# VCISwang/STCD

Hardware: AMD Instinct MI355X
Metric: image-pairs/sec (256x256 bf16 SiamUnet_diff train) (higher is better)
Workload: dtype bf16; 1 GPU; SiamUnet_diff(3,2) 256x256 full training step (fwd + cross_entropy + bwd + AdamW), 16 pairs/GPU, synthetic LEVIR-CD-shaped pairs resident in HBM; global_batch=16, image=256, parallelism=dp1

## Files before the change

include/stcd_hip.h:

```cpp
#ifndef STCD_HIP_H
#define STCD_HIP_H

#include <stdint.h>

#ifdef __cplusplus
extern "C" {
#endif

#define STCD_ABI_VERSION 2

#define STCD_ARCH_DIFF 0
#define STCD_ARCH_CONC 1
#define STCD_ARCH_SUB 2
#define STCD_ARCH_SNUNET 3
#define STCD_ARCH_SEGCD 4
#define STCD_ARCH_SEGCD_R18 5
#define STCD_ARCH_SEGCD_R34 6
#define STCD_ARCH_SEGCD_R101 7
#define STCD_ARCH_SEGCD_R152 8
#define STCD_ARCH_FCEF 9
#define STCD_ARCH_XCONC 10
#define STCD_ARCH_SNUNET_CONC 11
#define STCD_ARCH_SNUNET_CONC_DS 12
#define STCD_ARCH_UNETSEG 16
// ... 16 lines not shown
    int64_t numel;
} stcd_tensor_info;

typedef struct stcd_bn_info {
    char name[64];
    int32_t channels;
    int32_t calls_per_forward;
    int64_t offset;
} stcd_bn_info;

typedef struct stcd_dropout_info {
    char name[64];
    int32_t rows;
    int32_t channels;
    int64_t offset;
} stcd_dropout_info;

typedef struct stcd_cf_config {
    int32_t in_ch, out_ch;
    int32_t embed_dims[4];
    int32_t depths[4];
    int32_t num_heads[4];
    int32_t sr_ratios[4];
    int32_t mlp_ratio;
    int32_t embedding_dim;
    int32_t patch1, patch;
    float drop_rate, attn_drop, drop_path_rate;
    float diff_drop;
} stcd_cf_config;

typedef struct stcd_cf_site {
    char name[96];
    int32_t ndim;
    int32_t dims[4];
    float p;
} stcd_cf_site;

const char* stcd_last_error(void);
int stcd_abi_version(void);

int stcd_create(int arch, int in_ch, int label_ch, int dtype, stcd_engine** out);
int stcd_cf_default_config(stcd_cf_config* cfg);
int stcd_create_changeformer(const stcd_cf_config* cfg, int dtype, stcd_engine** out);
void stcd_destroy(stcd_engine* e);
int64_t stcd_output_floats(const stcd_engine* e);
int stcd_cf_output_info(const stcd_engine* e, int i, int64_t* offset, int* height, int* width);
int stcd_cf_num_sites(const stcd_engine* e);
int stcd_cf_site_get(const stcd_engine* e, int i, stcd_cf_site* out);
uint32_t stcd_cf_site_seed(uint64_t seed, int site);
int stcd_cf_set_drop_rates(stcd_engine* e, float drop_rate, float attn_drop, float diff_drop);
int stcd_cf_set_aux_backward(stcd_engine* e, int on);
int stcd_set_wgrad_side(stcd_engine* e, int on);

int stcd_num_params(const stcd_engine* e);
int stcd_param_info(const stcd_engine* e, int i, stcd_tensor_info* info);
int64_t stcd_param_floats(const stcd_engine* e);
int stcd_num_bn(const stcd_engine* e);
int stcd_bn_info_get(const stcd_engine* e, int i, stcd_bn_info* info);
int64_t stcd_bn_floats(const stcd_engine* e);

int stcd_configure(stcd_engine* e, int batch, int height, int width);
int64_t stcd_workspace_bytes(const stcd_engine* e);
int stcd_num_dropout(const stcd_engine* e);
int stcd_dropout_info_get(const stcd_engine* e, int i, stcd_dropout_info* info);
int64_t stcd_dropout_floats(const stcd_engine* e);
int stcd_set_dropout_p(stcd_engine* e, float p);

int stcd_forward(stcd_engine* e, const float* x1, const float* x2, const float* params, float* bn_running,
                 const float* dropout_masks, uint64_t dropout_seed, int training, float* logits,
                 void* workspace, void* hip_stream);

int stcd_backward(stcd_engine* e, const float* grad_logits, const float* params, float* grads,
                  void* workspace, int stage, void* hip_stream);
int stcd_set_weights_tag(stcd_engine* e, uint64_t tag);
int stcd_grad_stage_range(const stcd_engine* e, int stage, int64_t* begin, int64_t* end);

typedef struct stcd_ws_tensor {
    char name[96];
    int64_t offset_bytes;
    int n, h, w, c, ld;
    int dtype;
} stcd_ws_tensor;
int stcd_set_debug(stcd_engine* e, int flags);
int stcd_ws_tensor_count(const stcd_engine* e);
int stcd_ws_tensor_get(const stcd_engine* e, int index, stcd_ws_tensor* out);

#define STCD_PROFILE_CLASSES 8
int stcd_profile_enable(stcd_engine* e, int on);
int stcd_profile_read(stcd_engine* e, int klass, double* total_ms, int64_t* launches, double* flops, double* bytes);
int stcd_profile_num_kernels(const stcd_engine* e);
int stcd_profile_kernel(stcd_engine* e, int i, char* name, int name_cap, double* total_ms, int64_t* launches, double* flops,
                        double* bytes);

int64_t stcd_loss_scratch_bytes(void);
int stcd_loss_ce(const float* logits, const int64_t* target, int batch, int classes, int64_t hw, int ignore_index,
                 float* loss_out, float* dlogits, void* scratch, void* hip_stream);
int stcd_loss_bce_dice(const float* x, const float* target, int64_t numel, int from_logits, float* loss_out, float* dx,
                       void* scratch, void* hip_stream);
int stcd_loss_contrastive(const float* pred, const int64_t* cd_label, const int64_t* pse_label, int64_t numel_half, float* loss_out,
                          float* dpred, void* scratch, void* hip_stream);
int stcd_loss_focal(const float* x, const int64_t* target, int batch, int classes, int64_t hw, const float* alpha, float gamma,
                    float smooth, int flags, float* loss_out, float* dx, void* scratch, void* hip_stream);
int64_t stcd_loss_iou_scratch_bytes(int batch, int classes, int64_t hw);
int stcd_loss_iou(const float* logits, const int64_t* target, int batch, int classes, int64_t hw, const float* weight, int mode,
                  float* loss_out, float* dlogits, void* scratch, void* hip_stream);
int stcd_confusion_update(const float* logits, const int64_t* target, int batch, int classes, int64_t hw,
                          int64_t* cm, void* hip_stream);

int stcd_adam_step(float* params, const float* grads, float* exp_avg, float* exp_avg_sq, int64_t numel, int64_t step,
                   double lr, double beta1, double beta2, double eps, double weight_decay, int decoupled, void* hip_stream);

int stcd_adam_hyper(int64_t step, double lr, double beta1, double beta2, double eps, double weight_decay, float* hyper_host8);
int stcd_adam_step_dev(float* params, const float* grads, float* exp_avg, float* exp_avg_sq, int64_t numel, const float* hyper_dev8,
                       int decoupled, void* hip_stream);

int stcd_pseudo_pair(const uint8_t* img_a, const uint8_t* donor, const uint8_t* mask, const uint8_t* change, const float* alpha,
                     const int32_t* erase_xywh, uint64_t seed, int batch, int height, int width, const float* mean3,
                     const float* std3, float* x1, float* x2, int64_t* c_label, int64_t* s_label_a, int64_t* s_label_b,
                     void* hip_stream);

int64_t stcd_augment_scratch_bytes(int n_images, int height, int width);
int stcd_augment(const float* x, const float* params, int n_images, int height, int width, const float* mean3, const float* std3,
                 float* out, void* scratch, int64_t scratch_bytes, void* hip_stream);

int stcd_scene_gather(const uint8_t* scene_a, const uint8_t* scene_b, int height, int width, int tile, int stride, int tiles_x,
                      int first_tile, int n_tiles, const float* mean3, const float* std3, float* x1, float* x2, void* hip_stream);
int stcd_scene_stitch(const float* logits, int classes, int height, int width, int tile, int stride, int tiles_x, int tiles_y,
                      int first_tile, int n_tiles, const float* window, float* acc, float* wsum, void* hip_stream);
int stcd_scene_finalize(const float* acc, const float* wsum, int classes, int height, int width, float threshold,
                        const uint8_t* label, uint8_t* mask, float* prob, int64_t* cm, void* hip_stream);
int stcd_scene_gather_d4(const uint8_t* scene_a, const uint8_t* scene_b, int height, int width, int tile, int stride, int tiles_x,
                         int first_tile, int n_tiles, const float* mean3, const float* std3, float* x1, float* x2, int d4,
                         void* hip_stream);
int stcd_scene_stitch_d4(const float* logits, int classes, int height, int width, int tile, int stride, int tiles_x, int tiles_y,
                         int first_tile, int n_tiles, const float* window, float* acc, float* wsum, int d4, void* hip_stream);
int stcd_scene_gather_one_d4(const uint8_t* scene, int height, int width, int tile, int stride, int tiles_x, int first_tile,
                             int n_tiles, const float* mean3, const float* std3, float* x, int d4, void* hip_stream);
#define STCD_SCENE_MAX_HEADS 3
int stcd_scene_stitch_heads_d4(const float* const* logits, int n_heads, int classes, int height, int width, int tile, int stride,
                               int tiles_x, int tiles_y, int first_tile, int n_tiles, const float* window, float* acc, float* wsum,
                               int d4, void* hip_stream);
int stcd_scene_finalize_seg(const float* acc, const float* wsum, int classes, int height, int width, float seg_threshold,
                            float change_threshold, const uint8_t* label_a, const uint8_t* label_b, const uint8_t* label_c,
                            uint8_t* seg_a, uint8_t* seg_b, uint8_t* change, uint8_t* gated, float* prob, int64_t* cm,
                            void* hip_stream);

#define STCD_SELFTRAIN_MAX_MODELS 8
int stcd_selftrain_score(const float* const* logits, int n_models, int batch, int classes, int64_t hw, float threshold,
                         const uint8_t* label, int mask_value, uint8_t* mask, int64_t* agree, int64_t* cm, void* hip_stream);

int stcd_scene_cell_agree(const uint8_t* const* masks, int n_models, int height, int width, int cell, int cells_x, int cells_y,
                          const uint8_t* label, int64_t* agree, int64_t* cm, void* hip_stream);
int stcd_mask_close(const uint8_t* in, int height, int width, int radius, int mask_value, uint8_t* out, void* hip_stream);

int64_t stcd_objects_scratch_bytes(int height, int width);
int stcd_objects_label(const uint8_t* mask, int height, int width, int connectivity, int invert, int32_t* labels, int32_t* count,
                       void* scratch, int64_t scratch_bytes, void* hip_stream);
int stcd_objects_table(const int32_t* labels, int height, int width, int n, const uint8_t* overlay, int64_t* area, int32_t* bbox,
                       int64_t* overlap, void* hip_stream);
int stcd_mask_filter_objects(const uint8_t* in, int height, int width, int connectivity, int64_t min_area, int64_t max_hole,
                             int mask_value, uint8_t* out, void* scratch, int64_t scratch_bytes, void* hip_stream);

int64_t stcd_rings_scratch_bytes(int height, int width, int64_t max_corners);
int stcd_rings_count(const int32_t* labels, int height, int width, int connectivity, int64_t max_corners, int64_t* counts, void* scratch,
                     int64_t scratch_bytes, void* hip_stream);
int stcd_rings_write(const int32_t* labels, int height, int width, int connectivity, int64_t max_corners, int64_t n_rings, int64_t n_vertices,
// ... 105 lines not shown
```

stcd_amd/_lib.py:

```python
from __future__ import annotations

import ctypes as C
import os

import torch

_HERE = os.path.dirname(os.path.abspath(__file__))
LIB_PATH = os.environ.get("STCD_LIB_PATH") or os.path.join(_HERE, "libstcd_hip.so")

ARCH_DIFF, ARCH_CONC, ARCH_SUB, ARCH_SNUNET, ARCH_SEGCD = 0, 1, 2, 3, 4
ARCH_SEGCD_R18, ARCH_SEGCD_R34, ARCH_SEGCD_R101, ARCH_SEGCD_R152 = 5, 6, 7, 8
ARCH_FCEF = 9
ARCH_XCONC = 10
ARCH_SNUNET_CONC = 11
ARCH_SNUNET_CONC_DS = 12
ARCH_UNETSEG = 16
ARCH_FFCTLCD = 32
ARCH_BASE_RESNET = 48
ARCH_BIT = 52
ARCH_CHANGEFORMER = 64
DTYPE_F32, DTYPE_BF16 = 0, 1
ARCH_IDS = {"diff": ARCH_DIFF, "conc": ARCH_CONC, "sub": ARCH_SUB, "fcef": ARCH_FCEF, "xconc": ARCH_XCONC, "snunet": ARCH_SNUNET, "snunet_conc": ARCH_SNUNET_CONC, "snunet_conc_ds": ARCH_SNUNET_CONC_DS, "segcd": ARCH_SEGCD,
            "segcd_resnet50": ARCH_SEGCD, "segcd_resnet18": ARCH_SEGCD_R18, "segcd_resnet34": ARCH_SEGCD_R34,
            "segcd_resnet101": ARCH_SEGCD_R101, "segcd_resnet152": ARCH_SEGCD_R152,
# ... 16 lines not shown
class BnInfo(C.Structure):
    _fields_ = [("name", C.c_char * 64), ("channels", C.c_int32), ("calls_per_forward", C.c_int32),
                ("offset", C.c_int64)]


class DropoutInfo(C.Structure):
    _fields_ = [("name", C.c_char * 64), ("rows", C.c_int32), ("channels", C.c_int32), ("offset", C.c_int64)]


class ConvGeom(C.Structure):
    _fields_ = [("n", C.c_int32), ("hi", C.c_int32), ("wi", C.c_int32), ("ci", C.c_int32), ("ldi", C.c_int32),
                ("hm", C.c_int32), ("wm", C.c_int32), ("in_stride", C.c_int32),
                ("ho", C.c_int32), ("wo", C.c_int32), ("out_stride", C.c_int32), ("oy0", C.c_int32), ("ox0", C.c_int32),
                ("co", C.c_int32), ("ldo", C.c_int32), ("ntaps", C.c_int32),
                ("dy", C.c_int8 * 9), ("dx", C.c_int8 * 9), ("pad_", C.c_int8 * 2)]


class WsTensor(C.Structure):
    _fields_ = [("name", C.c_char * 96), ("offset_bytes", C.c_int64), ("n", C.c_int), ("h", C.c_int), ("w", C.c_int), ("c", C.c_int),
                ("ld", C.c_int), ("dtype", C.c_int)]


class CfConfig(C.Structure):
    _fields_ = [("in_ch", C.c_int32), ("out_ch", C.c_int32), ("embed_dims", C.c_int32 * 4), ("depths", C.c_int32 * 4),
                ("num_heads", C.c_int32 * 4), ("sr_ratios", C.c_int32 * 4), ("mlp_ratio", C.c_int32), ("embedding_dim", C.c_int32),
                ("patch1", C.c_int32), ("patch", C.c_int32), ("drop_rate", C.c_float), ("attn_drop", C.c_float),
                ("drop_path_rate", C.c_float), ("diff_drop", C.c_float)]


class CfSite(C.Structure):
    _fields_ = [("name", C.c_char * 96), ("ndim", C.c_int32), ("dims", C.c_int32 * 4), ("p", C.c_float)]


class MapGeom(C.Structure):
    _fields_ = [("n", C.c_int32), ("h", C.c_int32), ("w", C.c_int32), ("c", C.c_int32), ("groups", C.c_int32)]


CONV_SMALL, CONV_RES, CONV_TILE, CONV_GEMM, CONV_HALO, CONV_DMA = range(6)


class ConvFused(C.Structure):
    _fields_ = [("kernel", C.c_int32), ("groups", C.c_int32),
                ("sum_acc", C.c_void_p), ("sum_c0", C.c_int32), ("sum_c", C.c_int32), ("sum_scale1", C.c_float), ("sum_scale2", C.c_float),
                ("use_epi", C.c_int32), ("relu", C.c_int32), ("gate", C.c_void_p), ("res", C.c_void_p), ("ldg", C.c_int32), ("ldr", C.c_int32),
                ("alpha", C.c_float), ("beta", C.c_float),
                ("bw_y", C.c_void_p), ("bw_stat", C.c_void_p), ("bw_mask", C.c_void_p), ("bw_acc", C.c_void_p), ("bw_ldy", C.c_int32),
                ("blocks", C.c_int32), ("tiles_per_group", C.c_int32), ("blocks_per_group", C.c_int32), ("bn_rep", C.c_int32),
                ("tile_m", C.c_int32)]


_vp, _i, _i64, _f, _d = C.c_void_p, C.c_int, C.c_int64, C.c_float, C.c_double
_PROTOS = {
    "stcd_last_error": (C.c_char_p, []),
    "stcd_abi_version": (_i, []),
    "stcd_create": (_i, [_i, _i, _i, _i, C.POINTER(_vp)]),
    "stcd_destroy": (None, [_vp]),
    "stcd_cf_default_config": (_i, [C.POINTER(CfConfig)]),
    "stcd_create_changeformer": (_i, [C.POINTER(CfConfig), _i, C.POINTER(_vp)]),
    "stcd_output_floats": (_i64, [_vp]),
    "stcd_cf_output_info": (_i, [_vp, _i, C.POINTER(_i64), C.POINTER(_i), C.POINTER(_i)]),
    "stcd_cf_num_sites": (_i, [_vp]),
    "stcd_cf_site_get": (_i, [_vp, _i, C.POINTER(CfSite)]),
    "stcd_cf_site_seed": (C.c_uint32, [C.c_uint64, _i]),
    "stcd_cf_set_drop_rates": (_i, [_vp, _f, _f, _f]),
    "stcd_cf_set_aux_backward": (_i, [_vp, _i]),
    "stcd_set_wgrad_side": (_i, [_vp, _i]),
    "stcd_num_params": (_i, [_vp]),
    "stcd_param_info": (_i, [_vp, _i, C.POINTER(TensorInfo)]),
    "stcd_param_floats": (_i64, [_vp]),
    "stcd_num_bn": (_i, [_vp]),
    "stcd_bn_info_get": (_i, [_vp, _i, C.POINTER(BnInfo)]),
    "stcd_bn_floats": (_i64, [_vp]),
    "stcd_configure": (_i, [_vp, _i, _i, _i]),
    "stcd_workspace_bytes": (_i64, [_vp]),
    "stcd_num_dropout": (_i, [_vp]),
    "stcd_dropout_info_get": (_i, [_vp, _i, C.POINTER(DropoutInfo)]),
    "stcd_dropout_floats": (_i64, [_vp]),
    "stcd_set_dropout_p": (_i, [_vp, _f]),
    "stcd_forward": (_i, [_vp, _vp, _vp, _vp, _vp, _vp, C.c_uint64, _i, _vp, _vp, _vp]),
    "stcd_backward": (_i, [_vp, _vp, _vp, _vp, _vp, _i, _vp]),
    "stcd_grad_stage_range": (_i, [_vp, _i, C.POINTER(_i64), C.POINTER(_i64)]),
    "stcd_set_weights_tag": (_i, [_vp, C.c_uint64]),
    "stcd_set_debug": (_i, [_vp, _i]),
    "stcd_ws_tensor_count": (_i, [_vp]),
    "stcd_ws_tensor_get": (_i, [_vp, _i, C.POINTER(WsTensor)]),
    "stcd_profile_enable": (_i, [_vp, _i]),
    "stcd_profile_read": (_i, [_vp, _i, C.POINTER(C.c_double), C.POINTER(_i64), C.POINTER(C.c_double), C.POINTER(C.c_double)]),
    "stcd_profile_num_kernels": (_i, [_vp]),
    "stcd_profile_kernel": (_i, [_vp, _i, C.c_char_p, _i, C.POINTER(C.c_double), C.POINTER(_i64), C.POINTER(C.c_double), C.POINTER(C.c_double)]),
    "stcd_loss_scratch_bytes": (_i64, []),
    "stcd_loss_ce": (_i, [_vp, _vp, _i, _i, _i64, _i, _vp, _vp, _vp, _vp]),
    "stcd_loss_bce_dice": (_i, [_vp, _vp, _i64, _i, _vp, _vp, _vp, _vp]),
    "stcd_loss_contrastive": (_i, [_vp, _vp, _vp, _i64, _vp, _vp, _vp, _vp]),
    "stcd_loss_focal": (_i, [_vp, _vp, _i, _i, _i64, _vp, _f, _f, _i, _vp, _vp, _vp, _vp]),
    "stcd_loss_iou_scratch_bytes": (_i64, [_i, _i, _i64]),
    "stcd_loss_iou": (_i, [_vp, _vp, _i, _i, _i64, _vp, _i, _vp, _vp, _vp, _vp]),
    "stcd_confusion_update": (_i, [_vp, _vp, _i, _i, _i64, _vp, _vp]),
    "stcd_adam_step": (_i, [_vp, _vp, _vp, _vp, _i64, _i64, _d, _d, _d, _d, _d, _i, _vp]),
    "stcd_adam_hyper": (_i, [_i64, _d, _d, _d, _d, _d, C.POINTER(_f)]),
    "stcd_adam_step_dev": (_i, [_vp, _vp, _vp, _vp, _i64, _vp, _i, _vp]),
    "stcd_pseudo_pair": (_i, [_vp, _vp, _vp, _vp, _vp, _vp, C.c_uint64, _i, _i, _i, C.POINTER(_f), C.POINTER(_f), _vp, _vp, _vp, _vp, _vp, _vp]),
    "stcd_augment_scratch_bytes": (_i64, [_i, _i, _i]),
    "stcd_augment": (_i, [_vp, _vp, _i, _i, _i, C.POINTER(_f), C.POINTER(_f), _vp, _vp, _i64, _vp]),
    "stcd_scene_gather": (_i, [_vp, _vp, _i, _i, _i, _i, _i, _i, _i, C.POINTER(_f), C.POINTER(_f), _vp, _vp, _vp]),
    "stcd_scene_stitch": (_i, [_vp, _i, _i, _i, _i, _i, _i, _i, _i, _i, _vp, _vp, _vp, _vp]),
    "stcd_scene_finalize": (_i, [_vp, _vp, _i, _i, _i, _f, _vp, _vp, _vp, _vp, _vp]),
    "stcd_scene_gather_d4": (_i, [_vp, _vp, _i, _i, _i, _i, _i, _i, _i, C.POINTER(_f), C.POINTER(_f), _vp, _vp, _i, _vp]),
    "stcd_scene_stitch_d4": (_i, [_vp, _i, _i, _i, _i, _i, _i, _i, _i, _i, _vp, _vp, _vp, _i, _vp]),
    "stcd_scene_gather_one_d4": (_i, [_vp, _i, _i, _i, _i, _i, _i, _i, C.POINTER(_f), C.POINTER(_f), _vp, _i, _vp]),
    "stcd_scene_stitch_heads_d4": (_i, [C.POINTER(_vp), _i, _i, _i, _i, _i, _i, _i, _i, _i, _i, _vp, _vp, _vp, _i, _vp]),
    "stcd_scene_finalize_seg": (_i, [_vp, _vp, _i, _i, _i, _f, _f, _vp, _vp, _vp, _vp, _vp, _vp, _vp, _vp, _vp, _vp]),
    "stcd_selftrain_score": (_i, [C.POINTER(_vp), _i, _i, _i, _i64, _f, _vp, _i, _vp, _vp, _vp, _vp]),
    "stcd_scene_cell_agree": (_i, [C.POINTER(_vp), _i, _i, _i, _i, _i, _i, _vp, _vp, _vp, _vp]),
    "stcd_mask_close": (_i, [_vp, _i, _i, _i, _i, _vp, _vp]),
    "stcd_objects_scratch_bytes": (_i64, [_i, _i]),
    "stcd_objects_label": (_i, [_vp, _i, _i, _i, _i, _vp, _vp, _vp, _i64, _vp]),
    "stcd_objects_table": (_i, [_vp, _i, _i, _i, _vp, _vp, _vp, _vp, _vp]),
    "stcd_mask_filter_objects": (_i, [_vp, _i, _i, _i, _i64, _i64, _i, _vp, _vp, _i64, _vp]),
    "stcd_rings_scratch_bytes": (_i64, [_i, _i, _i64]),
    "stcd_rings_count": (_i, [_vp, _i, _i, _i, _i64, _vp, _vp, _i64, _vp]),
    "stcd_rings_write": (_i, [_vp, _i, _i, _i, _i64, _i64, _i64, _vp, _vp, _vp, _vp, _vp, _i64, _vp]),
    "stcd_op_conv": (_i, [_i, _i, C.POINTER(ConvGeom), _vp, _vp, _vp, _vp, _vp, _i64, _vp]),
    "stcd_op_conv_fused": (_i, [C.POINTER(ConvGeom), C.POINTER(ConvFused), _vp, _vp, _vp, _vp, _vp, _i64, _vp]),
    "stcd_op_wgrad": (_i, [_i, _i, C.POINTER(ConvGeom), _vp, _vp, _vp, _vp, _i64, _vp]),
    "stcd_op_scratch_bytes": (_i64, [C.POINTER(ConvGeom)]),
    "stcd_op_ew_scratch_bytes": (_i64, [C.POINTER(MapGeom)]),
    "stcd_op_bn_act": (_i, [_i, C.POINTER(MapGeom), _vp, _i, _vp, _vp, _vp, _vp, _vp, _i, _i, _vp, _i, _vp, _i, _vp, _vp, _i64, _vp]),
    "stcd_op_bn_act_pair": (_i, [_i, C.POINTER(MapGeom), _vp, _i, _vp, _vp, _vp, _vp, _vp, _i, _vp, _i, _vp, _i, _vp, _i, _vp, _vp, _i64, _vp]),
    "stcd_op_bn_act_bwd": (_i, [_i, C.POINTER(MapGeom), _vp, _i, _vp, _i, _vp, _vp, _i, _vp, _i, _vp, _vp, _vp, _i64, _vp]),
    "stcd_op_maxpool": (_i, [_i, C.POINTER(MapGeom), _vp, _i, _vp, _i, _vp]),
    "stcd_op_maxpool_bwd": (_i, [_i, C.POINTER(MapGeom), _vp, _i, _vp, _i, _vp, _i, _i, _vp]),
    "stcd_op_maxpool3": (_i, [_i, C.POINTER(MapGeom), _vp, _i, _vp, _i, _vp, _vp]),
    "stcd_op_maxpool3_bwd": (_i, [_i, C.POINTER(MapGeom), _vp, _vp, _i, _vp, _i, _vp]),
    "stcd_op_pairdw_scratch_bytes": (_i64, [C.POINTER(MapGeom)]),
    "stcd_op_pairdw": (_i, [_i, C.POINTER(MapGeom), _vp, _i, _vp, _vp, _vp, _i, _vp]),
    "stcd_op_pairdw_bwd": (_i, [_i, C.POINTER(MapGeom), _vp, _i, _vp, _i, _vp, _vp, _i, _vp, _vp, _i64, _vp]),
    "stcd_op_fuse": (_i, [_i, _i, C.POINTER(MapGeom), _vp, _i, _vp, _i, _vp]),
    "stcd_op_fuse_bwd": (_i, [_i, _i, C.POINTER(MapGeom), _vp, _i, _vp, _i, _vp, _i, _vp]),
    "stcd_op_rep_pad": (_i, [_i, C.POINTER(MapGeom), _vp, _i, _i, _i, _vp]),
    "stcd_op_rep_pad_bwd": (_i, [_i, C.POINTER(MapGeom), _vp, _i, _i, _i, _vp]),
    "stcd_op_skip_bwd": (_i, [_i, _i, C.POINTER(MapGeom), _vp, _i, _vp, _i, _vp, _i, _vp, _i, _vp, _vp, _vp, _i, _vp, _i, _vp, _vp, _vp, _i64, _vp]),
    "stcd_op_cf_scratch_bytes": (_i64, [_i64, _i, _i, _i, _i]),
    "stcd_op_cf_im2col": (_i, [_i, _vp, _vp, _i, _i, _i, _i, _i, _i, _i, _i, _vp]),
    "stcd_op_cf_col2im": (_i, [_i, _vp, _i, _vp, _i, _i, _i, _i, _i, _i, _i, _i, _vp]),
    "stcd_op_cf_layernorm": (_i, [_i, _vp, _vp, _vp, _vp, _vp, _i64, _i, _f, _vp]),
    "stcd_op_cf_layernorm_bwd": (_i, [_i, _vp, _vp, _vp, _vp, _vp, _vp, _vp, _vp, _vp, _vp, _i64, _i, _vp]),
    "stcd_op_cf_colsum": (_i, [_i, _vp, _i64, _i, _vp, _vp, _vp]),
    "stcd_op_cf_attention": (_i, [_i, _vp, _vp, _vp, _vp, _i, _i, _i, _i, _i, _f, C.c_uint64, _vp]),
    "stcd_op_cf_attention_scratch_bytes": (_i64, [_i, _i, _i, _i, _i]),
    "stcd_op_cf_attention_bwd": (_i, [_i, _vp, _vp, _vp, _vp, _vp, _vp, _vp, _vp, _i, _i, _i, _i, _i, _f, C.c_uint64, _vp]),
    "stcd_op_cf_dwgelu": (_i, [_i, _vp, _vp, _vp, _vp, _vp, _i, _i, _i, _i, _f, C.c_uint64, _vp]),
    "stcd_op_cf_dwgelu_scratch_bytes": (_i64, [_i, _i, _i, _i]),
    "stcd_op_cf_dwgelu_bwd": (_i, [_i, _vp, _vp, _vp, _vp, _vp, _vp, _vp, _vp, _i, _i, _i, _i, _f, C.c_uint64, _vp]),
    "stcd_op_cf_resid_drop": (_i, [_i, _vp, _vp, _vp, _i, _i64, _i, _f, _f, C.c_uint64, _i, _vp]),
    "stcd_op_cf_bilinear": (_i, [_i, _vp, _vp, _i, _i, _i, _i, _i, _i, _i, _i, _vp]),
    "stcd_op_cf_elementwise": (_i, [_i, _i, _vp, _vp, _vp, _i64, _i, _vp, _f, _f, _f, C.c_uint64, _vp]),
    "stcd_op_cf_prelu_bwd": (_i, [_i, _vp, _vp, _vp, _vp, _vp, _vp, _i64, _i, _vp]),
}
EXPORTS = tuple(_PROTOS)

_lib = None


class StcdError(RuntimeError):
    pass

# ... 22 lines not shown
```

stcd_amd/csrc/common.h:

```cpp
#pragma once
#include <hip/hip_runtime.h>
#include <stdint.h>
#include <stdio.h>
#include <stdlib.h>
#include <string>
#include <string.h>

#include "../../include/stcd_hip.h"

namespace stcd {

typedef __bf16 bf16;

enum DType { F32 = STCD_DTYPE_F32, BF16 = STCD_DTYPE_BF16 };
inline size_t dsize(int dt) { return dt == BF16 ? 2 : 4; }

void set_error(const std::string& msg);

static inline int env_int(const char* name, int dflt) { const char* v = getenv(name); return v ? atoi(v) : dflt; }
static inline bool env_flag(const char* name, bool dflt) { const char* v = getenv(name); return v && v[0] == (dflt ? '0' : '1') ? !dflt : dflt; }

#define STCD_CHECK_AS(fn, cond, msg)                                       \
    do {                                                                   \
        if (!(cond)) {                                                     \
            ::stcd::set_error(std::string(fn) + ": " + (msg));             \
            return 1;                                                      \
        }                                                                  \
    } while (0)
#define STCD_CHECK(cond, msg) STCD_CHECK_AS(__func__, cond, msg)

#define STCD_HIP(call)                                                                        \
    do {                                                                                      \
        hipError_t err_ = (call);                                                             \
        if (err_ != hipSuccess) {                                                             \
            ::stcd::set_error(std::string(__func__) + ": " #call ": " + hipGetErrorString(err_)); \
            return 1;                                                                         \
        }                                                                                     \
    } while (0)

template <typename T>
__device__ __forceinline__ void load8(const T* p, float (&v)[8]);
template <>
__device__ __forceinline__ void load8<float>(const float* p, float (&v)[8]) {
    float4 a = *reinterpret_cast<const float4*>(p), b = *reinterpret_cast<const float4*>(p + 4);
    v[0] = a.x; v[1] = a.y; v[2] = a.z; v[3] = a.w; v[4] = b.x; v[5] = b.y; v[6] = b.z; v[7] = b.w;
}
template <>
__device__ __forceinline__ void load8<bf16>(const bf16* p, float (&v)[8]) {
    uint4 r = *reinterpret_cast<const uint4*>(p);
    uint32_t w[4] = {r.x, r.y, r.z, r.w};
#pragma unroll
    for (int i = 0; i < 4; ++i) {
        v[2 * i] = __uint_as_float(w[i] << 16);
        v[2 * i + 1] = __uint_as_float(w[i] & 0xffff0000u);
    }
}
template <typename T>
__device__ __forceinline__ void store8(T* p, const float (&v)[8]);
template <>
__device__ __forceinline__ void store8<float>(float* p, const float (&v)[8]) {
    *reinterpret_cast<float4*>(p) = make_float4(v[0], v[1], v[2], v[3]);
    *reinterpret_cast<float4*>(p + 4) = make_float4(v[4], v[5], v[6], v[7]);
}
__device__ __forceinline__ void barrier_lds() { asm volatile("s_waitcnt lgkmcnt(0)\n\ts_barrier" ::: "memory"); }

__device__ __forceinline__ uint32_t pack_bf16x2(float lo, float hi) {
    typedef __attribute__((ext_vector_type(2))) __bf16 bf16x2;
    bf16x2 t;
    t[0] = (__bf16)lo;
    t[1] = (__bf16)hi;
    return __builtin_bit_cast(uint32_t, t);
}
template <>
__device__ __forceinline__ void store8<bf16>(bf16* p, const float (&v)[8]) {
    uint4 r;
    r.x = pack_bf16x2(v[0], v[1]); r.y = pack_bf16x2(v[2], v[3]);
    r.z = pack_bf16x2(v[4], v[5]); r.w = pack_bf16x2(v[6], v[7]);
    *reinterpret_cast<uint4*>(p) = r;
}
template <typename T>
__device__ __forceinline__ float round_as(float v) { return (float)(T)v; }

__device__ __forceinline__ float wave_sum(float v) {
#pragma unroll
    for (int o = 32; o > 0; o >>= 1) v += __shfl_xor(v, o, 64);
    return v;
}

constexpr int BN_REP = 8;
constexpr float BN_FS1 = 67108864.f;
constexpr float BN_FS2 = 262144.f;
constexpr float BN_BS = 68719476736.f;
inline int64_t bn_acc_bytes(int groups, int C) { return (int64_t)BN_REP * groups * 2 * C * 8; }
__device__ __forceinline__ void bn_acc_add(long long* acc, int rep, int groups, int C, int g, int which, int c, double v, float scale) {
    const long long q = (long long)llrint(v * (double)scale);
    atomicAdd(reinterpret_cast<unsigned long long*>(acc + (((int64_t)(rep & (BN_REP - 1)) * groups + g) * 2 + which) * C + c),
              (unsigned long long)q);
}
__device__ __forceinline__ double bn_acc_get(const long long* __restrict__ acc, int groups, int C, int g, int which, int c, float scale) {
    long long s = 0;
#pragma unroll
    for (int r = 0; r < BN_REP; ++r) s += acc[(((int64_t)r * groups + g) * 2 + which) * C + c];
    return (double)s * (1.0 / (double)scale);
}
__device__ __forceinline__ double bn_rsqrt(double x) {
    double y = (double)__frsqrt_rn((float)x);
    y = y * (1.5 - 0.5 * x * y * y);
    return y * (1.5 - 0.5 * x * y * y);
}

__device__ __forceinline__ void bn_fwd_table(float* tab, const long long* __restrict__ facc, const float* __restrict__ gamma,
                                             const float* __restrict__ beta, float* __restrict__ rmean, float* __restrict__ rvar,
                                             float* __restrict__ stat, int C, int groups, int64_t ppg, float momentum, float eps,
                                             bool publish, int cbase = 0, int CS = 0, int g_first = 0) {
    if (CS == 0) CS = C;
    const double inv_n = 1.0 / (double)ppg;
    for (int cl = threadIdx.x; cl < CS; cl += blockDim.x) {
        const int c = cbase + cl;
        if (facc) {
            const float gam = gamma[c], bet = beta[c];
            float rm = (publish && rmean) ? rmean[c] : 0.f, rv = (publish && rvar) ? rvar[c] : 0.f;
            for (int gi = 0; gi < groups; ++gi) {
                int g = gi + g_first;
                if (g >= groups) g -= groups;
                const double s1 = bn_acc_get(facc, groups, C, g, 0, c, BN_FS1), s2 = bn_acc_get(facc, groups, C, g, 1, c, BN_FS2);
                const double mean = s1 * inv_n;
                double var = s2 * inv_n - mean * mean;
                if (var < 0.0) var = 0.0;
                const double invstd = bn_rsqrt(var + (double)eps);
                const float sc = (float)(gam * invstd), sh = (float)(bet - mean * gam * invstd);
                tab[(g * 2 + 0) * CS + cl] = sc;
                tab[(g * 2 + 1) * CS + cl] = sh;
                if (publish) {
                    float* st = stat + (int64_t)g * 4 * C;
                    st[c] = (float)mean; st[C + c] = (float)invstd; st[2 * C + c] = sc; st[3 * C + c] = sh;
                    const double unb = ppg > 1 ? var * ((double)ppg / (double)(ppg - 1)) : var;
                    rm = (float)((1.0 - momentum) * rm + momentum * mean);
                    rv = (float)((1.0 - momentum) * rv + momentum * unb);
                }
            }
            if (publish && rmean) rmean[c] = rm;
            if (publish && rvar) rvar[c] = rv;
        } else if (gamma) {
            const float invstd = 1.f / sqrtf(rvar[c] + eps);
            const float sc = gamma[c] * invstd, sh = beta[c] - rmean[c] * gamma[c] * invstd;
            for (int g = 0; g < groups; ++g) {
                tab[(g * 2 + 0) * CS + cl] = sc;
                tab[(g * 2 + 1) * CS + cl] = sh;
            }
        } else {
            for (int g = 0; g < groups; ++g) {
                tab[(g * 2 + 0) * CS + cl] = stat[(int64_t)g * 4 * C + 2 * C + c];
                tab[(g * 2 + 1) * CS + cl] = stat[(int64_t)g * 4 * C + 3 * C + c];
            }
        }
    }
}

struct XfSrc {
    const long long* facc = nullptr;
    const float* gamma = nullptr;
    const float* beta = nullptr;
    float* rmean = nullptr; float* rvar = nullptr;
    float* stat = nullptr;
    const float* mask = nullptr;
    int C = 0, groups = 1, npg = 0, publish = 0;
    long long ppg = 0;
    float momentum = 0.1f, eps = 1e-5f;
    int on = 0;
};
__device__ __forceinline__ uint4 xf_act8(const uint4 raw, const float (&sc)[8], const float (&sh)[8], const unsigned okm) {
    typedef short s16x2 __attribute__((ext_vector_type(2)));
    const uint32_t w[4] = {raw.x, raw.y, raw.z, raw.w};
    uint32_t o[4];
#pragma unroll
    for (int i = 0; i < 4; ++i) {
        const float lo = fmaf(__uint_as_float(w[i] << 16), sc[2 * i], sh[2 * i]);
        const float hi = fmaf(__uint_as_float(w[i] & 0xffff0000u), sc[2 * i + 1], sh[2 * i + 1]);
        const s16x2 p = __builtin_bit_cast(s16x2, pack_bf16x2(lo, hi));
        o[i] = __builtin_bit_cast(uint32_t, __builtin_elementwise_max(p, s16x2{0, 0})) & okm;
    }
    return make_uint4(o[0], o[1], o[2], o[3]);
}
__device__ __forceinline__ void xf_fold8(const float* __restrict__ tab_sc, const float* __restrict__ tab_sh, const float4 m0, const float4 m1,
                                         float (&sc)[8], float (&sh)[8]) {
    const float mk[8] = {m0.x, m0.y, m0.z, m0.w, m1.x, m1.y, m1.z, m1.w};
#pragma unroll
    for (int j = 0; j < 8; ++j) { sc[j] = tab_sc[j] * mk[j]; sh[j] = tab_sh[j] * mk[j]; }
}


void launch_in_pack(int dt, const float* x1, const float* x2, void* X, int B, int cin, int H, int W, hipStream_t s, int dates = 2);
void launch_gout_pack(int dt, const float* g, void* G, int B, int L, int H, int W, hipStream_t s, long long* bias_acc = nullptr);
struct BiasJob { int64_t acc_off; int64_t out_off; int C, valid; float scale; int pad_; };
void launch_bias_finish(const BiasJob* jobs_dev, int njobs, const char* ws, float* grads, hipStream_t s);

void launch_conv_ref(int dt, const stcd_conv_geom& g, const void* in, const float* w, int kpad, int wld,
                     const float* bias, void* out, bool out_nchw_f32, hipStream_t s);
void launch_wgrad_ref(int dt, const stcd_conv_geom& g, const void* in, const void* dout, float* dw, int kpad, int wld,
                      hipStream_t s);
void launch_wgrad_ref_f64(int dt, const stcd_conv_geom& g, const void* in, const void* dout, double* dw, int kpad, int wld,
                          hipStream_t s);

struct ConvMfmaPlan {
    int CiB = 0, nchunks = 0, KS = 0, modeB = 0, NT = 0, NTtot = 0;
    int64_t wf_elems = 0;
    bool ok = false;
};
ConvMfmaPlan conv_mfma_plan(const stcd_conv_geom& g);
void launch_pack_frag(const stcd_conv_geom& g, const ConvMfmaPlan& p, const float* w, int kpad, int wld, void* dst,
                      hipStream_t s);
int launch_conv_mfma(const stcd_conv_geom& g, const ConvMfmaPlan& p, const void* in, const void* wf, const float* bias,
                     void* out, bool out_nchw_f32, hipStream_t s);
bool conv_mfma_x4_ok(const stcd_conv_geom g[4], const ConvMfmaPlan p[4]);
int launch_conv_mfma_x4(const stcd_conv_geom g[4], const ConvMfmaPlan p[4], const void* in, const void* const wf[4],
                        const float* bias, void* out, hipStream_t s);
struct ConvResPlan {
    int NT = 0, CW = 32, nslices = 0, P = 0, blocks = 0;
    int filt_bytes = 0, lds_bytes = 0;
    int single_halo = 0;
    bool ok = false;
};
ConvResPlan conv_res_plan(const stcd_conv_geom& g, const ConvMfmaPlan& p, int groups);
struct BwdSum {
    const void* Y = nullptr; int ldy = 0;
    const float* stat = nullptr;
    const float* mask = nullptr;
    long long* acc = nullptr;
    int groups = 1;
};
int launch_conv_res(const stcd_conv_geom& g, const ConvMfmaPlan& p, const ConvResPlan& rp, const void* in, const void* wf,
                    const float* bias, void* out, int groups, long long* stat_acc, int cpad, hipStream_t s, int stat_c0 = 0,
                    float s1_scale = BN_FS1, float s2_scale = BN_FS2, const XfSrc* xf = nullptr, const BwdSum* bs = nullptr);
bool conv_res_bwdsum_ok(const stcd_conv_geom& g, const ConvResPlan& rp);
bool conv_res_xf_ok(const stcd_conv_geom& g, const ConvResPlan& rp, int groups, const XfSrc& xf);
struct ConvTilePlan {
    int NT = 0, nparts = 0, nbuf = 0, nslices = 0, P = 0, blocks = 0, ntiles = 0;
    int filt_bytes = 0, lds_bytes = 0;
    bool ok = false;
};
ConvTilePlan conv_tile_plan(const stcd_conv_geom& g, const ConvMfmaPlan& p, int groups);
int launch_conv_tile(const stcd_conv_geom& g, const ConvMfmaPlan& p, const ConvTilePlan& tp, const void* in, const void* wf,
                     const float* bias, void* out, int groups, long long* stat_acc, int cpad, hipStream_t s, int stat_c0 = 0,
                     float s1_scale = BN_FS1, float s2_scale = BN_FS2);
struct ConvGemmPlan {
    int W = 0;
    int tiles_m = 0, tiles_n = 0, blocks = 0, lds_bytes = 0;
    int pix_chunks = 0;
    bool ok = false;
};
ConvGemmPlan conv_gemm_plan(const stcd_conv_geom& g, const ConvMfmaPlan& p, int groups);
struct ConvEpi {
    int relu = 0;
    const void* gate = nullptr; int ldg = 0;
    const void* res = nullptr; int ldr = 0;
    float alpha = 1.f, beta = 1.f;
};
int launch_conv_gemm(const stcd_conv_geom& g, const ConvMfmaPlan& p, const ConvGemmPlan& gp, const void* in, const void* wf,
                   const float* bias, void* out, int groups, long long* stat_acc, int cpad, hipStream_t s, int stat_c0 = 0,
                   float s1_scale = BN_FS1, float s2_scale = BN_FS2, const ConvEpi* epi = nullptr);
struct ConvHaloPlan {
    int NH = 0;
    int nslices = 0, P = 0, blocks = 0, lds_bytes = 0;
    bool ok = false;
};
ConvHaloPlan conv_halo_plan(const stcd_conv_geom& g, const ConvMfmaPlan& p);
int launch_conv_halo(const stcd_conv_geom& g, const ConvMfmaPlan& p, const ConvHaloPlan& hp, const void* in, const void* wf,
                     const float* bias, void* out, hipStream_t s, const ConvEpi* epi = nullptr);

struct ConvDmaPlan {
    int tiles_m = 0, tiles_n = 0, blocks = 0, lds_bytes = 0;
    bool ok = false;
};
ConvDmaPlan conv_dma_plan(const stcd_conv_geom& g, const ConvMfmaPlan& p);
int launch_conv_dma(const stcd_conv_geom& g, const ConvMfmaPlan& p, const ConvDmaPlan& dp, const void* in, const void* wf,
                    const float* bias, void* out, hipStream_t s, const ConvEpi* epi = nullptr);
// ... 6 lines not shown
bool conv_small_call_ok(const stcd_conv_geom& g, int groups, const XfSrc* xf);
bool conv_small_bwdsum_ok(const stcd_conv_geom& g);
struct WgradMfmaPlan {
    int WCI = 1, NTW = 1, gx = 1, gy = 1, gz = 1;
    int64_t slab_floats = 0;
    int wi_valid = 0;
    int gemm = 0;
    int dma = 0;
    bool ok = false;
};
WgradMfmaPlan wgrad_mfma_plan(const stcd_conv_geom& g, int kpad, int wld, bool allow_wide = false, int force_co64 = -1);
int launch_wgrad_mfma(const stcd_conv_geom& g, const WgradMfmaPlan& p, const void* in, const void* dout, float* slab,
                      int kpad, int wld, hipStream_t s);
struct WgradJob {
    stcd_conv_geom g;
    int64_t in_off, dout_off, slab_off;
    int kpad, wld;
    int dymin, dxmin, HH, HWp;
    int tiles_x, tiles_y, ntiles;
    int xrow_bytes;
    int x_bytes, y_bytes;
    int co_valid;
    unsigned in_bytes, dout_bytes;
    int gx, gy, gz;
    int start;
    int lds_bytes;
    int wi_valid;
    int dma_L, dma_nk;
    int pad_;
    int64_t xf_stat_off, xf_mask_off;
    int xf_C, xf_groups, xf_npg, pad2_;
};
WgradMfmaPlan wgrad_gemm_plan(const stcd_conv_geom& g, int kpad, int wld);
WgradJob wgrad_gemm_make_job(const stcd_conv_geom& g, const WgradMfmaPlan& p, int64_t in_off, int64_t dout_off, int64_t slab_off,
                             int kpad, int wld);
int launch_wgrad_gemm_group(int W, const WgradJob* jobs_dev, int njobs, int total_blocks, const char* base, hipStream_t s);
WgradMfmaPlan wgrad_dma_plan(const stcd_conv_geom& g, int kpad, int wld);
void wgrad_dma_set_split(WgradMfmaPlan& p, const stcd_conv_geom& g, int S, int kpad, int wld);
WgradJob wgrad_dma_make_job(const stcd_conv_geom& g, const WgradMfmaPlan& p, int64_t in_off, int64_t dout_off, int64_t slab_off,
                            int kpad, int wld);
int launch_wgrad_dma_group(const WgradJob* jobs_dev, int njobs, int total_blocks, const char* base, hipStream_t s);
WgradJob wgrad_make_job(const stcd_conv_geom& g, const WgradMfmaPlan& p, int64_t in_off, int64_t dout_off, int64_t slab_off,
                        int kpad, int wld);
void wgrad_job_set_xf(WgradJob& a, int64_t stat_off, int64_t mask_off, int C, int groups, int npg);
int wgrad_variant_slots(int WCI, int NTW, bool t9, int lds_bytes);
int launch_wgrad_group(int WCI, int NTW, bool t9, const WgradJob* jobs_dev, int njobs, int total_blocks, int lds_bytes,
                       const char* base, hipStream_t s, bool xf = false);
struct PackSpec;
struct ReduceJob {
    int64_t start, count;
    int64_t slab_off;
    int64_t out_off;
    int64_t slab_stride;
    int gx, ntaps, K, N, kpad, wld;
    int ks, kn_major;
    int8_t ky[9], kx[9];
    int8_t tiled, parts, pad_[4];
};
void launch_reduce_jobs(const ReduceJob* jobs_dev, int njobs, int64_t total, const char* ws, float* grads, hipStream_t s);
void launch_reduce_dw(const float* slab, int gx, const stcd_conv_geom& g, int K, int N, int kpad, int wld,
                      const PackSpec* ps, float* out, hipStream_t s);

struct PackSpec {
    int ks;
    int kn_major;
    int K, N, wld;
    int kpad;
    int ntaps;
    int8_t ky[9], kx[9];
};
void launch_pack_w(const PackSpec& ps, const float* src, float* dst, hipStream_t s);
void launch_unpack_dw(const PackSpec& ps, const double* dwe, float* gsrc, hipStream_t s);

struct PackJob {
    int64_t start, count;
    int64_t src_off;
    int64_t dst_off;
    int kind;
    PackSpec ps;
    int Ci, Co, CiB, nchunks, KS, NTtot, modeB;
    int aux;
};
void launch_pack_jobs(const PackJob* jobs_dev, int njobs, int64_t total, const float* params, char* ws, hipStream_t s);

int bn_stats_chunks(int64_t pixels_per_group, int C);
void launch_bn_stats(int dt, const void* Y, int ld, int C, int groups, int64_t pixels_per_group, long long* acc, hipStream_t s);
void launch_bn_eval_prepare(int C, int groups, const float* gamma, const float* beta, const float* running_mean,
                            const float* running_var, float* stat, float eps, hipStream_t s);
constexpr int MAX_VIEWS = 6;
struct SliceViews {
    int n = 0;
    void* p[MAX_VIEWS]; int ld[MAX_VIEWS]; int64_t goff[MAX_VIEWS]; int gmask[MAX_VIEWS];
};
struct BnActArgs {
    const void* Y; int ldy;
    void* A; int lda; int64_t a_group_off;
    void* P; int ldp;
    float* stat;
    const float* mask;
    int C, groups, npg, H, W;
    int relu;
    const void* res = nullptr; int ldres = 0;
    const long long* facc = nullptr;
    const float* gamma = nullptr; const float* beta = nullptr;
    float* running_mean = nullptr; float* running_var = nullptr;
    float momentum = 0.1f, eps = 1e-5f;
    SliceViews extra;
    int g_first = 0;
};
void launch_bn_act(int dt, const BnActArgs& a, hipStream_t s);
void launch_bn_act_pair(int dt, const BnActArgs& a, void* F, int ldf, int fmode, hipStream_t s);
void launch_maxpool(int dt, const void* A, int lda, void* P, int ldp, int N, int H, int W, int C, hipStream_t s);

void launch_fuse(int dt, int mode, const void* A, int lda, int64_t a_goff, void* D, int ldd, int B, int64_t HW, int C,
                 hipStream_t s);
void launch_fuse_bwd(int dt, int mode, const void* A, int lda, int64_t a_goff, const void* dD, int ldd, void* dA, int ldda,
                     int64_t da_goff, int B, int64_t HW, int C, hipStream_t s);
void launch_rep_pad(int dt, void* D, int ld, int N, int H, int W, int h0, int w0, int C, hipStream_t s);
void launch_rep_pad_bwd(int dt, void* dD, int ld, int N, int H, int W, int h0, int w0, int C, hipStream_t s);

void launch_bn_bwd_reduce(int dt, const void* dA, int ldda, int64_t da_goff, const void* Y, int ldy, const float* stat,
                          const float* mask, int C, int groups, int npg, int64_t HW, int relu, long long* bacc,
                          hipStream_t s, const void* res = nullptr, int ldres = 0, const SliceViews* extra_src = nullptr,
                          int base_valid = 1, void* dA_sum = nullptr);
void launch_bn_bwd_apply(int dt, const void* dA, int ldda, int64_t da_goff, void* dY, int lddy, const void* Y, int ldy,
                         const float* stat, const long long* bacc, float* dgamma, float* dbeta, const float* mask, int C, int groups,
                         int npg, int64_t HW, int relu, hipStream_t s, const void* res = nullptr, int ldres = 0,
                         void* dZout = nullptr, int lddz = 0, const void* extra = nullptr, int ldex = 0,
                         float* dbeta_copy = nullptr);
void launch_pairdw_fwd(int dt, const void* A, int lda, int64_t goff, void* G, int ldg, const float* w, const float* b, int B, int H,
                       int W, int C, hipStream_t s);
void launch_pairdw_bwd_data(int dt, const void* dG, int lddg, void* dA, int ldda, int64_t goff, const float* w, int B, int H, int W,
                            int C, hipStream_t s);
int64_t pairdw_partial_floats(int B, int H, int W, int C);
void launch_pairdw_bwd_filter(int dt, const void* A, int lda, int64_t goff, const void* dG, int lddg, float* dw, float* partial, int B,
                              int H, int W, int C, hipStream_t s);
void launch_slice(int dt, void* dst, int ldd, const void* src, int lds, int64_t pixels, int C, int accumulate, hipStream_t s);
void launch_ecam_forward(int dt, const void* X, int ld, void* Z, int ldz, int N, int64_t HW, int C4, const float* w1a,
                         const float* w2a, const float* w1b, const float* w2b, float* pool, int64_t* argm, float* att,
                         float* hid, float* part, hipStream_t s);
int64_t ecam_part_floats(int N, int C4);
void launch_ecam_backward(int dt, const void* X, int ld, const void* dZ, int lddz, void* dX, int lddx, int N, int64_t HW, int C4,
                          const float* w1a, const float* w2a, const float* w1b, const float* w2b, float* gw1a, float* gw2a,
                          float* gw1b, float* gw2b, const float* pool, const int64_t* argm, const float* att, const float* hid,
                          float* sums, float* dpool, float* part, hipStream_t s);
struct SnHeadParams { const float* w[4]; const float* b[4]; const float* wf; const float* bf; int L, ds; };
struct SnHeadGrads { float* w[4]; float* b[4]; float* wf; float* bf; };
int64_t snhead_scratch_floats(int B, int64_t HW, int L, int ds);
void launch_snhead_forward(int dt, const void* E, int ld, const SnHeadParams& p, float* out, int B, int64_t HW, hipStream_t s);
void launch_snhead_backward(int dt, const void* E, int ld, const SnHeadParams& p, const SnHeadGrads& g, const float* G, void* dE,
                            int ldd, float* scratch, int B, int64_t HW, hipStream_t s);
void launch_pool_bwd(int dt, const void* A, int lda, int64_t a_goff, const void* dP, int ldp, void* dA, int ldda,
                     int64_t da_goff, int groups, int npg, int H, int W, int C, int accumulate, hipStream_t s);
bool skip_pair_supported(int B, int H, int W, int C);
void launch_skip_bwd_pair(int dt, int mode, const void* Y, int ldy, const void* dD, int ldd, const void* dP, int ldp, void* dA,
                          int ldda, int64_t da_goff, const float* stat, const float* mask, int B, int H, int W, int C,
                          long long* partial, hipStream_t s);
void launch_skip_bwd(int dt, int mode, const void* A, int lda, int64_t a_goff, const void* Y, int ldy, const void* dD, int ldd,
                     const void* dP, int ldp, void* dA, int ldda, int64_t da_goff, const float* stat, const float* mask, int B,
                     int H, int W, int C, long long* bacc, hipStream_t s);
void launch_bias_grad(int dt, const void* dY, int ld, int64_t pixels, int C, float* db, hipStream_t s, long long* acc_i = nullptr);
void launch_dropout_gen(float* mask, int64_t n, uint64_t seed, float p, hipStream_t s);
void launch_fill(float* p, int64_t n, float v, hipStream_t s);

void launch_stem_fwd(int dt, const void* X, const float* w, void* Y, int N, int H, int W, int cin, int Co, hipStream_t s);
int64_t stem_wgrad_part_floats(int N, int H, int W, int cin, int Co);
// ... 160 lines not shown
```

stcd_amd/csrc/engine.hip:

```cpp
#include <algorithm>
#include <climits>
#include <cstdint>
#include <array>
#include <cstring>
#include <memory>
#include <vector>

#include "common.h"

namespace stcd {

static thread_local std::string g_err;
void set_error(const std::string& msg) { g_err = msg; }

enum ConvKind { K_CONV3 = 0, K_CONVT3_S1 = 1, K_UPCONV = 2, K_CONV1 = 3, K_CONVT2 = 4, K_CONV3_S2 = 5, K_CONV1_S2 = 6, K_STEM7 = 7 };

struct TRef { int64_t off = -1; int ld = 0; };
struct GRef { int64_t off = -1; int ld = 0; int64_t goff = 0; };

static inline int round8(int c) { return (c + 7) & ~7; }

struct ConvW {
    std::string name;
    int kind = 0, cin = 0, cout = 0;
// ... 139 lines not shown
    std::vector<ViewRef> extra_dst;
    std::vector<ViewRef> grad_src;
    bool grad_base = false;
    ConvOp f1, f2, d1, d2; WgradOp w1, w2;
};
struct SnUp {
    int conv = -1, N = 0, h = 0, w = 0, C = 0;
    TRef src, dsrc, out, dOut, tmp;
    ConvOp fwd[4], dgr; WgradOp wg[4];
    int64_t bias_acc = -1; bool bias_fused = false; int coff = 0;
};

struct CfPlan;
struct stcd_engine_impl {
    Prof prof;
    std::shared_ptr<CfPlan> cf;
    std::vector<NBlock> sn_blocks;
    std::vector<SnUp> sn_ups;
    std::vector<int> sn_order;
    std::vector<XConc> xc;
    int sn_final = -1;
    int64_t sn_w[4] = {0, 0, 0, 0};
    TRef snE, sndE, snZ, sndZ;
    TRef sn_dbg_dE;
    int64_t sn_pool = -1, sn_argm = -1, sn_att = -1, sn_hid = -1, sn_sums = -1, sn_dpool = -1, sn_part = -1;
    int64_t sn_dout_begin = -1, sn_dout_end = -1;
    ConvOp sn_final_fwd, sn_final_dgr; WgradOp sn_final_wg;
    int64_t snc_w[5] = {0, 0, 0, 0, 0}, snc_b[5] = {0, 0, 0, 0, 0}, snc_scratch = -1;
    std::vector<GLayer> g_layers;
    std::vector<GStep> g_fwd;
    int g_stem = -1, g_head_conv = -1;
    int debug_flags = 0;
    std::vector<stcd_ws_tensor> ws_tensors;
    std::vector<std::array<int, 4>> g_blocks;
    int seg_x = 4, seg_layers[4] = {3, 4, 6, 3};
    int seg_dates = 2;
    bool seg_ffc = false;
    TRef g_pool_idc;
    std::vector<std::array<int, 2>> g_dec;
    TRef gP0, gdP0, gX3, gdX3, gFuseTmp;
    int64_t g_pool_idx = -1;
    int64_t g_stem_part = -1;
    int64_t g_raw3 = -1, g_draw3 = -1;
    ConvOp g_head_fwd, g_head_dgr; WgradOp g_head_wg;
    bool bres = false; int seg_nstage = 4;
    int g_head_c = 16;
    int g_cls = -1, g_pred_conv = -1;
    ConvOp g_pred_fwd, g_pred_dgr; WgradOp g_pred_wg;
    int64_t g_pred_bias_acc = -1;
    struct BitPlan {
        bool on = false; int L = 1, dh = 64;
        int64_t pos_off = 0, wa_off = 0, enc_off = 0, dec_off = 0;
        int64_t tok_in = -1, tok_out = -1, dtok_out = -1, dtok_in = -1, stat = -1, AP = -1, dAP = -1, xs = -1, dG = -1, dec_part = -1,
                dmh = -1, dm = -1, enc_part = -1, tok_part = -1;
        TRef dec_din;
    } bit;
    int arch = 0, in_ch = 3, label = 2, dt = F32;
    int64_t min_bn_count = 0;
    float drop_p = 0.2f;
    std::vector<stcd_tensor_info> params;
    int64_t param_floats = 0, enc_param_end = 0;
    std::vector<ConvW> convs;
    std::vector<BnP> bns;
    int64_t bn_floats = 0;
    bool configured = false, fwd_training = false;
    int B = 0, H = 0, W = 0;
    std::vector<DropP> drops;
    int64_t drop_floats = 0;
    int64_t ws_bytes = 0;
    std::vector<Cbrd> enc, dec;
    std::vector<UpConv> ups;
    int final_conv = -1;
    ConvOp final_fwd, final_dgr; WgradOp final_wg;
    const Cbrd* final_dgr_bwd = nullptr;
    const Cbrd* final_xsrc = nullptr;
    int use_virt = 0;
    int fc_virt_layers = 0;
    std::vector<ConvOp*> conv_ops;
    int64_t slab = -1, slab_floats = 0;
    std::vector<WgradOp*> wgrad_ops;
    std::vector<WgradGroup> wgroups[2];
    std::vector<ReduceJob> rjobs[2];
    int64_t rjobs_total[2] = {0, 0}, rjobs_off[2] = {-1, -1};
    std::vector<PackJob> jobs[2];
    int64_t jobs_total[2] = {0, 0}, jobs_off[2] = {-1, -1};
    const void* jobs_uploaded_ws = nullptr;
    uint64_t weights_tag = 0, packed_tag = 0;
    const void* packed_ws = nullptr; const void* packed_params = nullptr; int packed_level = -1;
    TRef X0, G, finalIn, dFinalIn;
    int Hs[5] = {0}, Ws[5] = {0};
    TRef D[4], dD[4], P[4], dP[4];
    int64_t zero_begin = -1, zero_end = -1;
    int64_t final_bias_acc = -1;
    std::vector<BiasJob> bias_jobs; int64_t bias_jobs_off = -1;
    int64_t masks = -1, dwe_begin = -1, dwe_end = -1, scratch8 = -1;
    int use_mfma = 1, use_small = 1, use_wgroup = 1, use_res = 1, use_skip_fused = 1, use_act_fuse = 1, use_gemm = 1, use_skip_recompute = 1, use_bwdsum = 1, use_bwdsum_res = 0, use_tile = 1, use_halo = 0;
    int wg_side_on = 1;
    static constexpr int WG_SIDE_DIV = 4;
    static constexpr int WGROUP_ROUNDS = 1, WGROUP_MIN_TILES = 8;
    bool wg_early = false; hipStream_t wg_cur_side = nullptr;
    hipStream_t wg_side = nullptr; hipEvent_t wg_fork = nullptr, wg_join = nullptr; int wg_side_dev = -1;
};

}

using namespace stcd;
struct stcd_engine : stcd_engine_impl {};

namespace stcd {

static const int ENC_STAGE_CONVS[4] = {2, 2, 3, 3};
static const int ENC_C[4] = {16, 32, 64, 128};
static const int SKIP_IDX[4] = {1, 3, 6, 9};

static void add_param(stcd_engine& e, const std::string& name, std::initializer_list<int64_t> shape, int64_t* off_out) {
    stcd_tensor_info ti;
    memset(&ti, 0, sizeof(ti));
    snprintf(ti.name, sizeof(ti.name), "%s", name.c_str());
    ti.ndim = (int)shape.size();
    int64_t n = 1;
    int i = 0;
    for (auto s : shape) { ti.shape[i++] = s; n *= s; }
    ti.numel = n;
    ti.offset = e.param_floats;
    *off_out = ti.offset;
    e.param_floats += (n + 3) & ~(int64_t)3;
    e.params.push_back(ti);
}

static void make_specs(ConvW& c, bool need_dgrad) {
    if (c.kind == K_STEM7) {
        c.fwd = PackSpec{}; c.dgrad = PackSpec{};
        c.fwd.ks = 7; c.fwd.K = c.cin; c.fwd.N = c.cout; c.fwd.kpad = c.kin_p; c.fwd.wld = c.nout_p;
        return;
    }
    if (c.kind == K_CONV3_S2) {
        PackSpec& f = c.fwd;
        f.ks = 3; f.K = c.cin; f.N = c.cout; f.kpad = c.kin_p; f.wld = c.nout_p; f.ntaps = 9; f.kn_major = 0;
        {
            int t = 0;
            for (int py = 0; py < 2; ++py)
                for (int px = 0; px < 2; ++px)
                    for (int ky = 0; ky < 3; ++ky)
                        for (int kx = 0; kx < 3; ++kx)
                            if ((ky != 1) == (py == 1) && (kx != 1) == (px == 1)) { f.ky[t] = ky; f.kx[t] = kx; ++t; }
        }
        PackSpec& d = c.dgrad;
        d.ks = 3; d.K = c.cout; d.N = c.cin; d.kpad = c.nout_p; d.wld = round8(c.cin); d.ntaps = need_dgrad ? 9 : 0; d.kn_major = 1;
        int t = 0;
        for (int py = 0; py < 2; ++py)
            for (int px = 0; px < 2; ++px)
                for (int dy = 0; dy <= py; ++dy)
                    for (int dx = 0; dx <= px; ++dx) { d.ky[t] = py + 1 - 2 * dy; d.kx[t] = px + 1 - 2 * dx; ++t; }
        return;
    }
    if (c.kind == K_CONV1 || c.kind == K_CONVT2 || c.kind == K_CONV1_S2) {
        const int ks = c.kind == K_CONVT2 ? 2 : 1;
        PackSpec& f = c.fwd;
        f.ks = ks; f.K = c.cin; f.N = c.cout; f.kpad = c.kin_p; f.wld = c.nout_p;
        f.ntaps = ks * ks;
        f.kn_major = c.kind == K_CONVT2;
        for (int t = 0; t < f.ntaps; ++t) { f.ky[t] = t / ks; f.kx[t] = t % ks; }
        PackSpec& d = c.dgrad;
        d.ks = ks; d.K = c.cout; d.N = c.cin; d.kpad = c.nout_p; d.wld = round8(c.cin);
        d.ntaps = need_dgrad ? ks * ks : 0;
        d.kn_major = c.kind != K_CONVT2;
// ... 242 lines not shown

constexpr int TILE_MAX_TILES = 512;
static void pick_tile(const stcd_engine& e, ConvOp& op, const stcd_conv_geom& g, int groups) {
    if (!e.use_tile || !op.res.ok || op.gemm.ok || op.small) return;
    const ConvTilePlan tp = conv_tile_plan(g, op.plan, groups);
    if (tp.ok && tp.ntiles <= TILE_MAX_TILES) op.tile = tp;
}

static WgradMfmaPlan pick_wgrad_plan(const stcd_engine& e, const stcd_conv_geom& g, int kpad, int wld) {
    if (e.use_gemm && e.use_wgroup && 2.0 * g.n * g.hm * g.wm * (double)g.ci * g.co >= 0.8e9) {
        WgradMfmaPlan p = wgrad_gemm_plan(g, kpad, wld);
        if (p.ok) return p;
    }
    if (e.use_wgroup && (g.ntaps == 9 || (e.cf && g.ntaps == 4)) && (int64_t)g.n * g.hm * g.wm >= 65536) {
        WgradMfmaPlan p = wgrad_dma_plan(g, kpad, wld);
        if (p.ok) return p;
    }
    return wgrad_mfma_plan(g, kpad, wld, is_snunet(e.arch) || (e.cf && g.ntaps == 9));
}

static void plan_conv(const stcd_engine& e, ConvOp& op, int groups, bool with_tile) {
    op.plan = conv_mfma_plan(op.g);
    op.small = conv_small_ok(op.g, op.plan);
    if (e.use_res && !op.small) op.res = conv_res_plan(op.g, op.plan, groups);
    pick_gemm_or_res(e, op, op.g, groups);
    if (with_tile) pick_tile(e, op, op.g, groups);
}
static bool conv_on_ref(bool mfma, const ConvOp& op) { return !(mfma && op.plan.ok && op.wf >= 0); }
struct Binder {
    stcd_engine& e; Planner& ws;
    bool with_tile = false;
    void conv(ConvOp& op, const stcd_conv_geom& g, int conv, bool dgrad, int tap0, int kreal, int nreal, int groups = 1) const {
        op = ConvOp();
        op.g = g; op.conv = conv; op.dgrad = dgrad; op.tap0 = tap0; op.kreal = kreal; op.nreal = nreal; op.res_groups = groups;
        if (e.dt == BF16) plan_conv(e, op, groups, with_tile);
        if (op.plan.ok) op.wf = ws.take(op.plan.wf_elems * 2);
        e.conv_ops.push_back(&op);
    }
    void stem(ConvOp& op, const stcd_conv_geom& g, int conv, int groups) const {
        op = ConvOp();
        op.g = g; op.conv = conv; op.kreal = e.convs[conv].cin; op.nreal = g.co; op.res_groups = groups;
        op.plan = conv_mfma_plan(g);
        if (g.ldi == 8 && g.co % 64 == 0) op.gemm = conv_gemm_plan(g, op.plan, groups);
        op.gemm.pix_chunks = 1;
        if (!op.gemm.ok) return;
        op.wf = ws.take(op.plan.wf_elems * 2);
        e.conv_ops.push_back(&op);
    }
    void wgrad(WgradOp& op, const stcd_conv_geom& g, int conv, int64_t in_off, int64_t dout_off, int stage = 0, int tap0 = 0,
               int wi_valid = 0, const int8_t* own_ky = nullptr, const int8_t* own_kx = nullptr) const {
        const ConvW& cv = e.convs[conv];
        op = WgradOp();
        op.g = g; op.conv = conv; op.tap0 = tap0; op.kreal = cv.cin; op.nreal = cv.cout;
        op.in_off = in_off; op.dout_off = dout_off; op.stage = stage;
        op.own_taps = own_ky != nullptr;
        for (int t = 0; t < g.ntaps && op.own_taps; ++t) { op.oky[t] = own_ky[t]; op.okx[t] = own_kx[t]; }
        if (e.dt == BF16) { op.plan = pick_wgrad_plan(e, g, cv.fwd.kpad, cv.fwd.wld); op.plan.wi_valid = wi_valid; }
        e.wgrad_ops.push_back(&op);
    }
};
static void take_ref_images(stcd_engine& e, Planner& ws, bool with_dwe = true) {
    for (auto& c : e.convs) {
        c.wpk_fwd = ws.take((int64_t)c.fwd.ntaps * c.fwd.kpad * c.fwd.wld * 4);
        if (c.dgrad.ntaps) c.wpk_dgrad = ws.take((int64_t)c.dgrad.ntaps * c.dgrad.kpad * c.dgrad.wld * 4);
    }
    e.dwe_begin = ws.cur;
    for (auto& c : e.convs) {
        c.dwe_floats = (int64_t)c.fwd.ntaps * c.fwd.kpad * c.fwd.wld;
        c.dwe = with_dwe ? ws.take(c.dwe_floats * 8) : -1;
    }
    e.dwe_end = ws.cur;
}

static bool same_group(const WgradGroup& G, const WgradOp& op) {
    const bool t9 = !op.plan.dma && op.g.ntaps == 9;
    return G.gemm == op.plan.gemm && G.dma == op.plan.dma && G.WCI == op.plan.WCI && G.NTW == op.plan.NTW && G.t9 == t9 && G.xf == (op.xf_C > 0);
}

static bool cf_side_on() { static const bool on = env_flag("STCD_CF_SIDE", true); return on; }

static void build_pack_jobs(stcd_engine& e, Planner& ws) {
    for (int st = 0; st < 2; ++st) { e.rjobs[st].clear(); e.rjobs_total[st] = 0; }
    for (int st = 0; st < 2; ++st) e.wgroups[st].clear();
    if (e.dt == BF16 && e.use_mfma) {
        if (e.use_wgroup) {
            for (WgradOp* op : e.wgrad_ops) {
                if (!op->plan.ok) continue;
                const bool t9 = !op->plan.dma && op->g.ntaps == 9;
                std::vector<WgradGroup>& gs = e.wgroups[op->stage];
                size_t gi = 0;
                while (gi < gs.size() && !same_group(gs[gi], *op)) ++gi;
                if (gi == gs.size()) { WgradGroup g; g.WCI = op->plan.WCI; g.NTW = op->plan.NTW; g.t9 = t9; g.gemm = op->plan.gemm; g.dma = op->plan.dma; g.xf = op->xf_C > 0; gs.push_back(g); }
                op->grouped = true;
            }
            for (int st = 0; st < 2; ++st)
                for (WgradGroup& G : e.wgroups[st]) {
                    if (G.gemm) { G.lds_bytes = 2 * 2 * G.gemm * (64 * 64 + 8 * 32); continue; }
                    if (G.dma) {
                        G.lds_bytes = 128 * 1024;
                        std::vector<WgradOp*> dops;
                        for (WgradOp* op : e.wgrad_ops)
                            if (op->grouped && op->stage == st && op->plan.dma) dops.push_back(op);
                        auto blocks_at = [&](int64_t kt) {
                            int64_t b = 0;
                            for (WgradOp* op : dops) {
                                const int64_t M = (int64_t)op->g.n * op->g.hi * op->g.wi;
                                b += ((M + kt * 64 - 1) / (kt * 64)) * op->plan.gy * op->plan.gz;
                            }
                            return b;
                        };
                        int64_t lo = 1, hi = 1;
                        const int dma_blocks = e.wg_side_on && cf_side_on() ? 192 : 256;
                        while (blocks_at(hi) > dma_blocks) hi *= 2;
                        while (lo < hi) { const int64_t mid = (lo + hi) / 2; if (blocks_at(mid) <= dma_blocks) hi = mid; else lo = mid + 1; }
                        for (WgradOp* op : dops) {
                            const ConvW& cv = e.convs[op->conv];
                            const int64_t M = (int64_t)op->g.n * op->g.hi * op->g.wi;
                            int64_t S = (M + lo * 64 - 1) / (lo * 64);
                            const int64_t slab_bytes = (int64_t)op->g.ntaps * cv.fwd.kpad * cv.fwd.wld * 4;
                            S = std::min<int64_t>(S, std::max<int64_t>(1, ((int64_t)64 << 20) / slab_bytes));
                            wgrad_dma_set_split(op->plan, op->g, (int)S, cv.fwd.kpad, cv.fwd.wld);
                        }
                        continue;
                    }
                    std::vector<WgradOp*> ops;
                    int64_t W = 0;
                    for (WgradOp* op : e.wgrad_ops)
                        if (op->grouped && op->stage == st && same_group(G, *op)) {
                            ops.push_back(op);
                            const int64_t ntiles = (int64_t)op->g.n * ((op->g.wm + 15) / 16) * ((op->g.hm + 7) / 8);
                            W += ntiles * op->plan.gy * op->plan.gz;
                        }
                    for (WgradOp* op : ops) {
                        const ConvW& cv = e.convs[op->conv];
                        WgradJob j = wgrad_make_job(op->g, op->plan, 0, 0, 0, cv.fwd.kpad, cv.fwd.wld);
                        if (op->xf_C > 0) wgrad_job_set_xf(j, op->xf_stat_off, op->xf_mask_off, op->xf_C, op->xf_groups, op->xf_npg);
                        G.lds_bytes = std::max(G.lds_bytes, j.lds_bytes);
                    }
                    int slots = wgrad_variant_slots(G.WCI, G.NTW, G.t9, G.lds_bytes);
                    if (st == 0 && e.wg_side_on && fc_family(e)) slots = std::max(64, slots / stcd_engine_impl::WG_SIDE_DIV);
                    const int64_t rounds = stcd_engine_impl::WGROUP_ROUNDS;
                    const int64_t tpb = std::max<int64_t>(stcd_engine_impl::WGROUP_MIN_TILES, (W + rounds * slots - 1) / (rounds * slots));
                    for (WgradOp* op : ops) {
                        const ConvW& cv = e.convs[op->conv];
                        const int64_t ntiles = (int64_t)op->g.n * ((op->g.wm + 15) / 16) * ((op->g.hm + 7) / 8);
                        const int64_t slab_bytes = (int64_t)op->g.ntaps * cv.fwd.kpad * cv.fwd.wld * 4;
                        int64_t gx = std::max<int64_t>(1, (ntiles + tpb - 1) / tpb);
                        gx = std::min<int64_t>(gx, std::max<int64_t>(1, ((int64_t)32 << 20) / slab_bytes));
                        op->plan.gx = (int)gx;
                        op->plan.slab_floats = gx * op->g.ntaps * cv.fwd.kpad * cv.fwd.wld;
                    }
                }
        }
        int64_t cur[2] = {0, 0};
        for (WgradOp* op : e.wgrad_ops) {
            if (!op->plan.ok) continue;
            const ConvW& cv = e.convs[op->conv];
            op->slab = ws.take(op->plan.slab_floats * 4);
            if (op->grouped) {
                for (WgradGroup& G : e.wgroups[op->stage])
                    if (same_group(G, *op)) {
                        op->group = (int)(&G - e.wgroups[op->stage].data());
                        WgradJob j = op->plan.dma ? wgrad_dma_make_job(op->g, op->plan, op->in_off, op->dout_off, op->slab, cv.fwd.kpad, cv.fwd.wld)
                                   : op->plan.gemm ? wgrad_gemm_make_job(op->g, op->plan, op->in_off, op->dout_off, op->slab, cv.fwd.kpad, cv.fwd.wld)
                                                   : wgrad_make_job(op->g, op->plan, op->in_off, op->dout_off, op->slab, cv.fwd.kpad, cv.fwd.wld);
                        if (op->xf_C > 0 && !op->plan.dma && !op->plan.gemm) wgrad_job_set_xf(j, op->xf_stat_off, op->xf_mask_off, op->xf_C, op->xf_groups, op->xf_npg);
                        j.start = G.total_blocks;
                        G.total_blocks += j.gx * j.gy * j.gz;
                        G.jobs.push_back(j);
                        double fl, by;
                        conv_work(e, op->g, op->kreal, op->nreal, &fl, &by);
                        G.flops += fl; G.bytes += by;
                    }
            }
            ReduceJob j{};
            j.slab_off = op->slab; j.out_off = cv.w_off;
            j.slab_stride = (int64_t)op->g.ntaps * cv.fwd.kpad * cv.fwd.wld;
            j.gx = op->plan.gx; j.ntaps = op->g.ntaps; j.K = cv.cin; j.N = cv.cout; j.kpad = cv.fwd.kpad; j.wld = cv.fwd.wld;
            j.ks = cv.fwd.ks; j.kn_major = cv.fwd.kn_major;
            for (int t = 0; t < op->g.ntaps; ++t) {
                j.ky[t] = op->own_taps ? op->oky[t] : cv.fwd.ky[op->tap0 + t];
                j.kx[t] = op->own_taps ? op->okx[t] : cv.fwd.kx[op->tap0 + t];
            }
            j.tiled = (int64_t)j.ntaps * j.K * j.N >= 512 * 1024;
            if (!j.tiled) {
                const int64_t outs = (int64_t)j.ntaps * j.K * j.N;
                int parts = 1;
                while (parts < 64 && parts * 32 < j.gx) parts *= 2;
                j.parts = (int8_t)parts;
                const int64_t OUTS = 256 / parts;
                j.count = ((outs + OUTS - 1) / OUTS) * 256;
            } else {
                const int TK = j.ntaps == 1 ? 32 : 16;
                const int64_t ntiles = (int64_t)((j.N + 31) / 32) * ((j.K + TK - 1) / TK);
                j.parts = 1;
                j.count = ntiles * 256;
            }
            j.start = cur[op->stage];
            cur[op->stage] += (j.count + 255) & ~(int64_t)255;
            e.rjobs[op->stage].push_back(j);
        }
        for (int st = 0; st < 2; ++st) {
            e.rjobs_total[st] = cur[st];
            e.rjobs_off[st] = ws.take((int64_t)e.rjobs[st].size() * sizeof(ReduceJob) + 16);
            for (WgradGroup& G : e.wgroups[st]) G.table_off = ws.take((int64_t)G.jobs.size() * sizeof(WgradJob) + 16);
        }
    }
    for (int with_dgrad = 0; with_dgrad < 2; ++with_dgrad) {
        std::vector<PackJob>& jobs = e.jobs[with_dgrad];
        jobs.clear();
        int64_t cur = 0;
        auto push = [&](PackJob j) { j.start = cur; cur += (j.count + 255) & ~(int64_t)255; jobs.push_back(j); };
        const bool mfma = e.dt == BF16 && e.use_mfma;
        if (!mfma) {
            for (auto& cv : e.convs)
                for (int d = 0; d <= with_dgrad; ++d) {
                    const PackSpec& ps = d ? cv.dgrad : cv.fwd;
                    if (!ps.ntaps) continue;
                    PackJob j{};
                    j.kind = 0; j.ps = ps; j.src_off = cv.w_off; j.dst_off = d ? cv.wpk_dgrad : cv.wpk_fwd;
                    j.count = (int64_t)ps.ntaps * ps.kpad * ps.wld;
                    push(j);
                }
        } else {
            for (const ConvOp* op : e.conv_ops) {
                if (op->dgrad && !with_dgrad) continue;
                const ConvW& cv = e.convs[op->conv];
                const PackSpec& full = op->dgrad ? cv.dgrad : cv.fwd;
                PackJob j{};
                j.ps = full;
                j.ps.ntaps = op->g.ntaps;
                for (int t = 0; t < op->g.ntaps; ++t) { j.ps.ky[t] = full.ky[op->tap0 + t]; j.ps.kx[t] = full.kx[op->tap0 + t]; }
                j.src_off = cv.w_off;
                if (cv.kind == K_STEM7) {
                    j.kind = 2; j.dst_off = op->wf; j.count = op->plan.wf_elems;
                    j.Co = cv.cout; j.NTtot = op->plan.NTtot; j.aux = cv.cin;
                    push(j);
                    continue;
                }
                if (!conv_on_ref(true, *op)) {
                    j.kind = 1; j.dst_off = op->wf;
                    j.count = op->plan.modeB ? op->plan.wf_elems : op->plan.wf_elems / op->g.ntaps;
                    j.Ci = op->g.ci; j.Co = op->g.co; j.CiB = op->plan.CiB; j.nchunks = op->plan.nchunks; j.KS = op->plan.KS;
                    j.NTtot = op->plan.NTtot; j.modeB = op->plan.modeB;
                } else {
                    j.kind = 0;
                    j.dst_off = (op->dgrad ? cv.wpk_dgrad : cv.wpk_fwd) + (int64_t)op->tap0 * full.kpad * full.wld * 4;
                    j.count = (int64_t)j.ps.ntaps * full.kpad * full.wld;
                }
                push(j);
            }
        }
        e.jobs_total[with_dgrad] = cur;
        e.jobs_off[with_dgrad] = ws.take((int64_t)jobs.size() * sizeof(PackJob) + 16);
    }
}

static int configure_fcsiam(stcd_engine& e, int B, int H, int W) {
    const int64_t T = (int64_t)dsize(e.dt);
    const int ND = fc_dates(e);
    e.Hs[0] = H; e.Ws[0] = W;
    for (int s = 0; s < 4; ++s) { e.Hs[s + 1] = e.Hs[s] / 2; e.Ws[s + 1] = e.Ws[s] / 2; }
    Planner ws(e);
    auto add_drop = [&](const std::string& name, int rows, int C) {
        DropP d; d.name = name; d.rows = rows; d.C = C; d.off = e.drop_floats;
        e.drop_floats += (int64_t)rows * C;
        e.drops.push_back(d);
        return (int)e.drops.size() - 1;
    };

    e.X0 = ws.plain(ND * B, H, W, 8);
    for (int s = 0; s < 4; ++s) {
        int Cd = ENC_C[s] + (e.arch == STCD_ARCH_CONC ? 2 : 1) * ENC_C[s];
        e.D[s] = ws.plain(B, e.Hs[s], e.Ws[s], Cd);
        e.dD[s] = ws.plain(B, e.Hs[s], e.Ws[s], Cd);
        e.P[s] = ws.plain(ND * B, e.Hs[s + 1], e.Ws[s + 1], ENC_C[s]);
        e.dP[s] = ws.plain(ND * B, e.Hs[s + 1], e.Ws[s + 1], ENC_C[s]);
    }
    auto r256 = [](int64_t b) { return (b + 255) & ~(int64_t)255; };
    auto zero_arena = [&](int64_t at, bool assign) {
        auto acc = [&](int groups, int C) { const int64_t o = at; at += r256(bn_acc_bytes(groups, C)); return o; };
        for (int s = 0; s < 4 && fc_cross(e); ++s) {
            const int C = ENC_C[s];
// ... 169 lines not shown
            for (size_t i = 1; i < v.size(); ++i) {
                Cbrd& N = v[i]; Cbrd& P = v[i - 1];
                if (N.has_dIn && N.dgr_sum_acc < 0 && dest_ok(P, N.dgr, N.dIn.off, N.dIn.ld, N.N)) { N.dgr_bwd = &P; P.bwd_sums_fused = true; }
            }
        };
        scan(e.enc); scan(e.dec);
        if (!e.dec.empty() && dest_ok(e.dec.back(), e.final_dgr, e.dFinalIn.off, e.dFinalIn.ld, e.dec.back().N)) {
            e.final_dgr_bwd = &e.dec.back(); e.dec.back().bwd_sums_fused = true;
        }
    }

    e.final_xsrc = nullptr; e.fc_virt_layers = 0;
    for (auto& L : e.enc) { L.virt = false; L.xsrc = nullptr; }
    for (auto& L : e.dec) { L.virt = false; L.xsrc = nullptr; }
    if (e.use_virt && e.dt == BF16 && e.use_mfma && e.use_wgroup && !fc_cross(e)) {
        auto fwd_ok = [&](const ConvOp& op, bool nchw) {
            if (op.wf < 0 || (op.gemm.ok && !nchw)) return false;
            if (op.small && e.use_small) return true;
            return op.res.ok && !nchw && !op.res.single_halo;
        };
        auto wg_ok = [&](const WgradOp& op) { return op.plan.ok && !op.plan.gemm && !op.plan.dma && op.plan.WCI < 4 && op.plan.NTW < 4; };
        auto link = [&](Cbrd& P, ConvOp& cf, WgradOp& cw, bool nchw) {
            if (P.pool || P.fuse_dst.off >= 0) return false;
            if (!fwd_ok(cf, nchw) || !wg_ok(cw)) return false;
            P.virt = true; ++e.fc_virt_layers;
            cw.in_off = P.Y.off;
            cw.xf_stat_off = P.stat;
            cw.xf_mask_off = (P.drop >= 0) ? e.masks + e.drops[P.drop].off * 4 : -1;
            cw.xf_C = e.convs[P.conv].cout; cw.xf_groups = P.groups; cw.xf_npg = P.npg;
            return true;
        };
        for (size_t i = 0; i + 1 < e.enc.size(); ++i) {
            Cbrd& P = e.enc[i]; Cbrd& Cn = e.enc[i + 1];
            if (Cn.in.off != P.A.off) continue;
            if (link(P, Cn.fwd, Cn.wg, false)) { Cn.xsrc = &P; Cn.in.off = P.Y.off; Cn.in.ld = P.Y.ld; }
        }
        for (size_t i = 0; i < e.dec.size(); ++i) {
            Cbrd& P = e.dec[i];
            if (i + 1 < e.dec.size() && e.dec[i + 1].in.off == P.A.off) {
                Cbrd& Cn = e.dec[i + 1];
                if (link(P, Cn.fwd, Cn.wg, false)) { Cn.xsrc = &P; Cn.in.off = P.Y.off; Cn.in.ld = P.Y.ld; }
            } else if (e.finalIn.off == P.A.off) {
                if (link(P, e.final_fwd, e.final_wg, true)) { e.final_xsrc = &P; e.finalIn.off = P.Y.off; e.finalIn.ld = P.Y.ld; }
            }
        }
    }

    {
        size_t di = 0;
        for (int k = 0; k < 4; ++k) {
            UpConv& U = e.ups[k];
            Cbrd& L = e.dec[di];
            int nb = 0;
            for (int j = 0; j < DEC[k].n; ++j) nb += DEC[k].cout[j] >= 0;
            di += nb;
            U.bias_fused = false;
            const bool even = 2 * U.h == U.Ho && 2 * U.w == U.Wo;
            if (e.dt == BF16 && e.use_mfma && nb > 0 && L.has_dIn && L.dIn.off == U.dOut.off && L.dgr.res.ok && L.dgr.wf >= 0 && even) {
                U.bias_fused = true;
                L.dgr_sum_acc = U.bias_acc; L.dgr_sum_c0 = 0; L.dgr_sum_C = U.C;
            }
            if (e.dt == BF16) ws.bias_job(U.bias_acc, U.conv, U.C, U.C);
        }
        ws.bias_job(e.final_bias_acc, e.final_conv, 8, e.label);
    }

    auto rec_layer = [&](const Cbrd& L) {
        const ConvW& cv = e.convs[L.conv];
        ws.tensor(cv.name + (L.xsrc ? ".in.virt" : ".in"), L.in, L.N, L.H, L.W, L.K);
        ws.tensor(cv.name + ".Y", L.Y, L.N, L.H, L.W, cv.cout);
        for (int g = 0; g < L.groups && !L.virt && !skip_recomputed(e, L); ++g)
            ws.tensor(cv.name + ".A.g" + std::to_string(g), L.A.off + g * L.A.goff * T, L.A.ld, L.npg, L.H, L.W, cv.cout);
        ws.tensor(cv.name + ".dY", L.dY, L.N, L.H, L.W, cv.cout);
    };
    for (const Cbrd& L : e.enc) rec_layer(L);
    for (const Cbrd& L : e.dec) rec_layer(L);
    for (const XConc& X : e.xc) {
        const std::string n = "cross_conc" + std::to_string(X.level + 1) + ".diff.0.";
        const Cbrd& R = X.res;
        ws.tensor(n + "Y", X.G, R.N, R.H, R.W, X.C); ws.tensor(n + "A.g0", X.R, R.N, R.H, R.W, X.C); ws.tensor(n + "dY", X.dG, R.N, R.H, R.W, X.C);
        rec_layer(R);
    }

    ws.tables();
    return 0;
}

struct Ctx {
    stcd_engine& e;
    char* ws;
    const float* params;
    float* grads;
    hipStream_t s;
    template <typename P = void> P* at(int64_t off) const { return (P*)(ws + off); }
};

struct ProfScope {
    Prof& p; hipStream_t s; bool on; hipEvent_t b;
    ProfScope(const Ctx& c, int klass, double flops, double bytes, const char* kernel = nullptr);
    ~ProfScope() { if (on) (void)hipEventRecord(b, s); }
};

ProfScope::ProfScope(const Ctx& c, int klass, double flops, double bytes, const char* kernel)
    : p(c.e.prof), s(c.s), on(c.e.prof.on), b(nullptr) {
    if (!on) return;
    static const char* DEF[PC_COUNT] = {"k_conv", "k_wgrad", "k_bn_reduce<T, 0>", "k_bn_act", "k_bn_reduce<T, 1>", "k_bn_bwd_apply",
                                        "k_pool_bwd|k_fuse|k_slice", "k_pack_jobs|k_reduce_dw"};
    ProfRec r;
    r.a = p.get(); r.b = p.get(); r.klass = klass; r.flops = flops; r.bytes = bytes;
    r.name_id = p.intern(kernel ? kernel : DEF[klass]);
    b = r.b;
    p.recs.push_back(r);
    (void)hipEventRecord(r.a, s);
}

static void conv_work(const stcd_engine& e, const stcd_conv_geom& g, int kreal, int nreal, double* flops, double* bytes) {
    double pos = (double)g.n * g.hm * g.wm;
    *flops = 2.0 * pos * g.ntaps * kreal * nreal;
    double in_px = g.in_stride == 1 ? pos : (double)g.n * (2.0 * g.hm) * (2.0 * g.wm);
    *bytes = (in_px * kreal + pos * nreal + (double)g.ntaps * kreal * nreal) * (double)dsize(e.dt);
}

static bool mfma_on(const stcd_engine& e) { return e.dt == BF16 && e.use_mfma; }

struct StatReq { long long* acc = nullptr; int groups = 1; int c0 = 0; int C = 0; float s1 = BN_FS1, s2 = BN_FS2; };

enum class ConvKernel { REF, MFMA, SMALL, RES, TILE, GEMM, HALO, DMA };
constexpr unsigned conv_kernel_bit(ConvKernel k) { return 1u << (int)k; }
struct ConvCall {
    bool nchw = false;
    int stat_groups = 0;
    bool bn_form = false;
    const XfSrc* xf = nullptr;
    bool bwd = false;
    unsigned allowed = ~0u;
};
static int conv_small_groups(const ConvCall& k) {
    return (k.xf && k.xf->on) ? k.xf->groups : (k.stat_groups > 0 && k.bn_form) ? k.stat_groups : 1;
}
static ConvKernel conv_kernel(bool mfma, bool use_small, const ConvOp& op, const ConvCall& k) {
    auto may = [&](ConvKernel x) { return (k.allowed & conv_kernel_bit(x)) != 0; };
    if (conv_on_ref(mfma, op)) return ConvKernel::REF;
    const bool xf_on = k.xf && k.xf->on, stats = k.stat_groups > 0;
    const bool small = op.small && use_small;
    if (k.bwd) return small ? ConvKernel::SMALL : ConvKernel::RES;
    if (op.gemm.ok && !k.nchw) {
        if (op.dma.ok && op.res_groups == 1 && !stats && may(ConvKernel::DMA)) return ConvKernel::DMA;
        if (op.halo.ok && !stats && may(ConvKernel::HALO)) return ConvKernel::HALO;
        return ConvKernel::GEMM;
    }
    if (small && conv_small_call_ok(op.g, conv_small_groups(k), k.xf)) return ConvKernel::SMALL;
    if (op.res.ok && !k.nchw && !small) {
        if (op.tile.ok && !xf_on && may(ConvKernel::TILE)) return ConvKernel::TILE;
        if (!xf_on || conv_res_xf_ok(op.g, op.res, op.res_groups, *k.xf)) return ConvKernel::RES;
    }
    return ConvKernel::MFMA;
}
static void conv_kernel_name(ConvKernel kern, const ConvOp& op, bool bwd, char (&kname)[64]) {
    switch (kern) {
        case ConvKernel::DMA: snprintf(kname, sizeof(kname), "k_conv_dma"); break;
        case ConvKernel::HALO: snprintf(kname, sizeof(kname), "k_conv_halo"); break;
        case ConvKernel::GEMM: snprintf(kname, sizeof(kname), "k_conv_gemm<%d>", op.gemm.W); break;
        case ConvKernel::TILE: snprintf(kname, sizeof(kname), "k_conv_tile<%d>", op.tile.NT); break;
        case ConvKernel::RES:
            if (bwd) snprintf(kname, sizeof(kname), "k_conv_res<bwd>");
            else snprintf(kname, sizeof(kname), "k_conv_res<%d, %d, %s>", op.res.NT, op.res.CW, op.res.single_halo ? "true" : "false");
            break;
// ... 59 lines not shown
        case ConvKernel::TILE:
            rc = launch_conv_tile(op.g, op.plan, op.tile, in, wf, bias, out, op.res_groups, sp, sC, c.s, sc0, s1, s2);
            if (stat_chunks && want) *stat_chunks = 1;
            break;
        case ConvKernel::RES:
            if (bs) {
                rc = launch_conv_res(op.g, op.plan, op.res, in, wf, bias, out, op.res_groups, nullptr, op.g.co, c.s, 0, BN_BS, BN_BS, nullptr, bs);
            } else {
                rc = launch_conv_res(op.g, op.plan, op.res, in, wf, bias, out, op.res_groups, sp, sC, c.s, sc0, s1, s2, xf);
                if (stat_chunks && want) *stat_chunks = 1;
            }
            break;
        case ConvKernel::MFMA:
            rc = launch_conv_mfma(op.g, op.plan, in, wf, bias, out, nchw, c.s);
            break;
        case ConvKernel::REF: {
            const PackSpec& ps = op.dgrad ? cv.dgrad : cv.fwd;
            const float* w = c.at<float>(op.dgrad ? cv.wpk_dgrad : cv.wpk_fwd) + (int64_t)op.tap0 * ps.kpad * ps.wld;
            launch_conv_ref(c.e.dt, op.g, in, w, ps.kpad, ps.wld, bias, out, nchw, c.s);
            break;
        }
    }
    if (rc != 0)
        set_error(bs ? std::string("fused BatchNorm-backward sums: the data-gradient launch of ") + cv.name + " does not fit " + kname
                     : std::string("internal: ") + kname + " rejected the " + (op.dgrad ? "data-gradient" : "forward") + " launch of " +
                           cv.name + " it was chosen for");
}

static bool exec_conv_x4(const Ctx& c, const ConvOp ops[4], const void* in, const float* bias, void* out) {
    if (!mfma_on(c.e)) return false;
    stcd_conv_geom g[4]; ConvMfmaPlan p[4]; const void* wf[4];
    double fl = 0.0, by = 0.0;
    for (int k = 0; k < 4; ++k) {
        if (!ops[k].plan.ok || ops[k].wf < 0) return false;
        g[k] = ops[k].g; p[k] = ops[k].plan; wf[k] = c.at(ops[k].wf);
        double f1, b1;
        conv_work(c.e, ops[k].g, ops[k].kreal, ops[k].nreal, &f1, &b1);
        fl += f1; by += b1;
    }
    if (!conv_mfma_x4_ok(g, p)) return false;
    char kname[64];
    snprintf(kname, sizeof(kname), "k_conv_mfma_x4<%d>", p[0].NT);
    ProfScope prof(c, PC_CONV, fl, by, kname);
    if (launch_conv_mfma_x4(g, p, in, wf, bias, out, c.s) != 0) set_error(std::string("internal: ") + kname + " rejected the launch it was chosen for");
    return true;
}

static void wgroup_member_ready(const Ctx& c, const WgradOp& op);
static void exec_wgrad(const Ctx& c, const WgradOp& op, const void* in, const void* dout) {
    const ConvW& cv = c.e.convs[op.conv];
    PackSpec sub = cv.fwd;
    sub.ntaps = op.g.ntaps;
    for (int t = 0; t < op.g.ntaps; ++t) {
        sub.ky[t] = op.own_taps ? op.oky[t] : cv.fwd.ky[op.tap0 + t];
        sub.kx[t] = op.own_taps ? op.okx[t] : cv.fwd.kx[op.tap0 + t];
    }
    double fl, by;
    conv_work(c.e, op.g, op.kreal, op.nreal, &fl, &by);
    if (mfma_on(c.e) && op.plan.ok && op.grouped) {
        if (c.e.wg_early) wgroup_member_ready(c, op);
        return;
    }
    if (mfma_on(c.e) && op.plan.ok) {
        int rc;
        {
            char kname[64];
            snprintf(kname, sizeof(kname), "k_wgrad_mfma<%d, %d>", op.plan.WCI, op.plan.NTW);
            ProfScope prof(c, PC_WGRAD, fl, by, kname);
            rc = launch_wgrad_mfma(op.g, op.plan, in, dout, c.at<float>(op.slab), sub.kpad, sub.wld, c.s);
        }
        if (rc == 0) return;
    }
    if (op.own_taps) { set_error("internal: no reference fallback for a launch with its own tap table"); return; }
    double* dwe = c.at<double>(cv.dwe) + (int64_t)op.tap0 * sub.kpad * sub.wld;
    if (mfma_on(c.e))
        (void)hipMemsetAsync(dwe, 0, (size_t)sub.ntaps * sub.kpad * sub.wld * 8, c.s);
    {
        ProfScope prof(c, PC_WGRAD, fl, by, "k_wgrad_ref");
        launch_wgrad_ref_f64(c.e.dt, op.g, in, dout, dwe, sub.kpad, sub.wld, c.s);
    }
    launch_unpack_dw(sub, dwe, c.grads + cv.w_off, c.s);
}

static int pack_all_weights(const Ctx& c, bool with_dgrad) {
    stcd_engine& e = c.e;
    if (e.jobs_uploaded_ws != (const void*)c.ws) {
        for (int k = 0; k < 2; ++k) {
            if (!e.jobs[k].empty())
                STCD_HIP(hipMemcpyAsync(c.at(e.jobs_off[k]), e.jobs[k].data(), e.jobs[k].size() * sizeof(PackJob),
                                        hipMemcpyHostToDevice, c.s));
            if (!e.rjobs[k].empty())
                STCD_HIP(hipMemcpyAsync(c.at(e.rjobs_off[k]), e.rjobs[k].data(), e.rjobs[k].size() * sizeof(ReduceJob),
                                        hipMemcpyHostToDevice, c.s));
            for (WgradGroup& G : e.wgroups[k])
                STCD_HIP(hipMemcpyAsync(c.at(G.table_off), G.jobs.data(), G.jobs.size() * sizeof(WgradJob), hipMemcpyHostToDevice, c.s));
        }
        if (!e.bias_jobs.empty())
            STCD_HIP(hipMemcpyAsync(c.at(e.bias_jobs_off), e.bias_jobs.data(), e.bias_jobs.size() * sizeof(BiasJob), hipMemcpyHostToDevice, c.s));
        e.jobs_uploaded_ws = c.ws;
    }
    const int k = with_dgrad ? 1 : 0;
    if (k == 0 && e.weights_tag != 0 && e.weights_tag == e.packed_tag && e.packed_ws == (const void*)c.ws && e.packed_params == (const void*)c.params)
        return 0;
    ProfScope prof(c, PC_PACK, 0.0, 0.0);
    launch_pack_jobs(c.at<PackJob>(e.jobs_off[k]), (int)e.jobs[k].size(), e.jobs_total[k], c.params, c.ws, c.s);
    e.packed_tag = k == 0 ? e.weights_tag : 0; e.packed_ws = c.ws; e.packed_params = c.params; e.packed_level = k;
    return 0;
}

static void launch_wgroup(const Ctx& c, WgradGroup& G) {
    {
        char kname[64];
        if (G.dma) snprintf(kname, sizeof(kname), "k_wgrad_dma");
        else if (G.gemm) snprintf(kname, sizeof(kname), "k_wgrad_gemm<%d>", G.gemm);
        else snprintf(kname, sizeof(kname), "k_wgrad_group<%d, %d, %s>", G.WCI, G.NTW, G.t9 ? "true" : "false");
        ProfScope prof(c, PC_WGRAD, G.flops, G.bytes, kname);
        G.launched = true;
        if (G.dma) {
            launch_wgrad_dma_group(c.at<WgradJob>(G.table_off), (int)G.jobs.size(), G.total_blocks, c.ws, c.s);
            return;
        }
        if (G.gemm) {
            launch_wgrad_gemm_group(G.gemm, c.at<WgradJob>(G.table_off), (int)G.jobs.size(), G.total_blocks, c.ws, c.s);
            return;
        }
        if (launch_wgrad_group(G.WCI, G.NTW, G.t9, c.at<WgradJob>(G.table_off), (int)G.jobs.size(), G.total_blocks, G.lds_bytes,
                               c.ws, c.s, G.xf) != 0)
            set_error("grouped weight-gradient launch exceeds the LDS budget");
    }
}

static void wgroup_member_ready(const Ctx& c, const WgradOp& op) {
    stcd_engine& e = c.e;
    if (op.group < 0 || op.group >= (int)e.wgroups[op.stage].size()) return;
    WgradGroup& G = e.wgroups[op.stage][op.group];
    if (++G.seen < (int)G.jobs.size() || G.launched) return;
    if (e.wg_cur_side) {
        if (hipEventRecord(e.wg_fork, c.s) != hipSuccess || hipStreamWaitEvent(e.wg_cur_side, e.wg_fork, 0) != hipSuccess) { set_error("side-stream fork failed"); return; }
        Ctx cs{e, c.ws, c.params, c.grads, e.wg_cur_side};
        launch_wgroup(cs, G);
    } else {
        launch_wgroup(c, G);
    }
}

static void reduce_stage(const Ctx& c, int stage) {
    stcd_engine& e = c.e;
    for (WgradGroup& G : e.wgroups[stage]) {
        if (!G.launched) launch_wgroup(c, G);
        G.launched = false; G.seen = 0;
    }
    if (e.rjobs[stage].empty()) return;
    ProfScope prof(c, PC_PACK, 0.0, 0.0, "k_reduce_jobs");
    launch_reduce_jobs(c.at<ReduceJob>(e.rjobs_off[stage]), (int)e.rjobs[stage].size(), e.rjobs_total[stage], c.ws, c.grads, c.s);
}

static XfSrc xf_source(const Ctx& c, const Cbrd& P, float* bn_running, bool training) {
    stcd_engine& e = c.e;
    const BnP& bn = e.bns[P.bn];
    XfSrc x;
    x.C = e.convs[P.conv].cout; x.groups = P.groups; x.npg = P.npg; x.ppg = (long long)P.npg * P.H * P.W;
    x.facc = training ? c.at<long long>(P.facc) : nullptr;
    x.gamma = c.params + bn.g_off; x.beta = c.params + bn.b_off;
    x.rmean = bn_running + bn.run_off; x.rvar = bn_running + bn.run_off + x.C;
    x.stat = c.at<float>(P.stat);
    x.mask = (training && e.drop_p > 0.f && P.drop >= 0) ? c.at<float>(e.masks) + e.drops[P.drop].off : nullptr;
    x.publish = training ? 1 : 0;
    x.on = 1;
    return x;
}

static void cbrd_forward(const Ctx& c, const Cbrd& L, float* bn_running, bool training) {
    stcd_engine& e = c.e;
    const ConvW& cv = e.convs[L.conv];
    const BnP& bn = e.bns[L.bn];
    const int C = cv.cout;
    int fused_chunks = 0;
    StatReq sr; sr.acc = training ? c.at<long long>(L.facc) : nullptr; sr.groups = L.groups; sr.C = C;
    XfSrc xf;
    if (L.xsrc) xf = xf_source(c, *L.xsrc, bn_running, training);
    exec_conv(c, L.fwd, c.at(L.in.off), c.params + cv.b_off, c.at(L.Y.off), false, &sr, &fused_chunks, nullptr, nullptr, L.xsrc ? &xf : nullptr);
    const int64_t ppg = (int64_t)L.npg * L.H * L.W;
    const double act_bytes = (double)L.N * L.H * L.W * C * (double)dsize(e.dt);
    float* stat = c.at<float>(L.stat);
    if (training) {
        if (!fused_chunks) {
            ProfScope ps(c, PC_BN_STATS, 0.0, act_bytes);
            launch_bn_stats(e.dt, c.at(L.Y.off), L.Y.ld, C, L.groups, ppg, c.at<long long>(L.facc), c.s);
        }
    }
    if (L.virt) return;
    BnActArgs a;
    a.Y = c.at(L.Y.off); a.ldy = L.Y.ld;
    a.A = skip_recomputed(e, L) ? nullptr : c.at(L.A.off); a.lda = L.A.ld; a.a_group_off = L.A.goff;
    a.P = L.pool ? c.at(L.P.off) : nullptr; a.ldp = L.P.ld;
    a.stat = stat;
    a.mask = (training && e.drop_p > 0.f && L.drop >= 0) ? c.at<float>(e.masks) + e.drops[L.drop].off : nullptr;
    a.C = C; a.groups = L.groups; a.npg = L.npg; a.H = L.H; a.W = L.W; a.relu = 1;
    a.facc = training ? c.at<long long>(L.facc) : nullptr;
    a.gamma = c.params + bn.g_off; a.beta = c.params + bn.b_off;
    a.running_mean = bn_running + bn.run_off; a.running_var = bn_running + bn.run_off + C;
    if (L.fuse_dst.off >= 0 && e.use_act_fuse && L.groups == 2) {
        ProfScope ps(c, PC_BN_ACT, 0.0, act_bytes * (a.A ? 2.75 : 1.75), "k_bn_act_pair");
        launch_bn_act_pair(e.dt, a, c.at(L.fuse_dst.off), L.fuse_dst.ld, e.arch == STCD_ARCH_DIFF ? 0 : 1, c.s);
        return;
    }
    ProfScope ps(c, PC_BN_ACT, 0.0, act_bytes * (L.pool ? 2.25 : 2.0));
    launch_bn_act(e.dt, a, c.s);
}

static BwdSum bwd_sum_of(const Ctx& c, const Cbrd& P) {
    stcd_engine& e = c.e;
    BwdSum b;
    b.Y = c.at(P.Y.off); b.ldy = P.Y.ld; b.stat = c.at<float>(P.stat);
    b.mask = (e.drop_p > 0.f && P.drop >= 0) ? c.at<float>(e.masks) + e.drops[P.drop].off : nullptr;
    b.acc = c.at<long long>(P.bacc); b.groups = P.groups;
    return b;
}

static void cbrd_backward(const Ctx& c, const Cbrd& L, int skip_chunks = 0) {
    stcd_engine& e = c.e;
    const ConvW& cv = e.convs[L.conv];
    const BnP& bn = e.bns[L.bn];
    const int C = cv.cout;
    const int64_t HW = (int64_t)L.H * L.W, ppg = (int64_t)L.npg * HW;
    const float* stat = c.at<float>(L.stat);
    const float* mask = (e.drop_p > 0.f && L.drop >= 0) ? c.at<float>(e.masks) + e.drops[L.drop].off : nullptr;
    long long* bacc = c.at<long long>(L.bacc);
    const double act_bytes = (double)L.N * HW * C * (double)dsize(e.dt);
    (void)ppg;
    if (!skip_chunks && !L.bwd_sums_fused) {
        ProfScope ps(c, PC_BN_BWD_REDUCE, 0.0, 2.0 * act_bytes);
        launch_bn_bwd_reduce(e.dt, c.at(L.dA.off), L.dA.ld, L.dA.goff, c.at(L.Y.off), L.Y.ld, stat, mask, C, L.groups, L.npg, HW, 1,
                             bacc, c.s);
    }
// ... 3 lines not shown
                            c.grads + bn.g_off, c.grads + bn.b_off, mask, C, L.groups, L.npg, HW, 1, c.s);
    }
    exec_wgrad(c, L.wg, c.at(L.in.off), c.at(L.dY.off));
    if (L.has_dIn) {
        StatReq sr;
        if (L.dgr_sum_acc >= 0) { sr.acc = c.at<long long>(L.dgr_sum_acc); sr.groups = 1; sr.c0 = L.dgr_sum_c0; sr.C = L.dgr_sum_C; sr.s1 = sr.s2 = BN_BS; }
        BwdSum bs;
        if (L.dgr_bwd) bs = bwd_sum_of(c, *L.dgr_bwd);
        exec_conv(c, L.dgr, c.at(L.dY.off), nullptr, c.at(L.dIn.off), false, L.dgr_sum_acc >= 0 ? &sr : nullptr, nullptr, nullptr, nullptr, nullptr,
                  L.dgr_bwd ? &bs : nullptr);
    }
}

static void upconv_forward(const Ctx& c, const UpConv& U) {
    stcd_engine& e = c.e;
    const ConvW& cv = e.convs[U.conv];
    if (!exec_conv_x4(c, U.fwd, c.at(U.in.off), c.params + cv.b_off, c.at(U.out.off)))
        for (int ph = 0; ph < 4; ++ph) exec_conv(c, U.fwd[ph], c.at(U.in.off), c.params + cv.b_off, c.at(U.out.off), false);
    launch_rep_pad(e.dt, c.at(U.out.off), U.out.ld, U.N, U.Ho, U.Wo, 2 * U.h, 2 * U.w, U.C, c.s);
}

static void upconv_backward(const Ctx& c, const UpConv& U) {
    stcd_engine& e = c.e;
    const ConvW& cv = e.convs[U.conv];
    launch_rep_pad_bwd(e.dt, c.at(U.dOut.off), U.dOut.ld, U.N, U.Ho, U.Wo, 2 * U.h, 2 * U.w, U.C, c.s);
    if (U.bias_fused && mfma_on(e)) {
    } else if (2 * U.h == U.Ho && 2 * U.w == U.Wo) {
        launch_bias_grad(e.dt, c.at(U.dOut.off), U.dOut.ld, (int64_t)U.N * U.Ho * U.Wo, U.C, c.grads + cv.b_off, c.s,
                         e.dt == BF16 ? c.at<long long>(U.bias_acc) : nullptr);
    } else {
        const int64_t T = (int64_t)dsize(e.dt);
        for (int n = 0; n < U.N; ++n)
            for (int y = 0; y < 2 * U.h; ++y)
                launch_bias_grad(e.dt, c.at<char>(U.dOut.off) + ((int64_t)(n * U.Ho + y) * U.Wo) * U.dOut.ld * T, U.dOut.ld,
                                 2 * U.w, U.C, c.grads + cv.b_off, c.s, e.dt == BF16 ? c.at<long long>(U.bias_acc) : nullptr);
    }
    for (int ph = 0; ph < 4; ++ph) exec_wgrad(c, U.wg[ph], c.at(U.in.off), c.at(U.dOut.off));
    exec_conv(c, U.dgr, c.at(U.dOut.off), nullptr, c.at(U.dIn.off), false);
}

static void xconc_forward(const Ctx& c, const XConc& X, const Cbrd& skip, float* bn_running, bool training) {
    stcd_engine& e = c.e;
    const BnP& bn = e.bns[X.bn1];
    const int C = X.C, B = X.res.N, h = X.res.H, w = X.res.W;
    {
        ProfScope ps(c, PC_POOL_FUSE, 0.0, 3.0 * B * h * w * C * (double)dsize(e.dt), "k_pairdw_fwd");
        launch_pairdw_fwd(e.dt, c.at(skip.A.off), skip.A.ld, skip.A.goff, c.at(X.G.off), X.G.ld, c.params + X.w_off, c.params + X.b_off, B, h, w, C, c.s);
    }
    if (training) launch_bn_stats(e.dt, c.at(X.G.off), X.G.ld, C, 1, (int64_t)B * h * w, c.at<long long>(X.facc1), c.s);
    BnActArgs a;
    a.Y = c.at(X.G.off); a.ldy = X.G.ld;
    a.A = c.at(X.R.off); a.lda = X.R.ld; a.a_group_off = 0;
    a.P = nullptr; a.ldp = 0;
    a.stat = c.at<float>(X.stat1);
    a.mask = nullptr;
    a.C = C; a.groups = 1; a.npg = B; a.H = h; a.W = w; a.relu = 1;
    a.facc = training ? c.at<long long>(X.facc1) : nullptr;
    a.gamma = c.params + bn.g_off; a.beta = c.params + bn.b_off;
    a.running_mean = bn_running + bn.run_off; a.running_var = bn_running + bn.run_off + C;
    launch_bn_act(e.dt, a, c.s);
    cbrd_forward(c, X.res, bn_running, training);
}
static void xconc_backward(const Ctx& c, const XConc& X, const Cbrd& skip) {
    stcd_engine& e = c.e;
    const BnP& bn = e.bns[X.bn1];
    const int C = X.C, B = X.res.N, h = X.res.H, w = X.res.W;
    const int64_t HW = (int64_t)h * w;
    cbrd_backward(c, X.res);
    launch_bn_bwd_reduce(e.dt, c.at(X.dR.off), X.dR.ld, 0, c.at(X.G.off), X.G.ld, c.at<float>(X.stat1), nullptr, C, 1, B, HW, 1,
                         c.at<long long>(X.bacc1), c.s);
    launch_bn_bwd_apply(e.dt, c.at(X.dR.off), X.dR.ld, 0, c.at(X.dG.off), X.dG.ld, c.at(X.G.off), X.G.ld, c.at<float>(X.stat1),
                        c.at<long long>(X.bacc1), c.grads + bn.g_off, c.grads + bn.b_off, nullptr, C, 1, B, HW, 1, c.s);
    ProfScope ps(c, PC_POOL_FUSE, 0.0, 6.0 * B * h * w * C * (double)dsize(e.dt), "k_pairdw_bwd");
    launch_pairdw_bwd_data(e.dt, c.at(X.dG.off), X.dG.ld, c.at(skip.dA.off), skip.dA.ld, skip.dA.goff, c.params + X.w_off, B, h, w, C, c.s);
    launch_pairdw_bwd_filter(e.dt, c.at(skip.A.off), skip.A.ld, skip.A.goff, c.at(X.dG.off), X.dG.ld, c.grads + X.w_off, c.at<float>(X.part),
                             B, h, w, C, c.s);
}

static int forward_fcsiam(stcd_engine& e, const float* x1, const float* x2, const float* params, float* bn_running,
                          const float* masks, uint64_t seed, int training, float* logits, void* workspace, hipStream_t s) {
    Ctx c{e, (char*)workspace, params, nullptr, s};
    const int B = e.B, dt = e.dt;
    const int64_t T = (int64_t)dsize(dt);
    if (training && e.drop_p > 0.f) {
        if (masks) STCD_HIP(hipMemcpyAsync(c.at(e.masks), masks, e.drop_floats * 4, hipMemcpyDeviceToDevice, s));
        else launch_dropout_gen(c.at<float>(e.masks), e.drop_floats, seed, e.drop_p, s);
    } else if (training && e.fc_virt_layers > 0) {
        launch_dropout_gen(c.at<float>(e.masks), e.drop_floats, seed, 0.f, s);
    }
    if (pack_all_weights(c, training != 0)) return 1;
    if (training) STCD_HIP(hipMemsetAsync(c.at(e.zero_begin), 0, e.zero_end - e.zero_begin, s));
    launch_in_pack(dt, x1, x2, c.at(e.X0.off), B, e.in_ch, e.H, e.W, s, e.arch == STCD_ARCH_FCEF ? 0 : 2);
    for (auto& L : e.enc) cbrd_forward(c, L, bn_running, training != 0);
    size_t di = 0;
    for (int k = 0; k < 4; ++k) {
        const UpConv& U = e.ups[k];
        const int s_ = U.level, C = ENC_C[s_];
        upconv_forward(c, U);
        const Cbrd& skip = e.enc[SKIP_IDX[s_]];
        if (fc_cross(e)) xconc_forward(c, e.xc[s_], skip, bn_running, training != 0);
        else if (!fc_concat_skips(e) && !(e.use_act_fuse && skip.fuse_dst.off >= 0)) {
            ProfScope ps(c, PC_POOL_FUSE, 0.0, 3.0 * B * e.Hs[s_] * e.Ws[s_] * C * (double)T);
            launch_fuse(dt, e.arch == STCD_ARCH_DIFF ? 0 : 1, c.at(skip.A.off), skip.A.ld, skip.A.goff,
                        c.at<char>(e.D[s_].off) + C * T, e.D[s_].ld, B, (int64_t)e.Hs[s_] * e.Ws[s_], C, s);
        }
        for (int j = 0; j < DEC[k].n; ++j) {
            if (DEC[k].cout[j] < 0) break;
            cbrd_forward(c, e.dec[di++], bn_running, training != 0);
        }
    }
    {
        XfSrc xf;
        if (e.final_xsrc) xf = xf_source(c, *e.final_xsrc, bn_running, training != 0);
        exec_conv(c, e.final_fwd, c.at(e.finalIn.off), params + e.convs[e.final_conv].b_off, logits, true, nullptr, nullptr, nullptr, nullptr,
                  e.final_xsrc ? &xf : nullptr);
    }
    STCD_HIP(hipGetLastError());
    return 0;
}

static hipStream_t wgrad_side_stream(stcd_engine& e, hipStream_t s) {
    if (!e.wg_side_on || !e.use_wgroup || !mfma_on(e)) return nullptr;
    if (e.prof.on) return nullptr;
    hipStreamCaptureStatus cap = hipStreamCaptureStatusNone;
    if (hipStreamIsCapturing(s, &cap) != hipSuccess) { (void)hipGetLastError(); return nullptr; }
    if (cap != hipStreamCaptureStatusNone) return nullptr;
    int dev = 0;
    if (hipGetDevice(&dev) != hipSuccess) { (void)hipGetLastError(); return nullptr; }
    if (e.wg_side && e.wg_side_dev == dev) return e.wg_side;
    if (e.wg_side) return nullptr;
    int prio_lo = 0, prio_hi = 0;
    (void)hipDeviceGetStreamPriorityRange(&prio_lo, &prio_hi);
    hipStream_t st = nullptr;
    if (hipStreamCreateWithPriority(&st, hipStreamNonBlocking, prio_lo) != hipSuccess) { (void)hipGetLastError(); e.wg_side_on = 0; return nullptr; }
    if (hipEventCreateWithFlags(&e.wg_fork, hipEventDisableTiming) != hipSuccess || hipEventCreateWithFlags(&e.wg_join, hipEventDisableTiming) != hipSuccess) {
        (void)hipGetLastError(); (void)hipStreamDestroy(st); e.wg_side_on = 0; return nullptr;
    }
    e.wg_side = st; e.wg_side_dev = dev;
    return st;
}

static void finish_biases(const Ctx& c) {
    launch_bias_finish(c.at<BiasJob>(c.e.bias_jobs_off), (int)c.e.bias_jobs.size(), c.ws, c.grads, c.s);
}

template <typename Extra>
static int stage_tail(const Ctx& c, int stage, hipStream_t side, bool wait_join, Extra extra) {
    stcd_engine& e = c.e;
    if (!side) { reduce_stage(c, stage); extra(c); return 0; }
    STCD_HIP(hipEventRecord(e.wg_fork, c.s));
    STCD_HIP(hipStreamWaitEvent(side, e.wg_fork, 0));
    Ctx cs{e, c.ws, c.params, c.grads, side};
    reduce_stage(cs, stage);
    extra(cs);
    STCD_HIP(hipEventRecord(e.wg_join, side));
    if (wait_join) STCD_HIP(hipStreamWaitEvent(c.s, e.wg_join, 0));
    return 0;
}

struct EarlyScope {
    stcd_engine& e;
    EarlyScope(stcd_engine& e_, bool on, hipStream_t sd) : e(e_) { e.wg_early = on; e.wg_cur_side = sd; }
    ~EarlyScope() { e.wg_early = false; e.wg_cur_side = nullptr; }
};

static int backward_fcsiam(stcd_engine& e, const float* grad_logits, const float* params, float* grads, void* workspace,
                           int stage, hipStream_t s) {
    Ctx c{e, (char*)workspace, params, grads, s};
    hipStream_t side = stage < 0 ? wgrad_side_stream(e, s) : nullptr;
    EarlyScope early_scope(e, mfma_on(e) && e.use_wgroup, side);
    for (int st = 0; st < 2; ++st)
        if (stage < 0 || stage == st)
            for (WgradGroup& G : e.wgroups[st]) { G.seen = 0; G.launched = false; }
    const int B = e.B, dt = e.dt;
    const int64_t T = (int64_t)dsize(dt);
    if (stage <= 0) {
        STCD_HIP(hipMemsetAsync(grads, 0, e.param_floats * 4, s));
        if (!mfma_on(e)) STCD_HIP(hipMemsetAsync(c.at(e.dwe_begin), 0, e.dwe_end - e.dwe_begin, s));
        launch_gout_pack(dt, grad_logits, c.at(e.G.off), B, e.label, e.H, e.W, s, c.at<long long>(e.final_bias_acc));
        exec_wgrad(c, e.final_wg, c.at(e.finalIn.off), c.at(e.G.off));
        {
            BwdSum bs;
            if (e.final_dgr_bwd) bs = bwd_sum_of(c, *e.final_dgr_bwd);
            exec_conv(c, e.final_dgr, c.at(e.G.off), nullptr, c.at(e.dFinalIn.off), false, nullptr, nullptr, nullptr, nullptr, nullptr,
                      e.final_dgr_bwd ? &bs : nullptr);
        }
        int di = (int)e.dec.size() - 1;
        for (int k = 3; k >= 0; --k) {
            int nb = 0;
            for (int j = 0; j < DEC[k].n; ++j) nb += DEC[k].cout[j] >= 0;
            for (int j = 0; j < nb; ++j) cbrd_backward(c, e.dec[di--]);
            const UpConv& U = e.ups[k];
            const int s_ = U.level, C = ENC_C[s_];
            upconv_backward(c, U);
            const Cbrd& skip = e.enc[SKIP_IDX[s_]];
            if (fc_cross(e)) xconc_backward(c, e.xc[s_], skip);
            else if (!fc_concat_skips(e) && !e.use_skip_fused) {
                ProfScope ps(c, PC_POOL_FUSE, 0.0, (e.arch == STCD_ARCH_DIFF ? 5.0 : 3.0) * B * e.Hs[s_] * e.Ws[s_] * C * (double)T);
                launch_fuse_bwd(dt, e.arch == STCD_ARCH_DIFF ? 0 : 1, c.at(skip.A.off), skip.A.ld, skip.A.goff,
                                c.at<char>(e.dD[s_].off) + C * T, e.dD[s_].ld, c.at(skip.dA.off), skip.dA.ld, skip.dA.goff, B,
                                (int64_t)e.Hs[s_] * e.Ws[s_], C, s);
            }
        }
        if (stage_tail(c, 0, side, false, finish_biases)) return 1;
    }
    if (stage < 0 || stage == 1) {
        for (int li = (int)e.enc.size() - 1; li >= 0; --li) {
            const Cbrd& L = e.enc[li];
            int skip_chunks = 0;
            if (L.pool && !fc_concat_skips(e) && !fc_cross(e) && e.use_skip_fused) {
                const int C = e.convs[L.conv].cout;
                int lvl = 0;
                while (lvl < 4 && SKIP_IDX[lvl] != li) ++lvl;
                const float* mk = e.drop_p > 0.f ? c.at<float>(e.masks) + e.drops[L.drop].off : nullptr;
                if (skip_recomputed(e, L)) {
                    ProfScope ps(c, PC_POOL_FUSE, 0.0, 2.75 * L.N * L.H * L.W * C * (double)T, "k_skip_bwd_pair");
                    launch_skip_bwd_pair(dt, e.arch == STCD_ARCH_DIFF ? 0 : 1, c.at(L.Y.off), L.Y.ld, c.at<char>(e.dD[lvl].off) + C * T,
                                         e.dD[lvl].ld, c.at(L.dPool.off), L.dPool.ld, c.at(L.dA.off), L.dA.ld, L.dA.goff,
                                         c.at<float>(L.stat), mk, L.npg, L.H, L.W, C, c.at<long long>(L.bacc), s);
                } else {
                ProfScope ps(c, PC_POOL_FUSE, 0.0, 4.75 * L.N * L.H * L.W * C * (double)T, "k_skip_bwd");
                launch_skip_bwd(dt, e.arch == STCD_ARCH_DIFF ? 0 : 1, c.at(L.A.off), L.A.ld, L.A.goff, c.at(L.Y.off), L.Y.ld,
                                c.at<char>(e.dD[lvl].off) + C * T, e.dD[lvl].ld, c.at(L.dPool.off), L.dPool.ld, c.at(L.dA.off), L.dA.ld,
                                L.dA.goff, c.at<float>(L.stat), e.drop_p > 0.f ? c.at<float>(e.masks) + e.drops[L.drop].off : nullptr,
                                L.npg, L.H, L.W, C, c.at<long long>(L.bacc), s);
                }
                skip_chunks = 1;
            } else if (L.pool) {
                const int C = e.convs[L.conv].cout;
                ProfScope ps(c, PC_POOL_FUSE, 0.0, 3.25 * L.N * L.H * L.W * C * (double)T);
                launch_pool_bwd(dt, c.at(L.A.off), L.A.ld, L.A.goff, c.at(L.dPool.off), L.dPool.ld, c.at(L.dA.off), L.dA.ld,
                                L.dA.goff, L.groups, L.npg, L.H, L.W, C, 1, s);
            }
            cbrd_backward(c, L, skip_chunks);
        }
        if (stage_tail(c, 1, side, true, [](const Ctx&) {})) return 1;
    }
    STCD_HIP(hipGetLastError());
    return 0;
}

static const int SN_F[5] = {32, 64, 128, 256, 512};

static int add_block_params(stcd_engine& e, const std::string& name, int cin, int c, int calls, bool need_dgrad1, NBlock* b) {
    b->name = name; b->Cin = cin; b->C = c;
    b->c1 = add_conv(e, name + ".conv1", K_CONV3, cin, c, need_dgrad1);
    b->bn1 = add_bn(e, name + ".bn1", c, calls);
    b->c2 = add_conv(e, name + ".conv2", K_CONV3, c, c, true);
    b->bn2 = add_bn(e, name + ".bn2", c, calls);
    return 0;
}

static void build_snunet_tables(stcd_engine& e) {
    const int* f = SN_F;
    e.sn_blocks.clear(); e.sn_ups.clear();
    auto blk = [&](const std::string& n, int cin, int c, int calls, bool dg) {
        NBlock b; add_block_params(e, n, cin, c, calls, dg, &b); e.sn_blocks.push_back(b);
    };
    auto up = [&](const std::string& n, int c) {
        SnUp u; u.C = c; u.conv = add_conv(e, n + ".up", K_CONVT2, c, c, true); e.sn_ups.push_back(u);
    };
    blk("conv0_0", e.in_ch, f[0], 2, false);
// ... 1026 lines not shown
    if (stage == 1) return 0;
    Ctx c{e, (char*)workspace, params, grads, s};
    const int B = e.B, dt = e.dt;
    const int64_t T = (int64_t)dsize(dt), HW = (int64_t)e.H * e.W;
    STCD_HIP(hipMemsetAsync(grads, 0, e.param_floats * 4, s));
    if (!mfma_on(e)) STCD_HIP(hipMemsetAsync(c.at(e.dwe_begin), 0, e.dwe_end - e.dwe_begin, s));
    if (e.seg_dates == 1 || e.bres) {
        launch_gout_pack(dt, grad_logits, c.at(e.G.off), B, e.label, e.H, e.W, s, c.at<long long>(e.final_bias_acc));
        exec_wgrad(c, e.g_head_wg, c.at(e.gX3.off), c.at(e.G.off));
        exec_conv(c, e.g_head_dgr, c.at(e.G.off), nullptr, c.at(e.gdX3.off), false);
    } else {
        launch_segcd_combine_bwd(c.at<float>(e.g_raw3), grad_logits, c.at<float>(e.g_draw3), (int64_t)B * e.label * HW, s);
        launch_gout_pack(dt, c.at<float>(e.g_draw3), c.at(e.G.off), 3 * B, e.label, e.H, e.W, s, c.at<long long>(e.final_bias_acc));
        exec_wgrad(c, e.g_head_wg, c.at(e.gX3.off), c.at(e.G.off));
        exec_conv(c, e.g_head_dgr, c.at(e.G.off), nullptr, c.at(e.gdX3.off), false);
        if (!e.seg_ffc) launch_fuse_bwd(dt, 0, c.at(e.gX3.off), 16, (int64_t)B * HW * 16, c.at<char>(e.gdX3.off) + (int64_t)2 * B * HW * 16 * T, 16,
                        c.at(e.gFuseTmp.off), 16, (int64_t)B * HW * 16, B, HW, 16, s);
    }
    for (int k = (int)e.g_fwd.size() - 1; k >= 0; --k) {
        const GStep& st = e.g_fwd[k];
        if (st.kind == GS_LAYER) glayer_backward(c, e.g_layers[st.layer]);
        else if (st.kind == GS_UPSAMPLE)
            launch_upsample2_bwd(dt, c.at(st.ddst.off), st.ddst.ld, c.at(st.dsrc.off), st.dsrc.ld, st.N, st.h, st.w, st.C, s);
        else if (st.kind == GS_ABSDIFF) {
            const int64_t hw = (int64_t)st.h * st.w;
            launch_fuse_bwd(dt, 0, c.at(st.src.off), st.src.ld, (int64_t)st.N * hw * st.src.ld,
                            c.at<char>(st.dsrc.off) + (int64_t)2 * st.N * hw * st.dsrc.ld * T, st.dsrc.ld,
                            c.at(st.ddst.off), st.ddst.ld, (int64_t)st.N * hw * st.ddst.ld, st.N, hw, st.C, s);
        }
        else if (st.kind == GS_TOKENDEC) {
            auto& b = e.bit;
            const int n = st.h * st.w;
            const double rows = (double)st.N * n;
            {
                ProfScope ps(c, PC_POOL_FUSE, 3.0 * 12288.0 * b.L * rows, rows * 32 * ((b.L + 2.0) * (double)T + 8.0 * (b.L - 1)), "k_bit_dec_bwd");
                if (launch_bit_dec_bwd(dt, c.at(st.src.off), c.at(b.xs), c.at(st.ddst.off), c.at<float>(b.dG), c.at(st.dsrc.off), c.at<float>(b.AP),
                                       params + b.dec_off, c.at<float>(b.dec_part), n, st.N, b.L, b.dh, s)) return 1;
            }
            ProfScope ps(c, PC_POOL_FUSE, 2.0 * b.L * st.N * 6.0 * 8 * b.dh * 32 * 4, 4.0 * (double)bit_dec_part_floats(n, st.N, b.L), "k_bit_sum_parts|k_bit_dec_unfold|k_bit_dec_mfinish");
            launch_bit_dec_finish(c.at<float>(b.dec_part), c.at<float>(b.dAP), c.at<float>(b.tok_out), params + b.dec_off, grads + b.dec_off,
                                  c.at<float>(b.dmh), c.at<float>(b.dm), c.at<float>(b.dtok_out), n, st.N, b.L, b.dh, s);
        } else if (st.kind == GS_TOKENENC) {
            auto& b = e.bit;
            ProfScope ps(c, PC_POOL_FUSE, 6.0 * B * 8 * (4.0 * 512 * 32 + 2.0 * 32 * 64), 4.0 * (double)bit_enc_part_floats(B, 64) * 2, "k_bit_enc<true>");
            launch_bit_enc_bwd(c.at<float>(b.tok_in), params + b.pos_off, params + b.enc_off, c.at<float>(b.dtok_out), c.at<float>(b.dtok_in),
                               c.at<float>(b.enc_part), grads + b.enc_off, grads + b.pos_off, B, 64, s);
        } else if (st.kind == GS_TOKENIZE) {
            auto& b = e.bit;
            ProfScope ps(c, PC_POOL_FUSE, 48.0 * 32 * st.N * st.h * st.w, 4.0 * st.N * st.h * st.w * 32 * (double)T, "k_bit_tok_bwd");
            launch_bit_tok_bwd(dt, c.at(st.src.off), params + b.wa_off, c.at<float>(b.stat), c.at<float>(b.dtok_in), c.at(b.dec_din.off),
                               c.at(st.dsrc.off), c.at<float>(b.tok_part), grads + b.wa_off, st.N, st.h * st.w, s);
        }
        else if (st.kind == GS_BILINEAR) {
            ProfScope ps(c, PC_POOL_FUSE, 0.0, 17.0 * st.N * st.h * st.w * st.C * (double)T, "k_bilinear_bwd");
            launch_bilinear_bwd(dt, c.at(st.ddst.off), st.ddst.ld, c.at(st.dsrc.off), st.dsrc.ld, st.N, st.h, st.w, 4 * st.h, 4 * st.w, st.C, 0, s);
        } else if (st.kind == GS_ABSPAIR) {
            const int64_t hw = (int64_t)st.h * st.w;
            ProfScope ps(c, PC_POOL_FUSE, 0.0, 5.0 * st.N * hw * st.C * (double)T, "k_fuse_bwd");
            launch_fuse_bwd(dt, 0, c.at(st.src.off), st.src.ld, (int64_t)st.N * hw * st.src.ld, c.at(st.ddst.off), st.ddst.ld,
                            c.at(st.dsrc.off), st.dsrc.ld, (int64_t)st.N * hw * st.dsrc.ld, st.N, hw, st.C, s);
        } else if (st.kind == GS_BCONV) {
            { ProfScope ps(c, PC_POOL_FUSE, 0.0, (double)st.N * st.h * st.w * 32 * (double)T, "k_bias_grad");
            launch_bias_grad(dt, c.at(st.ddst.off), st.ddst.ld, (int64_t)st.N * st.h * st.w, 32, grads + e.convs[e.g_pred_conv].b_off, s,
                             dt == BF16 ? c.at<long long>(e.g_pred_bias_acc) : nullptr); }
            exec_wgrad(c, e.g_pred_wg, c.at(st.src.off), c.at(st.ddst.off));
            exec_conv(c, e.g_pred_dgr, c.at(st.ddst.off), nullptr, c.at(st.dsrc.off), false);
        }
        else {
            launch_slice(dt, c.at(st.ddst.off), st.ddst.ld, c.at(e.g_pool_idc.off), e.g_pool_idc.ld, (int64_t)st.N * (st.h / 2) * (st.w / 2), st.C, 1, s);
            launch_maxpool3_bwd(dt, c.at<unsigned char>(e.g_pool_idx), c.at(st.ddst.off), st.ddst.ld, c.at(st.dsrc.off), st.dsrc.ld, st.N, st.h, st.w, st.C, s);
        }
    }
    reduce_stage(c, 0);
    launch_bias_finish(c.at<BiasJob>(e.bias_jobs_off), (int)e.bias_jobs.size(), c.ws, c.grads, s);
    STCD_HIP(hipGetLastError());
    return 0;
}

#include "engine_cf.inl"

static void reset_plan(stcd_engine& e) {
    e.enc.clear(); e.dec.clear(); e.ups.clear();
    e.drops.clear(); e.drop_floats = 0;
    e.conv_ops.clear(); e.wgrad_ops.clear(); e.slab_floats = 0;
    e.ws_tensors.clear(); e.bias_jobs.clear();
    e.g_fwd.clear(); e.sn_order.clear();
    if (e.cf) cf_reset_plan(*e.cf);
}

}

extern "C" {

const char* stcd_last_error(void) { return stcd::g_err.c_str(); }
int stcd_abi_version(void) { return STCD_ABI_VERSION; }

static void engine_env_switches(stcd_engine* e) {
    e->use_mfma = !env_flag("STCD_FORCE_REF_KERNELS", false);
    e->use_small = !env_flag("STCD_NO_SMALL_KERNEL", false);
    e->use_gemm = !env_flag("STCD_NO_GEMM_KERNEL", false);
    e->use_res = !env_flag("STCD_NO_RES_KERNEL", false);
    e->use_halo = env_flag("STCD_HALO_KERNEL", false);
    e->use_tile = !env_flag("STCD_NO_TILE_KERNEL", false);
    e->use_wgroup = !env_flag("STCD_NO_WGRAD_GROUPS", false);
    e->use_act_fuse = !env_flag("STCD_NO_ACT_FUSE", false);
    e->use_skip_fused = !env_flag("STCD_NO_SKIP_FUSED", false);
    e->use_skip_recompute = !env_flag("STCD_NO_SKIP_RECOMPUTE", false);
    e->use_bwdsum = !env_flag("STCD_NO_BWDSUM_FUSE", false);
    e->use_bwdsum_res = env_flag("STCD_BWDSUM_RES", false);
    e->use_virt = env_int("STCD_VIRT_ACT", e->use_virt) != 0;
    e->wg_side_on = env_int("STCD_WGRAD_SIDE", e->wg_side_on) != 0;
}

int stcd_cf_default_config(stcd_cf_config* cfg) {
    STCD_CHECK(cfg != nullptr, "cfg is null");
    static const int E[4] = {64, 128, 320, 512}, DP[4] = {3, 3, 4, 3}, HD[4] = {1, 2, 4, 8}, SR[4] = {8, 4, 2, 1};
    memset(cfg, 0, sizeof(*cfg));
    cfg->in_ch = 3; cfg->out_ch = 2;
    for (int i = 0; i < 4; ++i) { cfg->embed_dims[i] = E[i]; cfg->depths[i] = DP[i]; cfg->num_heads[i] = HD[i]; cfg->sr_ratios[i] = SR[i]; }
    cfg->mlp_ratio = 4; cfg->embedding_dim = 256; cfg->patch1 = 7; cfg->patch = 7;
    cfg->drop_rate = 0.1f; cfg->attn_drop = 0.1f; cfg->drop_path_rate = 0.1f; cfg->diff_drop = 0.6f;
    return 0;
}

int stcd_create_changeformer(const stcd_cf_config* cfg, int dtype, stcd_engine** out) {
    STCD_CHECK(out != nullptr && cfg != nullptr, "null argument");
    STCD_CHECK(cfg->in_ch >= 1 && cfg->in_ch <= 8, "in_ch must be in [1,8]");
    STCD_CHECK(cfg->out_ch >= 1 && cfg->out_ch <= 8, "out_ch must be in [1,8]");
    STCD_CHECK(dtype == STCD_DTYPE_F32 || dtype == STCD_DTYPE_BF16, "unknown dtype");
    STCD_CHECK(cfg->mlp_ratio >= 1 && cfg->embedding_dim >= 8 && cfg->embedding_dim % 8 == 0, "embedding_dim must be a positive multiple of 8");
    STCD_CHECK((cfg->embedding_dim & (cfg->embedding_dim - 1)) == 0, "embedding_dim must be a power of two (BatchNorm kernels)");
    STCD_CHECK((cfg->patch1 & 1) && (cfg->patch & 1) && cfg->patch1 >= 3 && cfg->patch >= 3, "patch sizes must be odd and >= 3");
    for (int i = 0; i < 4; ++i) {
        STCD_CHECK(cfg->embed_dims[i] >= 8 && cfg->embed_dims[i] % 8 == 0 && cfg->embed_dims[i] <= 1024, "embed_dims must be multiples of 8, <= 1024");
        STCD_CHECK(cfg->depths[i] >= 1 && cfg->num_heads[i] >= 1 && cfg->sr_ratios[i] >= 1, "depths, num_heads and sr_ratios must be >= 1");
        STCD_CHECK(cfg->embed_dims[i] % cfg->num_heads[i] == 0, "embed_dims must be divisible by num_heads");
    }
    for (float p : {cfg->drop_rate, cfg->attn_drop, cfg->drop_path_rate, cfg->diff_drop}) STCD_CHECK(p >= 0.f && p < 1.f, "drop rates must be in [0,1)");
    std::unique_ptr<stcd_engine> e(new stcd_engine());
    e->arch = STCD_ARCH_CHANGEFORMER; e->in_ch = cfg->in_ch; e->label = cfg->out_ch; e->dt = dtype;
    engine_env_switches(e.get());
    e->cf = std::make_shared<CfPlan>();
    CfPlan& P = *e->cf;
    for (int i = 0; i < 4; ++i) { P.E[i] = cfg->embed_dims[i]; P.depths[i] = cfg->depths[i]; P.heads[i] = cfg->num_heads[i]; P.srs[i] = cfg->sr_ratios[i]; }
    P.mlp_ratio = cfg->mlp_ratio; P.D = cfg->embedding_dim; P.patch1 = cfg->patch1; P.patch = cfg->patch;
    P.drop = cfg->drop_rate; P.attn_drop = cfg->attn_drop; P.drop_path = cfg->drop_path_rate; P.diff_drop = cfg->diff_drop;
    build_cf_tables(*e);
    *out = e.release();
    return 0;
}

int stcd_cf_num_sites(const stcd_engine* e) { return e && e->cf && e->configured ? (int)e->cf->sites.size() : 0; }
int stcd_cf_site_get(const stcd_engine* e, int i, stcd_cf_site* out) {
    STCD_CHECK(e && e->cf && e->configured && out && i >= 0 && i < (int)e->cf->sites.size(), "bad argument");
    memset(out, 0, sizeof(*out));
    const CfPlan::Site& s = e->cf->sites[i];
    snprintf(out->name, sizeof(out->name), "%s", s.name.c_str());
    out->ndim = s.nd;
    for (int k = 0; k < s.nd; ++k) out->dims[k] = s.dims[k];
    out->p = s.p;
    return 0;
}
uint32_t stcd_cf_site_seed(uint64_t seed, int site) { return cf_site_seed(seed, site); }
int stcd_cf_set_aux_backward(stcd_engine* e, int on) {
    STCD_CHECK(e && e->cf, "not a ChangeFormer engine");
    if (e->cf->aux_bwd != (on != 0)) e->configured = false;
    e->cf->aux_bwd = on != 0;
// ... 86 lines not shown
        STCD_CHECK(height % 32 == 0 && width % 32 == 0, "ChangeFormer needs height and width divisible by 32 (stride-4 patch embedding, sr_ratio 8)");
        if (configure_cf(*e, batch, height, width)) return 1;
    } else if (is_snunet(e->arch)) {
        STCD_CHECK(height % 16 == 0 && width % 16 == 0, "SNUNet needs height and width divisible by 16 (the reference's cat of up-sampled maps fails otherwise)");
        if (configure_snunet(*e, batch, height, width)) return 1;
    } else if (is_segcd(e->arch)) {
        STCD_CHECK(!is_bres(e->arch) || (height % 32 == 0 && width % 32 == 0), "base_resnet needs height and width divisible by 32 (the engine's rule: 1/8-resolution trunk, row tiles of 4 pixels at that level)");
        STCD_CHECK(height % 32 == 0 && width % 32 == 0, "SegCD needs height and width divisible by 32 (five stride-2 stages; the reference's cat of the x2 up-sampled maps fails otherwise)");
        STCD_CHECK((int64_t)3 * batch * height * width * 16 < ((int64_t)1 << 31), "tensor too large for 32-bit pixel indexing");
        if (configure_segcd(*e, batch, height, width)) return 1;
    } else if (configure_fcsiam(*e, batch, height, width)) return 1;
    e->min_bn_count = INT64_MAX;
    for (const auto& L : e->enc) e->min_bn_count = std::min<int64_t>(e->min_bn_count, (int64_t)L.npg * L.H * L.W);
    for (const auto& L : e->dec) e->min_bn_count = std::min<int64_t>(e->min_bn_count, (int64_t)L.npg * L.H * L.W);
    for (const auto& b : e->sn_blocks) e->min_bn_count = std::min<int64_t>(e->min_bn_count, (int64_t)b.npg * b.H * b.W);
    for (const auto& L : e->g_layers) e->min_bn_count = std::min<int64_t>(e->min_bn_count, (int64_t)L.npg * L.Ho * L.Wo);
    if (e->cf) e->min_bn_count = std::min<int64_t>(e->min_bn_count, (int64_t)batch * (height / 32) * (width / 32));
    e->configured = true;
    e->fwd_training = false;
    return 0;
}
int64_t stcd_workspace_bytes(const stcd_engine* e) { return e && e->configured ? e->ws_bytes : 0; }
int stcd_num_dropout(const stcd_engine* e) { return e && e->configured ? (int)e->drops.size() : 0; }
int stcd_dropout_info_get(const stcd_engine* e, int i, stcd_dropout_info* info) {
    STCD_CHECK(e && e->configured && info && i >= 0 && i < (int)e->drops.size(), "bad argument");
    memset(info, 0, sizeof(*info));
    snprintf(info->name, sizeof(info->name), "%s", e->drops[i].name.c_str());
    info->rows = e->drops[i].rows;
    info->channels = e->drops[i].C;
    info->offset = e->drops[i].off;
    return 0;
}
int64_t stcd_dropout_floats(const stcd_engine* e) { return e && e->configured ? e->drop_floats : 0; }
int stcd_set_dropout_p(stcd_engine* e, float p) {
    STCD_CHECK(e != nullptr, "engine is null");
    STCD_CHECK(p >= 0.f && p < 1.f, "p must be in [0,1)");
    e->drop_p = p;
    return 0;
}

int stcd_forward(stcd_engine* e, const float* x1, const float* x2, const float* params, float* bn_running,
                 const float* dropout_masks, uint64_t dropout_seed, int training, float* logits, void* workspace,
                 void* hip_stream) {
    STCD_CHECK(e && e->configured, "engine not configured");
    STCD_CHECK(x1 && x2 && params && bn_running && logits && workspace, "null pointer argument");
    STCD_CHECK(!(training && e->min_bn_count <= 1), "Expected more than 1 value per channel when training: a BatchNorm layer of this network sees "
               "one value per channel at this batch / image size (torch.nn.BatchNorm2d raises the same)");
    e->fwd_training = false;
    int rc = is_cf(e->arch)
                 ? forward_cf(*e, x1, x2, params, bn_running, dropout_masks, dropout_seed, training, logits, workspace, (hipStream_t)hip_stream)
             : is_snunet(e->arch)
                 ? forward_snunet(*e, x1, x2, params, bn_running, training, logits, workspace, (hipStream_t)hip_stream)
                 : is_segcd(e->arch)
                       ? forward_segcd(*e, x1, x2, params, bn_running, training, logits, workspace, (hipStream_t)hip_stream)
                       : forward_fcsiam(*e, x1, x2, params, bn_running, dropout_masks, dropout_seed, training, logits, workspace,
                                        (hipStream_t)hip_stream);
    if (rc == 0) e->fwd_training = training != 0;
    return rc;
}

int stcd_backward(stcd_engine* e, const float* grad_logits, const float* params, float* grads, void* workspace, int stage,
                  void* hip_stream) {
    STCD_CHECK(e && e->configured, "engine not configured");
    STCD_CHECK(e->fwd_training, "backward requires a preceding training-mode forward on this engine that no backward has consumed "
               "(one backward per forward: it overwrites the stored activations in place)");
    STCD_CHECK(grad_logits && params && grads && workspace, "null pointer argument");
    STCD_CHECK(stage >= -1 && stage <= 1, "stage must be -1, 0 or 1");
    if (stage != 0) e->fwd_training = false;
    if (is_cf(e->arch)) return backward_cf(*e, grad_logits, params, grads, workspace, stage, (hipStream_t)hip_stream);
    if (is_snunet(e->arch)) return backward_snunet(*e, grad_logits, params, grads, workspace, stage, (hipStream_t)hip_stream);
    if (is_segcd(e->arch)) return backward_segcd(*e, grad_logits, params, grads, workspace, stage, (hipStream_t)hip_stream);
    return backward_fcsiam(*e, grad_logits, params, grads, workspace, stage, (hipStream_t)hip_stream);
}

int stcd_set_weights_tag(stcd_engine* e, uint64_t tag) {
    STCD_CHECK(e != nullptr, "engine is null");
    e->weights_tag = tag;
    return 0;
}
int stcd_set_debug(stcd_engine* e, int flags) {
    STCD_CHECK(e != nullptr, "engine is null");
    e->debug_flags = flags;
    e->configured = false;
    return 0;
}
int stcd_ws_tensor_count(const stcd_engine* e) { return e ? (int)e->ws_tensors.size() : 0; }
int stcd_ws_tensor_get(const stcd_engine* e, int index, stcd_ws_tensor* out) {
    STCD_CHECK(e != nullptr && out != nullptr, "null argument");
    STCD_CHECK(index >= 0 && index < (int)e->ws_tensors.size(), "tensor index out of range");
    *out = e->ws_tensors[index];
    return 0;
}

int stcd_grad_stage_range(const stcd_engine* e, int stage, int64_t* begin, int64_t* end) {
    STCD_CHECK(e && begin && end, "bad argument");
    STCD_CHECK(stage == 0 || stage == 1, "stage must be 0 or 1");
    if (stage == 0) { *begin = e->enc_param_end; *end = e->param_floats; }
    else { *begin = 0; *end = e->enc_param_end; }
    return 0;
}

int stcd_profile_enable(stcd_engine* e, int on) {
    STCD_CHECK(e != nullptr, "engine is null");
    e->prof.on = on != 0;
    e->prof.recs.clear();
    e->prof.names.clear();
    e->prof.used = 0;
    return 0;
}
int stcd_profile_read(stcd_engine* e, int klass, double* total_ms, int64_t* launches, double* flops, double* bytes) {
    STCD_CHECK(e && total_ms && launches && flops && bytes, "bad argument");
    STCD_CHECK(klass >= 0 && klass < PC_COUNT, "unknown kernel class");
    *total_ms = 0.0; *launches = 0; *flops = 0.0; *bytes = 0.0;
    for (auto& r : e->prof.recs) {
        if (r.klass != klass) continue;
        STCD_HIP(hipEventSynchronize(r.b));
        float ms = 0.f;
        STCD_HIP(hipEventElapsedTime(&ms, r.a, r.b));
        *total_ms += ms; *launches += 1; *flops += r.flops; *bytes += r.bytes;
    }
    return 0;
}

int stcd_profile_num_kernels(const stcd_engine* e) { return e ? (int)e->prof.names.size() : 0; }
int stcd_profile_kernel(stcd_engine* e, int i, char* name, int name_cap, double* total_ms, int64_t* launches, double* flops,
                        double* bytes) {
    STCD_CHECK(e && name && total_ms && launches && flops && bytes && name_cap > 0, "bad argument");
    STCD_CHECK(i >= 0 && i < (int)e->prof.names.size(), "kernel index out of range");
    snprintf(name, (size_t)name_cap, "%s", e->prof.names[i].c_str());
    *total_ms = 0.0; *launches = 0; *flops = 0.0; *bytes = 0.0;
    for (auto& r : e->prof.recs) {
        if (r.name_id != i) continue;
        STCD_HIP(hipEventSynchronize(r.b));
        float ms = 0.f;
        STCD_HIP(hipEventElapsedTime(&ms, r.a, r.b));
        *total_ms += ms; *launches += 1; *flops += r.flops; *bytes += r.bytes;
    }
    return 0;
}

int64_t stcd_loss_scratch_bytes(void) { return loss_scratch_bytes(); }
int stcd_loss_ce(const float* logits, const int64_t* target, int batch, int classes, int64_t hw, int ignore_index,
                 float* loss_out, float* dlogits, void* scratch, void* hip_stream) {
    STCD_CHECK(logits && target && loss_out && scratch, "null pointer argument");
    STCD_CHECK(batch >= 1 && classes >= 2 && classes <= 16 && hw >= 1, "bad shape");
    launch_loss_ce(logits, target, batch, classes, hw, ignore_index, loss_out, dlogits, scratch, (hipStream_t)hip_stream);
    STCD_HIP(hipGetLastError());
    return 0;
}
int stcd_loss_bce_dice(const float* logits, const float* target, int64_t numel, int from_logits, float* loss_out,
                       float* dlogits, void* scratch, void* hip_stream) {
    STCD_CHECK(logits && target && loss_out && scratch, "null pointer argument");
    STCD_CHECK(numel >= 1, "bad shape");
    launch_loss_bce_dice(logits, target, numel, from_logits, loss_out, dlogits, scratch, (hipStream_t)hip_stream);
    STCD_HIP(hipGetLastError());
    return 0;
}
int stcd_loss_contrastive(const float* pred, const int64_t* cd_label, const int64_t* pse_label, int64_t numel_half, float* loss_out,
                          float* dpred, void* scratch, void* hip_stream) {
    STCD_CHECK(pred && cd_label && pse_label && loss_out && scratch, "null pointer argument");
    STCD_CHECK(numel_half >= 1, "bad shape");
    launch_loss_contrastive(pred, cd_label, pse_label, numel_half, loss_out, dpred, scratch, (hipStream_t)hip_stream);
    STCD_HIP(hipGetLastError());
    return 0;
}
int64_t stcd_loss_iou_scratch_bytes(int batch, int classes, int64_t hw) {
// ... 349 lines not shown
```

stcd_amd/csrc/kernels_conv_mfma.hip:

```cpp
#include "common.h"

namespace stcd {

typedef __attribute__((ext_vector_type(8))) __bf16 bf16x8;
typedef __attribute__((ext_vector_type(4))) float f32x4;
typedef __attribute__((ext_vector_type(4))) unsigned u32x4;

struct ConvMfmaArgs {
    stcd_conv_geom g;
    const bf16* in;
    const bf16* wf;
    const float* bias;
    void* out;
    int out_nchw;
    int CiB, nchunks, KS;
    int modeB;
    int NTtot;
    int dymin, dxmin, HH, HWp, swmask;
    int tiles_x, tiles_y;
    int halo_bytes, wbuf_bytes;
    int tap[9];
};

static inline void fill_taps(const stcd_conv_geom& g, int* tap) {
// ... 177 lines not shown
    }
}

template <int NT>
__global__ void __launch_bounds__(256, 2)
k_conv_mfma(const ConvMfmaArgs a) {
    conv_mfma_body<NT>(a, blockIdx.x, blockIdx.y);
}

struct ConvMfmaArgs4 { ConvMfmaArgs a[4]; };
template <int NT>
__global__ void __launch_bounds__(256, 2)
k_conv_mfma_x4(const ConvMfmaArgs4 j) {
    conv_mfma_body<NT>(j.a[blockIdx.z], blockIdx.x, blockIdx.y);
}

static void taps_extent(const stcd_conv_geom& g, int* dymin, int* dymax, int* dxmin, int* dxmax) {
    *dymin = *dxmin = 127; *dymax = *dxmax = -127;
    for (int t = 0; t < g.ntaps; ++t) {
        *dymin = std::min<int>(*dymin, g.dy[t]); *dymax = std::max<int>(*dymax, g.dy[t]);
        *dxmin = std::min<int>(*dxmin, g.dx[t]); *dxmax = std::max<int>(*dxmax, g.dx[t]);
    }
}

static size_t conv_mfma_lds(const stcd_conv_geom& g, const ConvMfmaPlan& p) {
    int dymin, dymax, dxmin, dxmax;
    taps_extent(g, &dymin, &dymax, &dxmin, &dxmax);
    const int HH = 7 * g.in_stride + (dymax - dymin) + 1, HWp = 15 * g.in_stride + (dxmax - dxmin) + 1;
    const int halo_bytes = (HH * HWp * p.CiB * 2 + 255) & ~255;
    const int wbuf_bytes = p.modeB ? ((p.KS * p.NT * 1024 + 1) / 2 + 255) & ~255 : (p.KS * p.NT * 1024 + 255) & ~255;
    return (size_t)halo_bytes + 2 * (size_t)wbuf_bytes + 128;
}

ConvMfmaPlan conv_mfma_plan(const stcd_conv_geom& g) {
    ConvMfmaPlan p;
    const int Ci = g.ci;
    if (Ci % 64 == 0) p.CiB = 64;
    else if (Ci % 32 == 0) p.CiB = 32;
    else p.CiB = Ci;
    p.modeB = (p.CiB % 32) != 0;
    p.nchunks = Ci / p.CiB;
    p.KS = p.modeB ? (g.ntaps * Ci + 31) / 32 : p.CiB / 32;
    p.NTtot = (g.co + 15) / 16;
    p.NT = p.NTtot >= 8 ? 8 : p.NTtot >= 4 ? 4 : p.NTtot >= 2 ? 2 : 1;
    {
        const int64_t tiles = (int64_t)g.n * ((g.hm + 7) / 8) * ((g.wm + 15) / 16);
        while (p.NT > 1 && tiles * ((p.NTtot + p.NT - 1) / p.NT) < 512) p.NT /= 2;
    }
    p.NTtot = ((p.NTtot + p.NT - 1) / p.NT) * p.NT;
    p.wf_elems = p.modeB ? (int64_t)p.KS * p.NTtot * 512 : (int64_t)p.nchunks * g.ntaps * p.KS * p.NTtot * 512;
    p.ok = (Ci % 8 == 0) && (p.modeB ? (Ci <= 64 && p.KS <= 24) : true) && g.ldi % 8 == 0 && conv_mfma_lds(g, p) <= 160 * 1024;
    return p;
}

__global__ void k_pack_frag(const float* __restrict__ w, int kpad, int wld, int ntaps, int Ci, int Co, int CiB, int nchunks,
                            int KS, int NTtot, int modeB, bf16* __restrict__ dst, int64_t total) {
    int64_t i = (int64_t)blockIdx.x * blockDim.x + threadIdx.x;
    if (i >= total) return;
    const int j = (int)(i & 7), lane = (int)((i >> 3) & 63);
    int64_t f = i >> 9;
    const int nt = (int)(f % NTtot); f /= NTtot;
    const int ks = (int)(f % KS); f /= KS;
    const int co = nt * 16 + (lane & 15);
    int t, ci;
    if (modeB) {
        const int kf = ks * 32 + 8 * (lane >> 4) + j;
        t = kf / Ci; ci = kf - t * Ci;
    } else {
        t = (int)(f % ntaps);
        const int cc = (int)(f / ntaps);
        ci = cc * CiB + ks * 32 + 8 * (lane >> 4) + j;
    }
    float v = 0.f;
    if (t < ntaps && ci < Ci && co < Co) v = w[((int64_t)t * kpad + ci) * wld + co];
    dst[i] = (bf16)v;
}

__device__ __forceinline__ float ref_weight(const PackSpec& ps, const float* src, int t, int k, int n) {
    if (n >= ps.N || k >= ps.K) return 0.f;
    const int64_t a_ = ps.kn_major ? ((int64_t)k * ps.N + n) : ((int64_t)n * ps.K + k);
    return src[(a_ * ps.ks + ps.ky[t]) * ps.ks + ps.kx[t]];
}

__global__ void __launch_bounds__(256)
k_pack_jobs(const PackJob* __restrict__ jobs, int njobs, int64_t total, const float* __restrict__ params, char* __restrict__ ws) {
    const int64_t i0 = (int64_t)blockIdx.x * blockDim.x, i = i0 + threadIdx.x;
    int lo = 0, hi = njobs - 1;
    while (lo < hi) {
        const int mid = (lo + hi + 1) >> 1;
        if (jobs[mid].start <= i0) lo = mid; else hi = mid - 1;
    }
    const PackJob& jb = jobs[lo];
    const int64_t e = i - jb.start;
    if (e >= jb.count) return;
    const float* src = params + jb.src_off;
    if (jb.kind == 0) {
        const int n = (int)(e % jb.ps.wld);
        const int k = (int)((e / jb.ps.wld) % jb.ps.kpad);
        const int t = (int)(e / ((int64_t)jb.ps.wld * jb.ps.kpad));
        reinterpret_cast<float*>(ws + jb.dst_off)[e] = ref_weight(jb.ps, src, t, k, n);
    } else if (jb.kind == 2) {
        const int j = (int)(e & 7), lane = (int)((e >> 3) & 63);
        int64_t f = e >> 9;
        const int nt = (int)(f % jb.NTtot); f /= jb.NTtot;
        const int ks = (int)(f % 2); f /= 2;
        const int ky = (int)f, co = nt * 16 + (lane & 15);
        const int k = ks * 32 + 8 * (lane >> 4) + j, kx = k >> 3, c = k & 7;
        float v = 0.f;
        if (ky < 7 && kx < 7 && c < jb.aux && co < jb.Co) v = src[(((int64_t)co * jb.aux + c) * 7 + ky) * 7 + kx];
        reinterpret_cast<bf16*>(ws + jb.dst_off)[e] = (bf16)v;
    } else if (!jb.modeB) {
        const int j = (int)(e & 7), lane = (int)((e >> 3) & 63);
        int64_t f = e >> 9;
        const int nt = (int)(f % jb.NTtot); f /= jb.NTtot;
        const int ks = (int)(f % jb.KS);
        const int cc = (int)(f / jb.KS);
        const int co = nt * 16 + (lane & 15), ci = cc * jb.CiB + ks * 32 + 8 * (lane >> 4) + j;
        const bool in = ci < jb.Ci && co < jb.Co;
        bf16* dst = reinterpret_cast<bf16*>(ws + jb.dst_off) + (((int64_t)cc * jb.ps.ntaps * jb.KS + ks) * jb.NTtot + nt) * 512 + (e & 511);
        const int64_t tstride = (int64_t)jb.KS * jb.NTtot * 512;
        for (int t = 0; t < jb.ps.ntaps; ++t) dst[t * tstride] = (bf16)(in ? ref_weight(jb.ps, src, t, ci, co) : 0.f);
    } else {
        const int j = (int)(e & 7), lane = (int)((e >> 3) & 63);
        int64_t f = e >> 9;
        const int nt = (int)(f % jb.NTtot); f /= jb.NTtot;
        const int ks = (int)(f % jb.KS); f /= jb.KS;
        const int co = nt * 16 + (lane & 15);
        int t, ci;
        if (jb.modeB) {
            const int kf = ks * 32 + 8 * (lane >> 4) + j;
            t = kf / jb.Ci; ci = kf - t * jb.Ci;
        } else {
            t = (int)(f % jb.ps.ntaps);
            ci = (int)(f / jb.ps.ntaps) * jb.CiB + ks * 32 + 8 * (lane >> 4) + j;
        }
        float v = 0.f;
        if (t < jb.ps.ntaps && ci < jb.Ci && co < jb.Co) v = ref_weight(jb.ps, src, t, ci, co);
        reinterpret_cast<bf16*>(ws + jb.dst_off)[e] = (bf16)v;
    }
}
void launch_pack_jobs(const PackJob* jobs_dev, int njobs, int64_t total, const float* params, char* ws, hipStream_t s) {
    if (njobs > 0 && total > 0) k_pack_jobs<<<(unsigned)((total + 255) / 256), 256, 0, s>>>(jobs_dev, njobs, total, params, ws);
}

void launch_pack_frag(const stcd_conv_geom& g, const ConvMfmaPlan& p, const float* w, int kpad, int wld, void* dst,
                      hipStream_t s) {
    k_pack_frag<<<(unsigned)((p.wf_elems + 255) / 256), 256, 0, s>>>(w, kpad, wld, g.ntaps, g.ci, g.co, p.CiB, p.nchunks, p.KS,
                                                                      p.NTtot, p.modeB, (bf16*)dst, p.wf_elems);
}

static size_t conv_mfma_args(const stcd_conv_geom& g, const ConvMfmaPlan& p, const void* in, const void* wf, const float* bias,
                             void* out, bool out_nchw, ConvMfmaArgs& a) {
    a.g = g;
    a.in = (const bf16*)in; a.wf = (const bf16*)wf; a.bias = bias; a.out = out; a.out_nchw = out_nchw ? 1 : 0;
    a.CiB = p.CiB; a.nchunks = p.nchunks; a.KS = p.KS; a.modeB = p.modeB; a.NTtot = p.NTtot;
    int dymax, dxmax;
    taps_extent(g, &a.dymin, &dymax, &a.dxmin, &dxmax);
    a.HH = 7 * g.in_stride + (dymax - a.dymin) + 1;
    a.HWp = 15 * g.in_stride + (dxmax - a.dxmin) + 1;
    const int nch8 = p.CiB / 8;
    a.swmask = (nch8 & (nch8 - 1)) == 0 ? nch8 - 1 : 0;
    a.tiles_x = (g.wm + 15) / 16;
    a.tiles_y = (g.hm + 7) / 8;
    a.halo_bytes = (a.HH * a.HWp * p.CiB * 2 + 255) & ~255;
    a.wbuf_bytes = p.modeB ? ((p.KS * p.NT * 1024 + 1) / 2 + 255) & ~255 : (p.KS * p.NT * 1024 + 255) & ~255;
    fill_taps(g, a.tap);
    return conv_mfma_lds(g, p);
}

int launch_conv_mfma(const stcd_conv_geom& g, const ConvMfmaPlan& p, const void* in, const void* wf, const float* bias,
                     void* out, bool out_nchw, hipStream_t s) {
    ConvMfmaArgs a;
    const size_t lds = conv_mfma_args(g, p, in, wf, bias, out, out_nchw, a);
    if (lds > 160 * 1024) return 1;
    dim3 grid((unsigned)(a.tiles_x * a.tiles_y * g.n), (unsigned)(p.NTtot / p.NT));
#define LAUNCH_NT(N_)                                                                                             \
    do {                                                                                                          \
        static bool attr_set = false;                                                                             \
        if (!attr_set) {                                                                                          \
            (void)hipFuncSetAttribute((const void*)k_conv_mfma<N_>, hipFuncAttributeMaxDynamicSharedMemorySize, 160 * 1024); \
            attr_set = true;                                                                                      \
        }                                                                                                         \
        k_conv_mfma<N_><<<grid, 256, lds, s>>>(a);                                                                \
    } while (0)
    switch (p.NT) {
        case 1: LAUNCH_NT(1); break;
        case 2: LAUNCH_NT(2); break;
        case 4: LAUNCH_NT(4); break;
        default: LAUNCH_NT(8); break;
    }
#undef LAUNCH_NT
    return 0;
}

bool conv_mfma_x4_ok(const stcd_conv_geom g[4], const ConvMfmaPlan p[4]) {
    for (int k = 0; k < 4; ++k)
        if (!p[k].ok || p[k].NT != p[0].NT || p[k].NTtot != p[0].NTtot || g[k].n != g[0].n || g[k].hm != g[0].hm || g[k].wm != g[0].wm)
            return false;
    return true;
}
int launch_conv_mfma_x4(const stcd_conv_geom g[4], const ConvMfmaPlan p[4], const void* in, const void* const wf[4],
                        const float* bias, void* out, hipStream_t s) {
    if (!conv_mfma_x4_ok(g, p)) return 1;
    ConvMfmaArgs4 j;
    size_t lds = 0;
    for (int k = 0; k < 4; ++k) lds = std::max(lds, conv_mfma_args(g[k], p[k], in, wf[k], bias, out, false, j.a[k]));
    if (lds > 160 * 1024) return 1;
    dim3 grid((unsigned)(j.a[0].tiles_x * j.a[0].tiles_y * g[0].n), (unsigned)(p[0].NTtot / p[0].NT), 4);
#define LAUNCH_X4(N_)                                                                                             \
    do {                                                                                                          \
        static bool attr_set = false;                                                                             \
        if (!attr_set) {                                                                                          \
            (void)hipFuncSetAttribute((const void*)k_conv_mfma_x4<N_>, hipFuncAttributeMaxDynamicSharedMemorySize, 160 * 1024); \
            attr_set = true;                                                                                      \
        }                                                                                                         \
        k_conv_mfma_x4<N_><<<grid, 256, lds, s>>>(j);                                                             \
    } while (0)
    switch (p[0].NT) {
        case 1: LAUNCH_X4(1); break;
        case 2: LAUNCH_X4(2); break;
        case 4: LAUNCH_X4(4); break;
        default: LAUNCH_X4(8); break;
    }
#undef LAUNCH_X4
    return 0;
// ... 1889 lines not shown
```

stcd_amd/csrc/kernels_ew.hip:

```cpp
#include <cstdlib>

#include "common.h"

namespace stcd {

__device__ __forceinline__ void ld8f(const float* p, float (&v)[8]) {
    float4 a = *reinterpret_cast<const float4*>(p), b = *reinterpret_cast<const float4*>(p + 4);
    v[0] = a.x; v[1] = a.y; v[2] = a.z; v[3] = a.w; v[4] = b.x; v[5] = b.y; v[6] = b.z; v[7] = b.w;
}


template <typename T> struct Raw8;
template <> struct Raw8<bf16> {
    uint4 v;
    __device__ __forceinline__ void opaque() { asm volatile("" : "+v"(v.x), "+v"(v.y), "+v"(v.z), "+v"(v.w)); }
    __device__ __forceinline__ void ld(const bf16* p) { v = *reinterpret_cast<const uint4*>(p); }
    __device__ __forceinline__ void get(float (&o)[8]) const {
        const uint32_t w[4] = {v.x, v.y, v.z, v.w};
#pragma unroll
        for (int i = 0; i < 4; ++i) { o[2 * i] = __uint_as_float(w[i] << 16); o[2 * i + 1] = __uint_as_float(w[i] & 0xffff0000u); }
    }
};
template <> struct Raw8<float> {
    float4 a, b;
    __device__ __forceinline__ void opaque() {}
    __device__ __forceinline__ void ld(const float* p) { a = *reinterpret_cast<const float4*>(p); b = *reinterpret_cast<const float4*>(p + 4); }
    __device__ __forceinline__ void get(float (&o)[8]) const { o[0] = a.x; o[1] = a.y; o[2] = a.z; o[3] = a.w; o[4] = b.x; o[5] = b.y; o[6] = b.z; o[7] = b.w; }
};

template <typename T, int V> struct RawV;
template <typename T> struct RawV<T, 8> : Raw8<T> {};
template <> struct RawV<bf16, 4> {
    uint2 v;
    __device__ __forceinline__ void opaque() { asm volatile("" : "+v"(v.x), "+v"(v.y)); }
    __device__ __forceinline__ void ld(const bf16* p) { v = *reinterpret_cast<const uint2*>(p); }
    __device__ __forceinline__ void get(float (&o)[4]) const {
        o[0] = __uint_as_float(v.x << 16); o[1] = __uint_as_float(v.x & 0xffff0000u);
        o[2] = __uint_as_float(v.y << 16); o[3] = __uint_as_float(v.y & 0xffff0000u);
    }
};
template <> struct RawV<float, 4> {
    float4 a;
    __device__ __forceinline__ void opaque() {}
    __device__ __forceinline__ void ld(const float* p) { a = *reinterpret_cast<const float4*>(p); }
    __device__ __forceinline__ void get(float (&o)[4]) const { o[0] = a.x; o[1] = a.y; o[2] = a.z; o[3] = a.w; }
};
template <int V> __device__ __forceinline__ void ldVf(const float* p, float (&v)[V]) {
#pragma unroll
    for (int i = 0; i < V / 4; ++i) {
        const float4 a = *reinterpret_cast<const float4*>(p + 4 * i);
        v[4 * i] = a.x; v[4 * i + 1] = a.y; v[4 * i + 2] = a.z; v[4 * i + 3] = a.w;
    }
}
template <typename T, int V> __device__ __forceinline__ void storeV(T* p, const float (&v)[V]);
template <> __device__ __forceinline__ void storeV<bf16, 8>(bf16* p, const float (&v)[8]) { store8<bf16>(p, v); }
template <> __device__ __forceinline__ void storeV<float, 8>(float* p, const float (&v)[8]) { store8<float>(p, v); }
template <> __device__ __forceinline__ void storeV<bf16, 4>(bf16* p, const float (&v)[4]) {
    *reinterpret_cast<uint2*>(p) = make_uint2(pack_bf16x2(v[0], v[1]), pack_bf16x2(v[2], v[3]));
}
template <> __device__ __forceinline__ void storeV<float, 4>(float* p, const float (&v)[4]) {
    *reinterpret_cast<float4*>(p) = make_float4(v[0], v[1], v[2], v[3]);
}

static inline int cdiv(int64_t a, int64_t b) { return (int)((a + b - 1) / b); }
static inline int ew_grid(int64_t total_threads) { return (int)std::min<int64_t>(cdiv(total_threads, 256), 2048); }
static inline int bn_slabs(int C) {
    constexpr int min_c = 128;
    return (C >= min_c && C % 64 == 0) ? C / 64 : 1;
}

struct GV {
    int ld;
    int64_t goff;
};

template <typename T>
__global__ void k_in_pack(const float* __restrict__ x1, const float* __restrict__ x2, T* __restrict__ X, int B, int cin,
                          int64_t HW, int64_t total, int concat) {
    int64_t i = (int64_t)blockIdx.x * blockDim.x + threadIdx.x;
    if (i >= total) return;
    int n = (int)(i / HW);
    int64_t p = i - (int64_t)n * HW;
    float v[8];
    if (concat) {
        const float* s1 = x1 + (int64_t)n * cin * HW + p;
        const float* s2 = x2 + (int64_t)n * cin * HW + p;
#pragma unroll
        for (int c = 0; c < 8; ++c) v[c] = c < cin ? s1[(int64_t)c * HW] : c < 2 * cin ? s2[(int64_t)(c - cin) * HW] : 0.f;
    } else {
        const float* src = (n < B ? x1 + (int64_t)n * cin * HW : x2 + (int64_t)(n - B) * cin * HW) + p;
#pragma unroll
        for (int c = 0; c < 8; ++c) v[c] = c < cin ? src[(int64_t)c * HW] : 0.f;
    }
    store8<T>(X + i * 8, v);
}

void launch_in_pack(int dt, const float* x1, const float* x2, void* X, int B, int cin, int H, int W, hipStream_t s, int dates) {
    const int concat = dates == 0 ? 1 : 0;
    int64_t HW = (int64_t)H * W, n = (int64_t)(concat ? 1 : dates) * B * HW;
    if (dt == BF16) k_in_pack<bf16><<<cdiv(n, 256), 256, 0, s>>>(x1, x2, (bf16*)X, B, cin, HW, n, concat);
    else k_in_pack<float><<<cdiv(n, 256), 256, 0, s>>>(x1, x2, (float*)X, B, cin, HW, n, concat);
}

template <typename T>
__global__ void __launch_bounds__(256)
k_gout_pack(const float* __restrict__ g, T* __restrict__ G, int B, int L, int64_t HW, long long* __restrict__ bias_acc) {
    __shared__ float red[4][8];
    int64_t i = (int64_t)blockIdx.x * blockDim.x + threadIdx.x;
    float v[8];
#pragma unroll
    for (int c = 0; c < 8; ++c) v[c] = 0.f;
    if (i < (int64_t)B * HW) {
        int n = (int)(i / HW);
        int64_t p = i - (int64_t)n * HW;
#pragma unroll
        for (int c = 0; c < 8; ++c) v[c] = c < L ? g[((int64_t)n * L + c) * HW + p] : 0.f;
        store8<T>(G + i * 8, v);
    }
    if (bias_acc) {
#pragma unroll
        for (int c = 0; c < 8; ++c) {
            const float t_ = wave_sum(v[c]);
            if ((threadIdx.x & 63) == 0) red[threadIdx.x >> 6][c] = t_;
        }
        __syncthreads();
        if ((int)threadIdx.x < L)
            bn_acc_add(bias_acc, blockIdx.x, 1, 8, 0, 0, threadIdx.x,
                       (red[0][threadIdx.x] + red[1][threadIdx.x]) + (red[2][threadIdx.x] + red[3][threadIdx.x]), BN_BS);
    }
}

void launch_gout_pack(int dt, const float* g, void* G, int B, int L, int H, int W, hipStream_t s, long long* bias_acc) {
    int64_t HW = (int64_t)H * W, n = (int64_t)B * HW;
    if (dt == BF16) k_gout_pack<bf16><<<cdiv(n, 256), 256, 0, s>>>(g, (bf16*)G, B, L, HW, bias_acc);
    else k_gout_pack<float><<<cdiv(n, 256), 256, 0, s>>>(g, (float*)G, B, L, HW, bias_acc);
}

__global__ void k_bias_finish(const BiasJob* __restrict__ jobs, const char* __restrict__ ws, float* __restrict__ grads) {
    const BiasJob& jb = jobs[blockIdx.x];
    const long long* acc = reinterpret_cast<const long long*>(ws + jb.acc_off);
    for (int c = threadIdx.x; c < jb.valid; c += blockDim.x) grads[jb.out_off + c] = (float)bn_acc_get(acc, 1, jb.C, 0, 0, c, jb.scale);
}
void launch_bias_finish(const BiasJob* jobs_dev, int njobs, const char* ws, float* grads, hipStream_t s) {
    if (njobs > 0) k_bias_finish<<<njobs, 128, 0, s>>>(jobs_dev, ws, grads);
}

__global__ void k_pack_w(PackSpec ps, const float* __restrict__ src, float* __restrict__ dst) {
    int64_t i = (int64_t)blockIdx.x * blockDim.x + threadIdx.x;
    int64_t total = (int64_t)ps.ntaps * ps.kpad * ps.wld;
    if (i >= total) return;
    int n = (int)(i % ps.wld);
    int k = (int)((i / ps.wld) % ps.kpad);
    int t = (int)(i / ((int64_t)ps.wld * ps.kpad));
    float v = 0.f;
    if (n < ps.N && k < ps.K) {
        int64_t a = ps.kn_major ? ((int64_t)k * ps.N + n) : ((int64_t)n * ps.K + k);
        v = src[(a * ps.ks + ps.ky[t]) * ps.ks + ps.kx[t]];
    }
    dst[i] = v;
}
void launch_pack_w(const PackSpec& ps, const float* src, float* dst, hipStream_t s) {
    int64_t total = (int64_t)ps.ntaps * ps.kpad * ps.wld;
    k_pack_w<<<cdiv(total, 256), 256, 0, s>>>(ps, src, dst);
}
__global__ void k_unpack_dw(PackSpec ps, const double* __restrict__ dwe, float* __restrict__ gsrc) {
    int64_t i = (int64_t)blockIdx.x * blockDim.x + threadIdx.x;
    int64_t total = (int64_t)ps.ntaps * ps.K * ps.N;
    if (i >= total) return;
    int n = (int)(i % ps.N);
    int k = (int)((i / ps.N) % ps.K);
    int t = (int)(i / ((int64_t)ps.N * ps.K));
    int64_t a = ps.kn_major ? ((int64_t)k * ps.N + n) : ((int64_t)n * ps.K + k);
    gsrc[(a * ps.ks + ps.ky[t]) * ps.ks + ps.kx[t]] = (float)dwe[((int64_t)t * ps.kpad + k) * ps.wld + n];
}
void launch_unpack_dw(const PackSpec& ps, const double* dwe, float* gsrc, hipStream_t s) {
    int64_t total = (int64_t)ps.ntaps * ps.K * ps.N;
    k_unpack_dw<<<cdiv(total, 256), 256, 0, s>>>(ps, dwe, gsrc);
}

template <int V>
__device__ __forceinline__ int block_reduce2(const float (&s1)[V], const float (&s2)[V], const int cb, float* __restrict__ red) {
#pragma unroll
    for (int j = 0; j < V; ++j) { red[threadIdx.x * 2 * V + j] = s1[j]; red[threadIdx.x * 2 * V + V + j] = s2[j]; }
    return 256 / cb;
}
template <int V>
__device__ __forceinline__ float block_reduce2_get(const float* __restrict__ red, const int n, const int cb, const int which, const int c) {
    float a = 0.f;
    for (int l = 0; l < n; ++l) a += red[(l * cb + c / V) * 2 * V + which * V + (c % V)];
    return a;
}
__device__ __forceinline__ int block_reduce16(const float (&s1)[8], const float (&s2)[8], const int cb, float* __restrict__ red) {
    return block_reduce2<8>(s1, s2, cb, red);
}
__device__ __forceinline__ float block_reduce16_get(const float* __restrict__ red, const int n, const int cb, const int which, const int c) {
    return block_reduce2_get<8>(red, n, cb, which, c);
}

int bn_stats_chunks(int64_t ppg, int C) {
    constexpr int per = 2048;
    int64_t c = ppg * (C / 8) / per;
    if (c < 1) c = 1;
    if (c > 1024) c = 1024;
    return (int)c;
}

template <typename T, int MODE, int NS = 0, bool RES = false, bool MASK = false>
__global__ void __launch_bounds__(256)
k_bn_reduce(const T* __restrict__ Y, int ldy, const T* __restrict__ dA, GV dav, const float* __restrict__ stat,
            const float* __restrict__ mask, const T* __restrict__ res, int ldres, int C, int npg, int64_t HW, int relu,
            int64_t ppg, int nchunk, long long* __restrict__ acc, const SliceViews xs, int base_valid, T* __restrict__ dA_sum,
            int nslab) {
    __shared__ float red[256 * 16];
    const int CS = C / nslab, slab = blockIdx.x % nslab, cbase = slab * CS;
    const int g = blockIdx.y, chunk = blockIdx.x / nslab;
    const int cb = CS >> 3;
    const int lanes = 256 / cb;
    const int mycb = threadIdx.x % cb, lane = threadIdx.x / cb;
// ... 719 lines not shown
        if constexpr (OPT == 2) load8<T>(extra + (p0 + k) * ldex + c0, ex[k]);
    }
#pragma unroll
    for (int k = 0; k < PX; ++k) {
        float o[8], dzv[8];
#pragma unroll
        for (int j = 0; j < 8; ++j) {
            float dz = MASK ? d[k][j] * mk[j] : d[k][j];
            float z = y[k][j] * sc[j] + sh[j];
            if constexpr (OPT == 1) z += rs[k][j];
            if (relu && !(z > 0.f)) dz = 0.f;
            dzv[j] = dz;
            o[j] = sc[j] * dz + kb[j] * (y[k][j] - mu[j]) + kc[j];
            if constexpr (OPT == 2) o[j] += ex[k][j];
        }
        if (dZout) store8<T>(dZout + (p0 + k) * lddz + c0, dzv);
        store8<T>(dY + (p0 + k) * lddy + c0, o);
    }
    }
}
template <typename T>
__global__ void __launch_bounds__(256)
k_bias_grad(const T* __restrict__ dY, int ld, int64_t pixels, int C, float* __restrict__ db, long long* __restrict__ acc_i) {
    __shared__ float red[256 * 8];
    const int cb = C >> 3, lanes = 256 / cb;
    const int mycb = threadIdx.x % cb, lane = threadIdx.x / cb;
    float s[8];
#pragma unroll
    for (int j = 0; j < 8; ++j) s[j] = 0.f;
    const int64_t stride = (int64_t)gridDim.x * lanes;
    int64_t p = (int64_t)blockIdx.x * lanes + lane;
    for (; p + 3 * stride < pixels; p += 4 * stride) {
        float v[4][8];
#pragma unroll
        for (int u = 0; u < 4; ++u) load8<T>(dY + (p + u * stride) * ld + mycb * 8, v[u]);
#pragma unroll
        for (int u = 0; u < 4; ++u)
#pragma unroll
            for (int j = 0; j < 8; ++j) s[j] += v[u][j];
    }
    for (; p < pixels; p += stride) {
        float v[8];
        load8<T>(dY + p * ld + mycb * 8, v);
#pragma unroll
        for (int j = 0; j < 8; ++j) s[j] += v[j];
    }
#pragma unroll
    for (int j = 0; j < 8; ++j) red[threadIdx.x * 8 + j] = s[j];
    __syncthreads();
    for (int c = threadIdx.x; c < C; c += 256) {
        float acc = 0.f;
        for (int l = 0; l < lanes; ++l) acc += red[(l * cb + (c >> 3)) * 8 + (c & 7)];
        if (acc_i) bn_acc_add(acc_i, blockIdx.x, 1, C, 0, 0, c, acc, BN_BS);
        else atomicAdd(db + c, acc);
    }
}
__global__ void __launch_bounds__(256)
k_bias_grad_det(const float* __restrict__ dY, int ld, int64_t pixels, int C, float* __restrict__ db) {
    __shared__ double red[256];
    const int c = blockIdx.x;
    double acc = 0.0;
    for (int64_t p = threadIdx.x; p < pixels; p += 256) acc += (double)dY[p * ld + c];
    red[threadIdx.x] = acc;
    __syncthreads();
    for (int o = 128; o > 0; o >>= 1) {
        if ((int)threadIdx.x < o) red[threadIdx.x] += red[threadIdx.x + o];
        __syncthreads();
    }
    if (threadIdx.x == 0) db[c] += (float)red[0];
}
void launch_bias_grad(int dt, const void* dY, int ld, int64_t pixels, int C, float* db, hipStream_t s, long long* acc_i) {
    if (dt != BF16) {
        k_bias_grad_det<<<C, 256, 0, s>>>((const float*)dY, ld, pixels, C, db);
        return;
    }
    int lanes = 256 / (C / 8);
    int grid = (int)std::min<int64_t>(256, (pixels + 4 * lanes - 1) / (4 * lanes));
    if (grid < 1) grid = 1;
    if (dt == BF16) k_bias_grad<bf16><<<grid, 256, 0, s>>>((const bf16*)dY, ld, pixels, C, db, acc_i);
    else k_bias_grad<float><<<grid, 256, 0, s>>>((const float*)dY, ld, pixels, C, db, acc_i);
}

__global__ void k_dropout_gen(float* __restrict__ mask, int64_t n, uint64_t seed, float p) {
    int64_t i = (int64_t)blockIdx.x * blockDim.x + threadIdx.x;
    if (i >= n) return;
    uint64_t z = seed + 0x9E3779B97F4A7C15ull * (uint64_t)(i + 1);
    z = (z ^ (z >> 30)) * 0xBF58476D1CE4E5B9ull;
    z = (z ^ (z >> 27)) * 0x94D049BB133111EBull;
    z ^= z >> 31;
    float u = (float)(z >> 40) * (1.0f / 16777216.0f);
    mask[i] = u >= p ? 1.0f / (1.0f - p) : 0.f;
}
void launch_dropout_gen(float* mask, int64_t n, uint64_t seed, float p, hipStream_t s) {
    if (n > 0) k_dropout_gen<<<cdiv(n, 256), 256, 0, s>>>(mask, n, seed, p);
}
__global__ void k_fill(float* p, int64_t n, float v) {
    int64_t i = (int64_t)blockIdx.x * blockDim.x + threadIdx.x;
    if (i < n) p[i] = v;
}
void launch_fill(float* p, int64_t n, float v, hipStream_t s) {
    if (n > 0) k_fill<<<cdiv(n, 256), 256, 0, s>>>(p, n, v);
}

template <typename T>
__global__ void k_slice(T* __restrict__ dst, int ldd, const T* __restrict__ src, int lds, int C, int accumulate, int64_t total) {
    int64_t i = (int64_t)blockIdx.x * blockDim.x + threadIdx.x;
    if (i >= total) return;
    const int cb = C >> 3;
    const uint32_t iu = (uint32_t)i;
    const int c0 = (int)(iu % (uint32_t)cb) * 8;
    const int64_t p = iu / (uint32_t)cb;
    float v[8];
    load8<T>(src + p * lds + c0, v);
    if (accumulate) {
        float w[8];
        load8<T>(dst + p * ldd + c0, w);
#pragma unroll
        for (int j = 0; j < 8; ++j) v[j] += w[j];
    }
    store8<T>(dst + p * ldd + c0, v);
}
void launch_slice(int dt, void* dst, int ldd, const void* src, int lds, int64_t pixels, int C, int accumulate, hipStream_t s) {
    int64_t total = pixels * (C / 8);
    if (total == 0) return;
    if (dt == BF16) k_slice<bf16><<<cdiv(total, 256), 256, 0, s>>>((bf16*)dst, ldd, (const bf16*)src, lds, C, accumulate, total);
    else k_slice<float><<<cdiv(total, 256), 256, 0, s>>>((float*)dst, ldd, (const float*)src, lds, C, accumulate, total);
}

constexpr int ECAM_CHUNKS = 128;
template <typename T>
__global__ void __launch_bounds__(256)
k_ecam_pool_part(const T* __restrict__ X, int ld, int64_t HW, int C4, float* __restrict__ part) {
    extern __shared__ float esm[];
    const int n = blockIdx.y, chunk = blockIdx.x, C1 = C4 / 4, CT = C4 + C1;
    const int cb = C4 >> 3, lanes = 256 / cb;
    const int mycb = threadIdx.x % cb, lane = threadIdx.x / cb;
    const bool do_intra = mycb < (C1 >> 3);
    const int64_t per = (HW + gridDim.x - 1) / gridDim.x;
    const int64_t p0 = (int64_t)chunk * per, p1 = min(HW, p0 + per);
    float sm[8], mx[8], smi[8], mxi[8];
    int am[8], ami[8];
#pragma unroll
    for (int j = 0; j < 8; ++j) { sm[j] = smi[j] = 0.f; mx[j] = mxi[j] = -INFINITY; am[j] = ami[j] = 0; }
    for (int64_t p = p0 + lane; p < p1; p += lanes) {
        const T* px = X + ((int64_t)n * HW + p) * ld + mycb * 8;
        float x0[8], x1[8], x2[8], x3[8];
        load8<T>(px, x0);
        if (do_intra) { load8<T>(px + C1, x1); load8<T>(px + 2 * C1, x2); load8<T>(px + 3 * C1, x3); }
#pragma unroll
        for (int j = 0; j < 8; ++j) {
            sm[j] += x0[j];
            if (x0[j] > mx[j]) { mx[j] = x0[j]; am[j] = (int)p; }
        }
        if (do_intra) {
#pragma unroll
            for (int j = 0; j < 8; ++j) {
                const float v = round_as<T>((x0[j] + x1[j]) + (x2[j] + x3[j]));
                smi[j] += v;
                if (v > mxi[j]) { mxi[j] = v; ami[j] = (int)p; }
            }
        }
    }
    float* ssum = esm; float* smax = esm + lanes * CT; int* sarg = reinterpret_cast<int*>(esm + 2 * lanes * CT);
#pragma unroll
    for (int j = 0; j < 8; ++j) {
        const int c = mycb * 8 + j;
        ssum[lane * CT + c] = sm[j]; smax[lane * CT + c] = mx[j]; sarg[lane * CT + c] = am[j];
        if (do_intra) { ssum[lane * CT + C4 + c] = smi[j]; smax[lane * CT + C4 + c] = mxi[j]; sarg[lane * CT + C4 + c] = ami[j]; }
    }
    __syncthreads();
    float* out = part + ((int64_t)n * gridDim.x + chunk) * 3 * CT;
    for (int c = threadIdx.x; c < CT; c += 256) {
        float s_ = 0.f, m_ = -INFINITY;
        int a_ = 0x7fffffff;
// ... 667 lines not shown
```

stcd_amd/engine.py:

```python
from __future__ import annotations

import ctypes as C
from dataclasses import dataclass
from typing import List, Optional, Tuple

import torch

from . import _lib


@dataclass
class ParamInfo:
    name: str
    shape: Tuple[int, ...]
    offset: int
    numel: int


@dataclass
class BnInfo:
    name: str
    channels: int
    calls_per_forward: int
    offset: int
# ... 72 lines not shown
        return {"arch": self.arch, "in_ch": self.in_ch, "label_ch": self.label_ch, "dtype": self.dtype, "cf_config": self.cf_config}

    def __setstate__(self, st):
        self.__init__(st["arch"], st["in_ch"], st["label_ch"], st["dtype"], st.get("cf_config"))

    def __deepcopy__(self, memo):
        return Engine(self.arch, self.in_ch, self.label_ch, self.dtype, self.cf_config)

    def set_dropout_p(self, p: float):
        _lib.check(self._l.stcd_set_dropout_p(self._h, C.c_float(p)))

    def configure(self, batch: int, height: int, width: int, device: torch.device):
        if self.shape == (batch, height, width) and self.workspace is not None and self.workspace.device == device:
            return
        _lib.check(self._l.stcd_configure(self._h, batch, height, width))
        self.shape = (batch, height, width)
        self.dropouts = []
        di = _lib.DropoutInfo()
        for i in range(self._l.stcd_num_dropout(self._h)):
            _lib.check(self._l.stcd_dropout_info_get(self._h, i, C.byref(di)))
            self.dropouts.append(DropoutInfo(di.name.decode(), di.rows, di.channels, di.offset))
        self.dropout_floats = self._l.stcd_dropout_floats(self._h)
        self.workspace = None
        self.workspace = torch.empty(self._l.stcd_workspace_bytes(self._h), dtype=torch.uint8, device=device)

    def output_floats(self) -> int:
        return int(self._l.stcd_output_floats(self._h))

    def cf_outputs(self):
        out = []
        for i in range(5):
            off, hh, ww = C.c_int64(), C.c_int(), C.c_int()
            _lib.check(self._l.stcd_cf_output_info(self._h, i, C.byref(off), C.byref(hh), C.byref(ww)))
            out.append((off.value, hh.value, ww.value))
        return out

    def cf_sites(self):
        st = _lib.CfSite()
        out = []
        for i in range(self._l.stcd_cf_num_sites(self._h)):
            _lib.check(self._l.stcd_cf_site_get(self._h, i, C.byref(st)))
            out.append((st.name.decode(), tuple(st.dims[k] for k in range(st.ndim)), float(st.p)))
        return out

    def cf_set_drop_rates(self, drop_rate: float, attn_drop: float, diff_drop: float):
        _lib.check(self._l.stcd_cf_set_drop_rates(self._h, C.c_float(drop_rate), C.c_float(attn_drop), C.c_float(diff_drop)))
        self.shape = None

    def cf_set_aux_backward(self, on: bool):
        _lib.check(self._l.stcd_cf_set_aux_backward(self._h, 1 if on else 0))
        self.shape = None

    def set_wgrad_side(self, on: bool):
        _lib.check(self._l.stcd_set_wgrad_side(self._h, 1 if on else 0))
        self.shape = None

    def pack_masks(self, masks: dict, device) -> torch.Tensor:
        flat = torch.empty(self.dropout_floats, dtype=torch.float32, device=device)
        for d in self.dropouts:
            m = masks[d.name]
            assert tuple(m.shape) == (d.rows, d.channels), (d.name, tuple(m.shape), d.rows, d.channels)
            flat[d.offset:d.offset + d.rows * d.channels] = m.reshape(-1).to(device)
        return flat

    def forward(self, x1, x2, flat_params, flat_bn, logits, training: bool, masks: Optional[torch.Tensor] = None,
                seed: int = 0):
        self.ticket += 1
        _lib.check(self._l.stcd_forward(self._h, _ptr(x1), _ptr(x2), _ptr(flat_params), _ptr(flat_bn), _ptr(masks),
                                        C.c_uint64(seed & (2 ** 64 - 1)), int(training), _ptr(logits),
                                        _ptr(self.workspace), _stream()))
        return self.ticket

    def backward(self, grad_logits, flat_params, flat_grads, stage: int = -1):
        _lib.check(self._l.stcd_backward(self._h, _ptr(grad_logits), _ptr(flat_params), _ptr(flat_grads),
                                         _ptr(self.workspace), stage, _stream()))

    def set_weights_tag(self, tag: int):
        _lib.check(self._l.stcd_set_weights_tag(self._h, C.c_uint64(tag & (2 ** 64 - 1))))

    def set_debug(self, flags: int):
        _lib.check(self._l.stcd_set_debug(self._h, int(flags)))
        self.shape = None

    def ws_tensors(self):
        out = {}
        wt = _lib.WsTensor()
        for i in range(self._l.stcd_ws_tensor_count(self._h)):
            _lib.check(self._l.stcd_ws_tensor_get(self._h, i, C.byref(wt)))
            dt = torch.bfloat16 if wt.dtype == _lib.DTYPE_IDS["bf16"] else torch.float32
            es = 2 if dt == torch.bfloat16 else 4
            flat = self.workspace[wt.offset_bytes:wt.offset_bytes + wt.n * wt.h * wt.w * wt.ld * es].view(dt)
            out[wt.name.decode()] = flat.view(wt.n, wt.h, wt.w, wt.ld)[..., :wt.c]
        return out

    PROFILE_CLASSES = ("conv", "wgrad", "bn_stats", "bn_act", "bn_bwd_reduce", "bn_bwd_apply", "pool_fuse_bwd", "pack")

    def profile_enable(self, on: bool):
        _lib.check(self._l.stcd_profile_enable(self._h, int(on)))

    def profile_read(self):
        out = {}
        for k, name in enumerate(self.PROFILE_CLASSES):
            ms, n, fl, by = C.c_double(), C.c_int64(), C.c_double(), C.c_double()
            _lib.check(self._l.stcd_profile_read(self._h, k, C.byref(ms), C.byref(n), C.byref(fl), C.byref(by)))
            out[name] = {"ms": ms.value, "launches": n.value, "flops": fl.value, "bytes": by.value}
        return out

    def profile_kernels(self):
        out = {}
        buf = C.create_string_buffer(96)
        for i in range(self._l.stcd_profile_num_kernels(self._h)):
            ms, n, fl, by = C.c_double(), C.c_int64(), C.c_double(), C.c_double()
            _lib.check(self._l.stcd_profile_kernel(self._h, i, buf, 96, C.byref(ms), C.byref(n), C.byref(fl), C.byref(by)))
            out[buf.value.decode()] = {"ms": ms.value, "launches": n.value, "flops": fl.value, "bytes": by.value}
        return out
```

Before: 7909 image-pairs/sec.

## Fuse step prologue launches and split final wgrad reduce to shorten seams

Merges dropout-mask generation, weight packing, workspace zeroing and input packing into one multi-role prologue kernel. The gradient-buffer memset moves into the gout-pack kernel as extra zero-fill blocks. The stage-1 wgrad reduce is split so that jobs not tied to the last wgrad group can run early on the side stream, while the final group runs on the main stream and skips a fork/join. This removes several small launches and serial gaps at the step's entry and tail, at the cost of more bookkeeping and a fused kernel whose blocks do unrelated work.

```diff
diff --git a/include/stcd_hip.h b/include/stcd_hip.h
--- a/include/stcd_hip.h
+++ b/include/stcd_hip.h
@@ -122,6 +122,7 @@
     int dtype;
 } stcd_ws_tensor;
 int stcd_set_debug(stcd_engine* e, int flags);
+int stcd_seam_plan(const stcd_engine* e, int* entry_fused, int* reduce_early_jobs, int* reduce_final_jobs, int* last_tail);
 int stcd_ws_tensor_count(const stcd_engine* e);
 int stcd_ws_tensor_get(const stcd_engine* e, int index, stcd_ws_tensor* out);
 
diff --git a/stcd_amd/_lib.py b/stcd_amd/_lib.py
--- a/stcd_amd/_lib.py
+++ b/stcd_amd/_lib.py
@@ -122,6 +122,7 @@
     "stcd_grad_stage_range": (_i, [_vp, _i, C.POINTER(_i64), C.POINTER(_i64)]),
     "stcd_set_weights_tag": (_i, [_vp, C.c_uint64]),
     "stcd_set_debug": (_i, [_vp, _i]),
+    "stcd_seam_plan": (_i, [_vp, C.POINTER(_i), C.POINTER(_i), C.POINTER(_i), C.POINTER(_i)]),
     "stcd_ws_tensor_count": (_i, [_vp]),
     "stcd_ws_tensor_get": (_i, [_vp, _i, C.POINTER(WsTensor)]),
     "stcd_profile_enable": (_i, [_vp, _i]),
diff --git a/stcd_amd/csrc/common.h b/stcd_amd/csrc/common.h
--- a/stcd_amd/csrc/common.h
+++ b/stcd_amd/csrc/common.h
@@ -85,6 +85,47 @@
 #pragma unroll
     for (int o = 32; o > 0; o >>= 1) v += __shfl_xor(v, o, 64);
     return v;
+}
+
+__device__ __forceinline__ void dropout_gen_body(float* __restrict__ mask, int64_t i, int64_t n, uint64_t seed, float p) {
+    if (i >= n) return;
+    uint64_t z = seed + 0x9E3779B97F4A7C15ull * (uint64_t)(i + 1);
+    z = (z ^ (z >> 30)) * 0xBF58476D1CE4E5B9ull;
+    z = (z ^ (z >> 27)) * 0x94D049BB133111EBull;
+    z ^= z >> 31;
+    float u = (float)(z >> 40) * (1.0f / 16777216.0f);
+    mask[i] = u >= p ? 1.0f / (1.0f - p) : 0.f;
+}
+template <typename T>
+__device__ __forceinline__ void in_pack_body(const float* __restrict__ x1, const float* __restrict__ x2, T* __restrict__ X, int B, int cin,
+                                             int64_t HW, int64_t total, int concat, int64_t i) {
+    if (i >= total) return;
+    int n = (int)(i / HW);
+    int64_t p = i - (int64_t)n * HW;
+    float v[8];
+    if (concat) {
+        const float* s1 = x1 + (int64_t)n * cin * HW + p;
+        const float* s2 = x2 + (int64_t)n * cin * HW + p;
+#pragma unroll
+        for (int c = 0; c < 8; ++c) v[c] = c < cin ? s1[(int64_t)c * HW] : c < 2 * cin ? s2[(int64_t)(c - cin) * HW] : 0.f;
+    } else {
+        const float* src = (n < B ? x1 + (int64_t)n * cin * HW : x2 + (int64_t)(n - B) * cin * HW) + p;
+#pragma unroll
+        for (int c = 0; c < 8; ++c) v[c] = c < cin ? src[(int64_t)c * HW] : 0.f;
+    }
+    store8<T>(X + i * 8, v);
+}
+constexpr int64_t ZERO_BLOCK_BYTES = 256 * 16 * 8;
+inline bool zero_fill_ok(const void* p, int64_t bytes) { return ((uintptr_t)p & 15) == 0 && bytes % 4 == 0; }
+inline int64_t zero_fill_blocks(int64_t bytes) { return bytes > 0 ? (bytes + ZERO_BLOCK_BYTES - 1) / ZERO_BLOCK_BYTES : 0; }
+__device__ __forceinline__ void zero_fill_body(char* __restrict__ p, int64_t bytes, int64_t b) {
+    const int64_t lo = b * ZERO_BLOCK_BYTES;
+    const int64_t hi = bytes < lo + ZERO_BLOCK_BYTES ? bytes : lo + ZERO_BLOCK_BYTES;
+    for (int64_t o = lo + (int64_t)threadIdx.x * 16; o < hi; o += 256 * 16) {
+        if (o + 16 <= hi) *reinterpret_cast<uint4*>(p + o) = make_uint4(0u, 0u, 0u, 0u);
+        else
+            for (int64_t q = o; q < hi; q += 4) *reinterpret_cast<uint32_t*>(p + q) = 0u;
+    }
 }
 
 constexpr int BN_REP = 8;
@@ -191,7 +232,8 @@
 
 
 void launch_in_pack(int dt, const float* x1, const float* x2, void* X, int B, int cin, int H, int W, hipStream_t s, int dates = 2);
-void launch_gout_pack(int dt, const float* g, void* G, int B, int L, int H, int W, hipStream_t s, long long* bias_acc = nullptr);
+int launch_gout_pack(int dt, const float* g, void* G, int B, int L, int H, int W, hipStream_t s, long long* bias_acc = nullptr,
+                     void* zero_p = nullptr, int64_t zero_bytes = 0);
 struct BiasJob { int64_t acc_off; int64_t out_off; int C, valid; float scale; int pad_; };
 void launch_bias_finish(const BiasJob* jobs_dev, int njobs, const char* ws, float* grads, hipStream_t s);
 
@@ -364,6 +406,22 @@
     int aux;
 };
 void launch_pack_jobs(const PackJob* jobs_dev, int njobs, int64_t total, const float* params, char* ws, hipStream_t s);
+inline int64_t pack_job_bytes(const PackJob& j) {
+    switch (j.kind) {
+        case 0: return j.count * 4;
+        case 1: return (j.modeB ? j.count : j.count * j.ps.ntaps) * 2;
+        case 2: return j.count * 2;
+        default: return -1;
+    }
+}
+struct StepPrologue {
+    float* mask; int64_t drop_n; uint64_t seed; float p;
+    const PackJob* jobs; int njobs; int64_t pack_total; const float* params; char* ws;
+    char* zero_p; int64_t zero_bytes;
+    const float* x1; const float* x2; void* X; int B, cin; int64_t HW, in_total; int concat;
+    int drop_end, pack_end, zero_end;
+};
+int launch_step_prologue(int dt, StepPrologue a, hipStream_t s);
 
 int bn_stats_chunks(int64_t pixels_per_group, int C);
 void launch_bn_stats(int dt, const void* Y, int ld, int C, int groups, int64_t pixels_per_group, long long* acc, hipStream_t s);
diff --git a/stcd_amd/csrc/engine.hip b/stcd_amd/csrc/engine.hip
--- a/stcd_amd/csrc/engine.hip
+++ b/stcd_amd/csrc/engine.hip
@@ -245,6 +245,11 @@
     std::vector<WgradGroup> wgroups[2];
     std::vector<ReduceJob> rjobs[2];
     int64_t rjobs_total[2] = {0, 0}, rjobs_off[2] = {-1, -1};
+    const WgradOp* wg_last_op = nullptr;
+    int rj_split = 0, wg_final_group = -1;
+    int64_t rj_total_early = 0, rj_total_final = 0;
+    bool rj_early_done = false, wg_final_on_main = false;
+    int last_tail = 0;
     std::vector<PackJob> jobs[2];
     int64_t jobs_total[2] = {0, 0}, jobs_off[2] = {-1, -1};
     const void* jobs_uploaded_ws = nullptr;
@@ -653,6 +658,7 @@
 static void build_pack_jobs(stcd_engine& e, Planner& ws) {
     for (int st = 0; st < 2; ++st) { e.rjobs[st].clear(); e.rjobs_total[st] = 0; }
     for (int st = 0; st < 2; ++st) e.wgroups[st].clear();
+    e.rj_split = 0; e.wg_final_group = -1; e.rj_early_done = false; e.wg_final_on_main = false;
     if (e.dt == BF16 && e.use_mfma) {
         if (e.use_wgroup) {
             for (WgradOp* op : e.wgrad_ops) {
@@ -724,6 +730,7 @@
                 }
         }
         int64_t cur[2] = {0, 0};
+        std::vector<int> rj_group1;
         for (WgradOp* op : e.wgrad_ops) {
             if (!op->plan.ok) continue;
             const ConvW& cv = e.convs[op->conv];
@@ -770,6 +777,26 @@
             j.start = cur[op->stage];
             cur[op->stage] += (j.count + 255) & ~(int64_t)255;
             e.rjobs[op->stage].push_back(j);
+            if (op->stage == 1) rj_group1.push_back(op->grouped ? op->group : -1);
+        }
+        e.rj_split = 0; e.wg_final_group = -1; e.rj_total_early = e.rj_total_final = 0;
+        if (e.wg_last_op && e.wg_last_op->plan.ok && e.wg_last_op->grouped && e.wg_last_op->stage == 1 && !(e.debug_flags & 2)) {
+            const int gf = e.wg_last_op->group;
+            std::vector<ReduceJob> part[2];
+            bool all_grouped = true;
+            for (size_t i = 0; i < e.rjobs[1].size(); ++i) {
+                all_grouped = all_grouped && rj_group1[i] >= 0;
+                part[rj_group1[i] == gf ? 1 : 0].push_back(e.rjobs[1][i]);
+            }
+            if (all_grouped && !part[0].empty() && !part[1].empty()) {
+                int64_t tot[2] = {0, 0};
+                for (int k = 0; k < 2; ++k)
+                    for (ReduceJob& j : part[k]) { j.start = tot[k]; tot[k] += (j.count + 255) & ~(int64_t)255; }
+                e.rjobs[1] = part[0];
+                e.rjobs[1].insert(e.rjobs[1].end(), part[1].begin(), part[1].end());
+                e.rj_split = (int)part[0].size(); e.wg_final_group = gf;
+                e.rj_total_early = tot[0]; e.rj_total_final = tot[1];
+            }
         }
         for (int st = 0; st < 2; ++st) {
             e.rjobs_total[st] = cur[st];
@@ -1105,7 +1132,27 @@
         rec_layer(R);
     }
 
+    e.wg_last_op = &e.enc[0].wg;
     ws.tables();
+    {
+        struct Rng { int64_t a, b; const char* what; };
+        std::vector<Rng> out;
+        out.push_back({e.X0.off, e.X0.off + (int64_t)ND * B * H * W * 8 * T, "packed input"});
+        out.push_back({e.zero_begin, e.zero_end, "zero range"});
+        if (e.drop_floats > 0) out.push_back({e.masks, e.masks + e.drop_floats * 4, "dropout masks"});
+        const size_t fixed = out.size();
+        for (const PackJob& j : e.jobs[1]) {
+            const int64_t bytes = pack_job_bytes(j);
+            if (bytes < 0) { set_error("internal: a filter pack job of a kind pack_job_bytes does not size"); return 1; }
+            out.push_back({j.dst_off, j.dst_off + bytes, "filter image"});
+        }
+        for (size_t i = 0; i < fixed; ++i)
+            for (size_t k = i + 1; k < out.size(); ++k)
+                if (out[i].a < out[k].b && out[k].a < out[i].b) {
+                    set_error(std::string("internal: the step prologue's outputs overlap (") + out[i].what + " / " + out[k].what + ")");
+                    return 1;
+                }
+    }
     return 0;
 }
 
@@ -1331,8 +1378,9 @@
     launch_unpack_dw(sub, dwe, c.grads + cv.w_off, c.s);
 }
 
-static int pack_all_weights(const Ctx& c, bool with_dgrad) {
+static int pack_prepare(const Ctx& c, bool with_dgrad, bool* need) {
     stcd_engine& e = c.e;
+    *need = false;
     if (e.jobs_uploaded_ws != (const void*)c.ws) {
         for (int k = 0; k < 2; ++k) {
             if (!e.jobs[k].empty())
@@ -1351,9 +1399,18 @@
     const int k = with_dgrad ? 1 : 0;
     if (k == 0 && e.weights_tag != 0 && e.weights_tag == e.packed_tag && e.packed_ws == (const void*)c.ws && e.packed_params == (const void*)c.params)
         return 0;
+    e.packed_tag = k == 0 ? e.weights_tag : 0; e.packed_ws = c.ws; e.packed_params = c.params; e.packed_level = k;
+    *need = true;
+    return 0;
+}
+static int pack_all_weights(const Ctx& c, bool with_dgrad) {
+    stcd_engine& e = c.e;
+    bool need = false;
+    if (pack_prepare(c, with_dgrad, &need)) return 1;
+    if (!need) return 0;
+    const int k = with_dgrad ? 1 : 0;
     ProfScope prof(c, PC_PACK, 0.0, 0.0);
     launch_pack_jobs(c.at<PackJob>(e.jobs_off[k]), (int)e.jobs[k].size(), e.jobs_total[k], c.params, c.ws, c.s);
-    e.packed_tag = k == 0 ? e.weights_tag : 0; e.packed_ws = c.ws; e.packed_params = c.params; e.packed_level = k;
     return 0;
 }
 
@@ -1379,17 +1436,30 @@
     }
 }
 
+static void reduce_early_if_due(const Ctx& c) {
+    stcd_engine& e = c.e;
+    if (e.rj_split <= 0 || e.rj_early_done) return;
+    if (e.prof.on) return;
+    for (size_t g = 0; g < e.wgroups[1].size(); ++g)
+        if ((int)g != e.wg_final_group && !e.wgroups[1][g].launched) return;
+    launch_reduce_jobs(c.at<ReduceJob>(e.rjobs_off[1]), e.rj_split, e.rj_total_early, c.ws, c.grads, c.s);
+    e.rj_early_done = true;
+}
 static void wgroup_member_ready(const Ctx& c, const WgradOp& op) {
     stcd_engine& e = c.e;
     if (op.group < 0 || op.group >= (int)e.wgroups[op.stage].size()) return;
     WgradGroup& G = e.wgroups[op.stage][op.group];
     if (++G.seen < (int)G.jobs.size() || G.launched) return;
-    if (e.wg_cur_side) {
+    const bool final_group = op.stage == 1 && e.rj_split > 0 && op.group == e.wg_final_group;
+    if (e.wg_cur_side && !final_group) {
         if (hipEventRecord(e.wg_fork, c.s) != hipSuccess || hipStreamWaitEvent(e.wg_cur_side, e.wg_fork, 0) != hipSuccess) { set_error("side-stream fork failed"); return; }
         Ctx cs{e, c.ws, c.params, c.grads, e.wg_cur_side};
         launch_wgroup(cs, G);
+        if (op.stage == 1) reduce_early_if_due(cs);
     } else {
         launch_wgroup(c, G);
+        if (final_group && e.wg_cur_side) e.wg_final_on_main = true;
+        else if (op.stage == 1) reduce_early_if_due(c);
     }
 }
 
@@ -1400,6 +1470,14 @@
         G.launched = false; G.seen = 0;
     }
     if (e.rjobs[stage].empty()) return;
+    if (stage == 1 && e.rj_split > 0) {
+        ProfScope prof(c, PC_PACK, 0.0, 0.0, "k_reduce_jobs");
+        if (!e.rj_early_done) launch_reduce_jobs(c.at<ReduceJob>(e.rjobs_off[1]), e.rj_split, e.rj_total_early, c.ws, c.grads, c.s);
+        e.last_tail = (e.rj_early_done ? 1 : 0) | (e.wg_final_on_main ? 2 : 0);
+        e.rj_early_done = false; e.wg_final_on_main = false;
+        launch_reduce_jobs(c.at<ReduceJob>(e.rjobs_off[1]) + e.rj_split, (int)e.rjobs[1].size() - e.rj_split, e.rj_total_final, c.ws, c.grads, c.s);
+        return;
+    }
     ProfScope prof(c, PC_PACK, 0.0, 0.0, "k_reduce_jobs");
     launch_reduce_jobs(c.at<ReduceJob>(e.rjobs_off[stage]), (int)e.rjobs[stage].size(), e.rjobs_total[stage], c.ws, c.grads, c.s);
 }
@@ -1569,15 +1647,45 @@
     Ctx c{e, (char*)workspace, params, nullptr, s};
     const int B = e.B, dt = e.dt;
     const int64_t T = (int64_t)dsize(dt);
+    float gen_p = -1.f;
     if (training && e.drop_p > 0.f) {
         if (masks) STCD_HIP(hipMemcpyAsync(c.at(e.masks), masks, e.drop_floats * 4, hipMemcpyDeviceToDevice, s));
-        else launch_dropout_gen(c.at<float>(e.masks), e.drop_floats, seed, e.drop_p, s);
+        else gen_p = e.drop_p;
     } else if (training && e.fc_virt_layers > 0) {
-        launch_dropout_gen(c.at<float>(e.masks), e.drop_floats, seed, 0.f, s);
-    }
-    if (pack_all_weights(c, training != 0)) return 1;
-    if (training) STCD_HIP(hipMemsetAsync(c.at(e.zero_begin), 0, e.zero_end - e.zero_begin, s));
-    launch_in_pack(dt, x1, x2, c.at(e.X0.off), B, e.in_ch, e.H, e.W, s, e.arch == STCD_ARCH_FCEF ? 0 : 2);
+        gen_p = 0.f;
+    }
+    const int in_dates = e.arch == STCD_ARCH_FCEF ? 0 : 2;
+    if (e.debug_flags & 2) {
+        if (gen_p >= 0.f) launch_dropout_gen(c.at<float>(e.masks), e.drop_floats, seed, gen_p, s);
+        if (pack_all_weights(c, training != 0)) return 1;
+        if (training) STCD_HIP(hipMemsetAsync(c.at(e.zero_begin), 0, e.zero_end - e.zero_begin, s));
+        launch_in_pack(dt, x1, x2, c.at(e.X0.off), B, e.in_ch, e.H, e.W, s, in_dates);
+    } else {
+        StepPrologue a{};
+        if (gen_p >= 0.f) { a.mask = c.at<float>(e.masks); a.drop_n = e.drop_floats; a.seed = seed; a.p = gen_p; }
+        bool need_pack = false;
+        if (pack_prepare(c, training != 0, &need_pack)) return 1;
+        if (need_pack) {
+            const int k = training ? 1 : 0;
+            a.jobs = c.at<PackJob>(e.jobs_off[k]); a.njobs = (int)e.jobs[k].size(); a.pack_total = e.jobs_total[k];
+            a.params = params; a.ws = c.ws;
+        }
+        if (training) {
+            if (zero_fill_ok(c.at(e.zero_begin), e.zero_end - e.zero_begin)) { a.zero_p = c.at<char>(e.zero_begin); a.zero_bytes = e.zero_end - e.zero_begin; }
+            else STCD_HIP(hipMemsetAsync(c.at(e.zero_begin), 0, e.zero_end - e.zero_begin, s));
+        }
+        a.x1 = x1; a.x2 = x2; a.X = c.at(e.X0.off); a.B = B; a.cin = e.in_ch; a.HW = (int64_t)e.H * e.W;
+        a.concat = in_dates == 0 ? 1 : 0;
+        a.in_total = (int64_t)(a.concat ? 1 : in_dates) * B * a.HW;
+        int rc;
+        if (need_pack) {
+            ProfScope prof(c, PC_PACK, 0.0, 0.0);
+            rc = launch_step_prologue(dt, a, s);
+        } else {
+            rc = launch_step_prologue(dt, a, s);
+        }
+        STCD_CHECK(rc == 0, "the step prologue's grid exceeds 2^31 - 1 blocks");
+    }
     for (auto& L : e.enc) cbrd_forward(c, L, bn_running, training != 0);
     size_t di = 0;
     for (int k = 0; k < 4; ++k) {
@@ -1635,6 +1743,13 @@
 static int stage_tail(const Ctx& c, int stage, hipStream_t side, bool wait_join, Extra extra) {
     stcd_engine& e = c.e;
     if (!side) { reduce_stage(c, stage); extra(c); return 0; }
+    if (stage == 1 && e.wg_final_on_main && e.rj_early_done) {
+        STCD_HIP(hipEventRecord(e.wg_join, side));
+        STCD_HIP(hipStreamWaitEvent(c.s, e.wg_join, 0));
+        reduce_stage(c, stage);
+        extra(c);
+        return 0;
+    }
     STCD_HIP(hipEventRecord(e.wg_fork, c.s));
     STCD_HIP(hipStreamWaitEvent(side, e.wg_fork, 0));
     Ctx cs{e, c.ws, c.params, c.grads, side};
@@ -1659,12 +1774,18 @@
     for (int st = 0; st < 2; ++st)
         if (stage < 0 || stage == st)
             for (WgradGroup& G : e.wgroups[st]) { G.seen = 0; G.launched = false; }
+    if (stage != 0) { e.rj_early_done = false; e.wg_final_on_main = false; e.last_tail = 0; }
     const int B = e.B, dt = e.dt;
     const int64_t T = (int64_t)dsize(dt);
     if (stage <= 0) {
-        STCD_HIP(hipMemsetAsync(grads, 0, e.param_floats * 4, s));
+        const bool sep = (e.debug_flags & 2) != 0 || !zero_fill_ok(grads, e.param_floats * 4);
+        if (sep) STCD_HIP(hipMemsetAsync(grads, 0, e.param_floats * 4, s));
         if (!mfma_on(e)) STCD_HIP(hipMemsetAsync(c.at(e.dwe_begin), 0, e.dwe_end - e.dwe_begin, s));
-        launch_gout_pack(dt, grad_logits, c.at(e.G.off), B, e.label, e.H, e.W, s, c.at<long long>(e.final_bias_acc));
+        if (launch_gout_pack(dt, grad_logits, c.at(e.G.off), B, e.label, e.H, e.W, s, c.at<long long>(e.final_bias_acc),
+                             sep ? nullptr : grads, e.param_floats * 4)) {
+            set_error("internal: k_gout_pack rejected the gradient buffer's zero-fill");
+            return 1;
+        }
         exec_wgrad(c, e.final_wg, c.at(e.finalIn.off), c.at(e.G.off));
         {
             BwdSum bs;
@@ -2857,7 +2978,7 @@
 static void reset_plan(stcd_engine& e) {
     e.enc.clear(); e.dec.clear(); e.ups.clear();
     e.drops.clear(); e.drop_floats = 0;
-    e.conv_ops.clear(); e.wgrad_ops.clear(); e.slab_floats = 0;
+    e.conv_ops.clear(); e.wgrad_ops.clear(); e.slab_floats = 0; e.wg_last_op = nullptr;
     e.ws_tensors.clear(); e.bias_jobs.clear();
     e.g_fwd.clear(); e.sn_order.clear();
     if (e.cf) cf_reset_plan(*e.cf);
@@ -3110,6 +3231,15 @@
     STCD_CHECK(e != nullptr, "engine is null");
     e->debug_flags = flags;
     e->configured = false;
+    return 0;
+}
+int stcd_seam_plan(const stcd_engine* e, int* entry_fused, int* reduce_early_jobs, int* reduce_final_jobs, int* last_tail) {
+    STCD_CHECK(e && entry_fused && reduce_early_jobs && reduce_final_jobs && last_tail, "null argument");
+    STCD_CHECK(e->configured, "stcd_configure first");
+    *entry_fused = (fc_family(*e) && !(e->debug_flags & 2)) ? 1 : 0;
+    *reduce_early_jobs = e->rj_split;
+    *reduce_final_jobs = e->rj_split > 0 ? (int)e->rjobs[1].size() - e->rj_split : 0;
+    *last_tail = e->last_tail;
     return 0;
 }
 int stcd_ws_tensor_count(const stcd_engine* e) { return e ? (int)e->ws_tensors.size() : 0; }
diff --git a/stcd_amd/csrc/kernels_conv_mfma.hip b/stcd_amd/csrc/kernels_conv_mfma.hip
--- a/stcd_amd/csrc/kernels_conv_mfma.hip
+++ b/stcd_amd/csrc/kernels_conv_mfma.hip
@@ -283,9 +283,9 @@
     return src[(a_ * ps.ks + ps.ky[t]) * ps.ks + ps.kx[t]];
 }
 
-__global__ void __launch_bounds__(256)
-k_pack_jobs(const PackJob* __restrict__ jobs, int njobs, int64_t total, const float* __restrict__ params, char* __restrict__ ws) {
-    const int64_t i0 = (int64_t)blockIdx.x * blockDim.x, i = i0 + threadIdx.x;
+__device__ __forceinline__ void pack_jobs_body(const PackJob* __restrict__ jobs, int njobs, const float* __restrict__ params,
+                                               char* __restrict__ ws, int64_t blk) {
+    const int64_t i0 = blk * 256, i = i0 + threadIdx.x;
     int lo = 0, hi = njobs - 1;
     while (lo < hi) {
         const int mid = (lo + hi + 1) >> 1;
@@ -340,8 +340,36 @@
         reinterpret_cast<bf16*>(ws + jb.dst_off)[e] = (bf16)v;
     }
 }
+__global__ void __launch_bounds__(256)
+k_pack_jobs(const PackJob* __restrict__ jobs, int njobs, int64_t total, const float* __restrict__ params, char* __restrict__ ws) {
+    pack_jobs_body(jobs, njobs, params, ws, (int64_t)blockIdx.x);
+}
 void launch_pack_jobs(const PackJob* jobs_dev, int njobs, int64_t total, const float* params, char* ws, hipStream_t s) {
     if (njobs > 0 && total > 0) k_pack_jobs<<<(unsigned)((total + 255) / 256), 256, 0, s>>>(jobs_dev, njobs, total, params, ws);
+}
+
+template <typename T>
+__global__ void __launch_bounds__(256)
+k_step_prologue(StepPrologue a) {
+    const int b = (int)blockIdx.x;
+    if (b < a.drop_end) dropout_gen_body(a.mask, (int64_t)b * 256 + threadIdx.x, a.drop_n, a.seed, a.p);
+    else if (b < a.pack_end) pack_jobs_body(a.jobs, a.njobs, a.params, a.ws, (int64_t)(b - a.drop_end));
+    else if (b < a.zero_end) zero_fill_body(a.zero_p, a.zero_bytes, (int64_t)(b - a.pack_end));
+    else in_pack_body<T>(a.x1, a.x2, (T*)a.X, a.B, a.cin, a.HW, a.in_total, a.concat, (int64_t)(b - a.zero_end) * 256 + threadIdx.x);
+}
+int launch_step_prologue(int dt, StepPrologue a, hipStream_t s) {
+    if (a.drop_n <= 0 || !a.mask) a.drop_n = 0;
+    if (a.njobs <= 0 || a.pack_total <= 0) { a.njobs = 0; a.pack_total = 0; }
+    if (!a.zero_p || a.zero_bytes <= 0) a.zero_bytes = 0;
+    if (a.in_total < 0) a.in_total = 0;
+    const int64_t b0 = (a.drop_n + 255) / 256, b1 = b0 + (a.pack_total + 255) / 256, b2 = b1 + zero_fill_blocks(a.zero_bytes),
+                  grid = b2 + (a.in_total + 255) / 256;
+    if (grid > 0x7fffffff) return 1;
+    a.drop_end = (int)b0; a.pack_end = (int)b1; a.zero_end = (int)b2;
+    if (grid <= 0) return 0;
+    if (dt == BF16) k_step_prologue<bf16><<<(unsigned)grid, 256, 0, s>>>(a);
+    else k_step_prologue<float><<<(unsigned)grid, 256, 0, s>>>(a);
+    return 0;
 }
 
 void launch_pack_frag(const stcd_conv_geom& g, const ConvMfmaPlan& p, const float* w, int kpad, int wld, void* dst,
diff --git a/stcd_amd/csrc/kernels_ew.hip b/stcd_amd/csrc/kernels_ew.hip
--- a/stcd_amd/csrc/kernels_ew.hip
+++ b/stcd_amd/csrc/kernels_ew.hip
@@ -77,22 +77,7 @@
 template <typename T>
 __global__ void k_in_pack(const float* __restrict__ x1, const float* __restrict__ x2, T* __restrict__ X, int B, int cin,
                           int64_t HW, int64_t total, int concat) {
-    int64_t i = (int64_t)blockIdx.x * blockDim.x + threadIdx.x;
-    if (i >= total) return;
-    int n = (int)(i / HW);
-    int64_t p = i - (int64_t)n * HW;
-    float v[8];
-    if (concat) {
-        const float* s1 = x1 + (int64_t)n * cin * HW + p;
-        const float* s2 = x2 + (int64_t)n * cin * HW + p;
-#pragma unroll
-        for (int c = 0; c < 8; ++c) v[c] = c < cin ? s1[(int64_t)c * HW] : c < 2 * cin ? s2[(int64_t)(c - cin) * HW] : 0.f;
-    } else {
-        const float* src = (n < B ? x1 + (int64_t)n * cin * HW : x2 + (int64_t)(n - B) * cin * HW) + p;
-#pragma unroll
-        for (int c = 0; c < 8; ++c) v[c] = c < cin ? src[(int64_t)c * HW] : 0.f;
-    }
-    store8<T>(X + i * 8, v);
+    in_pack_body<T>(x1, x2, X, B, cin, HW, total, concat, (int64_t)blockIdx.x * blockDim.x + threadIdx.x);
 }
 
 void launch_in_pack(int dt, const float* x1, const float* x2, void* X, int B, int cin, int H, int W, hipStream_t s, int dates) {
@@ -104,8 +89,13 @@
 
 template <typename T>
 __global__ void __launch_bounds__(256)
-k_gout_pack(const float* __restrict__ g, T* __restrict__ G, int B, int L, int64_t HW, long long* __restrict__ bias_acc) {
+k_gout_pack(const float* __restrict__ g, T* __restrict__ G, int B, int L, int64_t HW, long long* __restrict__ bias_acc,
+            int pack_blocks, char* __restrict__ zero_p, int64_t zero_bytes) {
     __shared__ float red[4][8];
+    if ((int)blockIdx.x >= pack_blocks) {
+        zero_fill_body(zero_p, zero_bytes, (int64_t)blockIdx.x - pack_blocks);
+        return;
+    }
     int64_t i = (int64_t)blockIdx.x * blockDim.x + threadIdx.x;
     float v[8];
 #pragma unroll
@@ -130,10 +120,17 @@
     }
 }
 
-void launch_gout_pack(int dt, const float* g, void* G, int B, int L, int H, int W, hipStream_t s, long long* bias_acc) {
+int launch_gout_pack(int dt, const float* g, void* G, int B, int L, int H, int W, hipStream_t s, long long* bias_acc, void* zero_p,
+                     int64_t zero_bytes) {
     int64_t HW = (int64_t)H * W, n = (int64_t)B * HW;
-    if (dt == BF16) k_gout_pack<bf16><<<cdiv(n, 256), 256, 0, s>>>(g, (bf16*)G, B, L, HW, bias_acc);
-    else k_gout_pack<float><<<cdiv(n, 256), 256, 0, s>>>(g, (float*)G, B, L, HW, bias_acc);
+    if (!zero_p || zero_bytes <= 0) { zero_p = nullptr; zero_bytes = 0; }
+    else if (!zero_fill_ok(zero_p, zero_bytes)) return 1;
+    const int64_t blocks = (n + 255) / 256 + zero_fill_blocks(zero_bytes);
+    if (blocks > 0x7fffffff) return 1;
+    const int pb = cdiv(n, 256), grid = (int)blocks;
+    if (dt == BF16) k_gout_pack<bf16><<<grid, 256, 0, s>>>(g, (bf16*)G, B, L, HW, bias_acc, pb, (char*)zero_p, zero_bytes);
+    else k_gout_pack<float><<<grid, 256, 0, s>>>(g, (float*)G, B, L, HW, bias_acc, pb, (char*)zero_p, zero_bytes);
+    return 0;
 }
 
 __global__ void k_bias_finish(const BiasJob* __restrict__ jobs, const char* __restrict__ ws, float* __restrict__ grads) {
@@ -1019,14 +1016,7 @@
 }
 
 __global__ void k_dropout_gen(float* __restrict__ mask, int64_t n, uint64_t seed, float p) {
-    int64_t i = (int64_t)blockIdx.x * blockDim.x + threadIdx.x;
-    if (i >= n) return;
-    uint64_t z = seed + 0x9E3779B97F4A7C15ull * (uint64_t)(i + 1);
-    z = (z ^ (z >> 30)) * 0xBF58476D1CE4E5B9ull;
-    z = (z ^ (z >> 27)) * 0x94D049BB133111EBull;
-    z ^= z >> 31;
-    float u = (float)(z >> 40) * (1.0f / 16777216.0f);
-    mask[i] = u >= p ? 1.0f / (1.0f - p) : 0.f;
+    dropout_gen_body(mask, (int64_t)blockIdx.x * blockDim.x + threadIdx.x, n, seed, p);
 }
 void launch_dropout_gen(float* mask, int64_t n, uint64_t seed, float p, hipStream_t s) {
     if (n > 0) k_dropout_gen<<<cdiv(n, 256), 256, 0, s>>>(mask, n, seed, p);
diff --git a/stcd_amd/engine.py b/stcd_amd/engine.py
--- a/stcd_amd/engine.py
+++ b/stcd_amd/engine.py
@@ -178,6 +178,11 @@
         _lib.check(self._l.stcd_set_debug(self._h, int(flags)))
         self.shape = None
 
+    def seam_plan(self):
+        v = [C.c_int() for _ in range(4)]
+        _lib.check(self._l.stcd_seam_plan(self._h, *[C.byref(x) for x in v]))
+        return tuple(x.value for x in v)
+
     def ws_tensors(self):
         out = {}
         wt = _lib.WsTensor()
```

Result: faster. 8018 image-pairs/sec (median of 6 runs) (+1.4%).
